# blyssprivacy/sdk

Measured on NVIDIA H100. Metric: PIR server queries/sec (Spiral process_query), higher is better.
Workload: dtype u64

## Files before the change

sdk_b200/build.py:

```python
import os
import subprocess
import sys

HERE = os.path.dirname(os.path.abspath(__file__))
CSRC = os.path.join(HERE, "csrc")
SO = os.path.join(HERE, "libb200pir.so")
SOURCES = ["api.cu", "poly_kernels.cu", "mul_kernels.cu", "imma_kernels.cu", "wire_kernels.cu", "tc5_kernels.cu", "dpir_gemm.cu",
           "export_kernels.cu"]
HEADERS = ["common.cuh", "kernels.h", "ntt_core.cuh", "tc5_layout.cuh", "tc5_ptx.cuh", "ntt_core4096.cuh", "ntt_tables.hpp",
           "item_place.cuh", "update_body.hpp", os.path.join("..", "..", "include", "b200pir.h")]
NVCC_FLAGS = ["-gencode", "arch=compute_90a,code=sm_90a", "-lineinfo", "-O3", "-std=c++17", "--extended-lambda",
              "-Xcompiler", "-fPIC", "-ccbin", "/usr/bin/g++" if os.path.exists("/usr/bin/g++") else "g++"]


def _stale():
    if not os.path.exists(SO):
        return True
    t = os.path.getmtime(SO)
    return any(os.path.getmtime(os.path.join(CSRC, f)) > t for f in SOURCES + HEADERS)


def build(force=False, verbose=False):
    if not force and not _stale():
        return SO
    nvcc = os.environ.get("NVCC", "/usr/local/cuda/bin/nvcc")
    objs = []
    procs = []
    for src in SOURCES:
        obj = os.path.join(CSRC, src.replace(".cu", ".o"))
        cmd = [nvcc] + NVCC_FLAGS + (["-Xptxas", "-v"] if verbose else []) + ["-c", os.path.join(CSRC, src), "-o", obj]
        procs.append((src, subprocess.Popen(cmd, stdout=subprocess.PIPE, stderr=subprocess.STDOUT, text=True)))
        objs.append(obj)
    for src, p in procs:
        out, _ = p.communicate()
        if verbose or p.returncode:
            sys.stderr.write(out)
        if p.returncode:
            raise RuntimeError("nvcc failed on " + src)
    subprocess.check_call([nvcc, "-shared", "-gencode", "arch=compute_90a,code=sm_90a", "-o", SO] + objs + ["-ccbin", NVCC_FLAGS[-1]])
    return SO


if __name__ == "__main__":
    print(build(force="--force" in sys.argv, verbose="-v" in sys.argv))
```

sdk_b200/csrc/api.cu:

```cuda
#include "../../include/b200pir.h"
#include "kernels.h"
#include "ntt_tables.hpp"
#include "update_body.hpp"
#include <cstdio>
#include <cerrno>
#include <fcntl.h>
#include <unistd.h>
#include <algorithm>
#include <cmath>
#include <memory>
#include <cstring>
#include <condition_variable>
#include <chrono>
#include <deque>
#include <mutex>
#include <set>
#include <string>
#include <utility>
#include <vector>

using namespace b200pir;

namespace b200pir {
thread_local unsigned long long g_kernel_launches = 0;

void opt_in_smem_impl(const void* kernel, int bytes) {
  static std::mutex mu;
  static std::set<std::pair<const void*, int>> done;
  int dev = 0;
  B200_CUDA(cudaGetDevice(&dev));
  std::lock_guard<std::mutex> lk(mu);
  if (done.count({kernel, dev})) return;
  B200_CUDA(cudaFuncSetAttribute(kernel, cudaFuncAttributeMaxDynamicSharedMemorySize, bytes));
  done.insert({kernel, dev});
}
}

namespace {

thread_local std::string g_last_error;

using b200pir::tables::build_tables;
using b200pir::tables::invmod;
uint64_t log2_ceil_u64(uint64_t a) { return (uint64_t)std::ceil(std::log2((double)a)); }
int bits_per(int t) {
  if (t == 56) return 1;
  return 56 / t + 1;
}
const uint64_t kQ2Values[37] = {0, 0, 0, 0, 0, 0, 0, 0, 0, 0, 0, 0, 0, 0, 12289ULL, 12289ULL, 61441ULL, 65537ULL,
                                65537ULL, 520193ULL, 786433ULL, 786433ULL, 3604481ULL, 7340033ULL, 16515073ULL,
                                33292289ULL, 67043329ULL, 132120577ULL, 268369921ULL, 469762049ULL, 1073479681ULL,
                                2013265921ULL, 4293918721ULL, 8588886017ULL, 17175674881ULL, 34359214081ULL,
                                68718428161ULL};

template <typename T>
struct DevBuf {
  T* p = nullptr;
  size_t n = 0;
  DevBuf() {}
  explicit DevBuf(size_t count) { alloc(count); }
  void alloc(size_t count) {
    release();
    n = count;
    if (count) B200_CUDA(cudaMalloc(&p, count * sizeof(T)));
  }
  void ensure(size_t count) { if (count > n) alloc(count); }
  void release() { if (p) cudaFree(p); p = nullptr; n = 0; }
  ~DevBuf() { release(); }
  DevBuf(const DevBuf&) = delete;
  DevBuf& operator=(const DevBuf&) = delete;
};

enum Stage { ST_EXPAND = 0, ST_MUL, ST_FROMNTT, ST_FOLD, ST_PACK, ST_ENCODE, ST_QIMG , ST_COUNT };

}

struct b200pir_ctx {
  int device = 0;
  cudaStream_t stream = nullptr;
  bool own_stream = true;
  std::recursive_mutex mu;
  b200pir_params hp;
  int dim0, num_per, slices, trials, g, stop_round, num_packing;
  int bits_gsw, bits_conv, bits_left, bits_right;
  bool has_right;
  uint64_t q2, q1, setup_bytes, query_bytes, response_bytes;
  int q1_bits;
  DevParams dp;
  DevBuf<Twiddle> d_tw;
  DevBuf<Twiddle> d_tw4k;
  DevBuf<uint32_t> d_neg1;
  int mul_variant = 0, max_group = 16, profile = 0;
  int intt_variant = 0;
  int expand_variant = 0;
  long pair_min_ctas = 1;
  int sparse_fold = 0;
  int imma_variant = 0;
  int db_format = -1;
  DevBuf<uint2> w_qf;
  DevBuf<uint8_t> w_qt;
  int sm_count = 0;
  size_t ws_queries = 0, ws_rows = 0;
  DevBuf<uint64_t> w_query;
  DevBuf<uint32_t> w_v;
  DevBuf<uint32_t> w_zflags;
  DevBuf<uint32_t> w_xr;
  DevBuf<uint4> w_qdev;
  DevBuf<uint32_t> w_vfold, w_vfold_neg;
  DevBuf<uint32_t> w_mult;
  DevBuf<uint32_t> w_cts;
  const uint32_t* folded = nullptr;
  size_t folded_stride = 0;
  DevBuf<uint64_t> w_packed;
  DevBuf<uint8_t> w_resp;
  static constexpr size_t kWriteStageBytes = (size_t)64 << 20;
  static constexpr size_t kWriteStageItems = 65536;
  DevBuf<uint8_t> w_wbytes;
  DevBuf<ItemWrite> w_witems;
  std::mutex export_mu;
  uint8_t* h_export[2] = {nullptr, nullptr};
  size_t h_export_bytes = 0;
  cudaEvent_t export_done[2] = {nullptr, nullptr};
  void ensure_export_staging(size_t bytes) {
    w_wbytes.ensure(std::max(kWriteStageBytes, bytes));
    if (!export_done[0])
      for (auto& e : export_done) B200_CUDA(cudaEventCreateWithFlags(&e, cudaEventDisableTiming | cudaEventBlockingSync));
    if (bytes <= h_export_bytes) return;
    release_export_pinned();
    const size_t n = std::max(kWriteStageBytes, bytes);
    for (auto& h : h_export) B200_CUDA(cudaHostAlloc(reinterpret_cast<void**>(&h), n, cudaHostAllocDefault));
    h_export_bytes = n;
  }
  void release_export_pinned() {
    for (auto& h : h_export) { if (h) cudaFreeHost(h); h = nullptr; }
    h_export_bytes = 0;
  }
  struct Pending {
    b200pir_db* db; b200pir_pp* pp; const uint64_t* query_ct; const uint8_t* query_bytes; uint8_t* out;
    int rc = 0; std::string err; bool done = false;
  };
  static constexpr size_t kCoalesceMax = 32;
  static constexpr size_t kPassQueries = 16;
  int coalesce = 1;
  int coalesce_window_us = 200;
  size_t last_batch = 0;
  std::chrono::steady_clock::time_point last_batch_end{};
  std::mutex qmu;
  std::condition_variable qcv;
  std::deque<Pending*> pending;
  bool leader_active = false;
  unsigned long long coalesced_batches = 0, coalesced_queries = 0;
  DevBuf<const uint32_t*> d_pptab;
  size_t pptab_cap = 0;
  std::vector<const uint32_t*> h_pptab;
  b200pir_pp* const* multi_pps = nullptr;
  PpTable pp_table(b200pir_pp* pp, size_t count);
  struct Span { int stage; cudaEvent_t a, b; };
  std::vector<Span> spans;
  std::vector<cudaEvent_t> event_pool;
  size_t event_next = 0;
  int mul_launches = 0;
  double last_ms[9] = {0, 0, 0, 0, 0, 0, 0, 0, 0};

  size_t v_words() const { return ((size_t)1 << g) * 4 * POLY; }
  size_t fold_words() const { return (size_t)hp.nu_2 * 2 * 2 * hp.t_gsw * 2 * POLY; }
  MulGeom geom(int rows) const { return MulGeom{dim0, rows, slices}; }

  cudaEvent_t get_event() {
    if (event_next == event_pool.size()) {
      cudaEvent_t e;
      B200_CUDA(cudaEventCreate(&e));
      event_pool.push_back(e);
    }
    return event_pool[event_next++];
  }
  struct Scope {
    b200pir_ctx* c; int stage; cudaEvent_t a = nullptr;
    Scope(b200pir_ctx* ctx, int st) : c(ctx), stage(st) {
      if (c->profile) { a = c->get_event(); cudaEventRecord(a, c->stream); }
    }
    ~Scope() {
      if (c->profile) { cudaEvent_t b = c->get_event(); cudaEventRecord(b, c->stream); c->spans.push_back({stage, a, b}); }
    }
  };
  void prof_reset() { if (profile == 2) return; spans.clear(); event_next = 0; mul_launches = 0; }
  void prof_collect() {
    if (!profile) return;
    B200_CUDA(cudaStreamSynchronize(stream));
    for (int i = 0; i < 9; i++) last_ms[i] = 0;
    for (auto& s : spans) {
      float ms = 0;
      cudaEventElapsedTime(&ms, s.a, s.b);
      last_ms[s.stage == ST_QIMG ? 8 : s.stage] += ms;
      last_ms[6] += ms;
    }
    last_ms[7] = mul_launches;
  }
  void ensure_workspace_lite(size_t queries, size_t rows) {
    w_mult.ensure(queries * slices * rows * 4 * POLY);
    w_cts.ensure(queries * slices * rows * 4 * POLY);
    w_packed.ensure(queries * hp.instances * (hp.n + 1) * hp.n * POLY);
  }
  void ensure_workspace(size_t queries, size_t rows) {
    if (queries <= ws_queries && rows <= ws_rows) return;
    queries = std::max(queries, ws_queries);
    rows = std::max(rows, ws_rows);
    w_query.ensure(queries * 2 * POLY);
    if (hp.expand_queries) w_v.ensure(queries * v_words());
    w_qdev.ensure(queries * (size_t)dim0 * POLY);
    w_vfold.ensure(queries * std::max<size_t>(fold_words(), 1));
    w_vfold_neg.ensure(queries * std::max<size_t>(fold_words(), 1));
    w_mult.ensure(queries * slices * rows * 4 * POLY);
    w_cts.ensure(queries * slices * rows * 4 * POLY);
    w_packed.ensure(queries * hp.instances * (hp.n + 1) * hp.n * POLY);
    w_resp.ensure(queries * response_bytes);
    ws_queries = queries;
    ws_rows = rows;
  }
};

struct b200pir_db {
  b200pir_ctx* ctx;
  Shard shard;
  int rows;
  int format = 0;
  DevBuf<uint4> d;
  DevBuf<uint4> f;
  DevBuf<uint8_t> t;
  Tc5Geom T;
  ImmaGeom F;
  size_t slice_cells() const { return (size_t)rows * (ctx->dim0 / 2) * POLY; }
  std::vector<uint64_t> present;
  uint64_t present_count = 0;
  std::vector<uint32_t> h_tile_mask;
  DevBuf<uint32_t> tile_mask;
  uint64_t capacity() const { return (uint64_t)ctx->slices * rows * ctx->dim0; }
  void presence_init() {
    present.assign((capacity() + 63) / 64, 0);
    present_count = 0;
    h_tile_mask.assign((size_t)ctx->slices * T.mt, 0u);
    tile_mask.alloc(h_tile_mask.size());
    B200_CUDA(cudaMemset(tile_mask.p, 0, h_tile_mask.size() * 4));
  }
  bool mark_host(int slice, int il, int j) {
    const uint64_t bit = ((uint64_t)slice * rows + il) * ctx->dim0 + j;
    if (!((present[bit >> 6] >> (bit & 63)) & 1)) { present[bit >> 6] |= 1ull << (bit & 63); present_count++; }
    const size_t w = (size_t)slice * T.mt + (il >> 5);
    const uint32_t nv = h_tile_mask[w] | (1u << (j >> 5));
    if (nv == h_tile_mask[w]) return false;
    h_tile_mask[w] = nv;
    return true;
  }
  void mark(int slice, int il, int j, cudaStream_t s) {
    if (mark_host(slice, il, j)) {
      const size_t w = (size_t)slice * T.mt + (il >> 5);
      B200_CUDA(cudaMemcpyAsync(tile_mask.p + w, &h_tile_mask[w], 4, cudaMemcpyHostToDevice, s));
    }
  }
  void mark_items(const ItemWrite* items, size_t count, cudaStream_t s) {
    bool changed = false;
    for (size_t k = 0; k < count; k++)
      for (int sl = 0; sl < ctx->slices; sl++) changed |= mark_host(sl, (int)items[k].il, (int)items[k].j);
    if (changed)
      B200_CUDA(cudaMemcpyAsync(tile_mask.p, h_tile_mask.data(), h_tile_mask.size() * 4, cudaMemcpyHostToDevice, s));
  }
  void mark_slice(int slice, cudaStream_t s) {
    const uint64_t lo = (uint64_t)slice * rows * ctx->dim0, hi = lo + (uint64_t)rows * ctx->dim0;
    for (uint64_t b = lo; b < hi; b++)
      if (!((present[b >> 6] >> (b & 63)) & 1)) { present[b >> 6] |= 1ull << (b & 63); present_count++; }
    const uint32_t full = T.ks >= 32 ? 0xffffffffu : ((1u << T.ks) - 1u);
    for (int m = 0; m < T.mt; m++) h_tile_mask[(size_t)slice * T.mt + m] = full;
    B200_CUDA(cudaMemcpyAsync(tile_mask.p + (size_t)slice * T.mt, &h_tile_mask[(size_t)slice * T.mt], (size_t)T.mt * 4,
                              cudaMemcpyHostToDevice, s));
  }
};

struct b200pir_pp {
  b200pir_ctx* ctx;
  DevBuf<uint32_t> pack, left, right, conv;
};

PpTable b200pir_ctx::pp_table(b200pir_pp* pp, size_t count) {
  if (count > pptab_cap) {
    pptab_cap = std::max<size_t>(count, 16);
    d_pptab.alloc(4 * pptab_cap);
    h_pptab.clear();
  }
  std::vector<const uint32_t*> h(4 * pptab_cap, nullptr);
  for (size_t i = 0; i < count; i++) {
    const b200pir_pp* p = multi_pps ? multi_pps[i] : pp;
    h[0 * pptab_cap + i] = p->pack.p;
    h[1 * pptab_cap + i] = p->left.p;
    h[2 * pptab_cap + i] = p->right.p ? p->right.p : p->left.p;
    h[3 * pptab_cap + i] = p->conv.p;
  }
  if (h != h_pptab) {
    B200_CUDA(cudaMemcpyAsync(d_pptab.p, h.data(), h.size() * sizeof(const uint32_t*), cudaMemcpyHostToDevice, stream));
    h_pptab = h;
  }
  return PpTable{d_pptab.p, d_pptab.p + pptab_cap, d_pptab.p + 2 * pptab_cap, d_pptab.p + 3 * pptab_cap};
}

struct b200pir_dpir {
  int device;
  std::mutex mu;
  cudaStream_t stream = nullptr;
  bool own_stream = true;
  uint64_t rows, cols;
  DevBuf<uint32_t> a;
  DevBuf<uint32_t> b, out;
};

namespace {

int fail(const std::exception& e) {
  cudaGetLastError();
  g_last_error = e.what();
  const Error* pe = dynamic_cast<const Error*>(&e);
  return pe ? pe->code : B200PIR_E_CUDA;
}
#define API_BEGIN try {
#define API_END                                     \
  }                                                 \
  catch (const std::exception& e) { return fail(e); } \
  return 0;

struct Guard {
  std::lock_guard<std::recursive_mutex> lk;
  explicit Guard(b200pir_ctx* c) : lk(c->mu) { cudaSetDevice(c->device); }
};

void upload_ntt32(b200pir_ctx* c, DevBuf<uint32_t>& dst, const uint64_t* host, size_t words) {
  dst.alloc(words);
  DevBuf<uint64_t> tmp(words);
  B200_CUDA(cudaMemcpyAsync(tmp.p, host, words * 8, cudaMemcpyHostToDevice, c->stream));
  launch_narrow(dst.p, tmp.p, words, c->stream);
  B200_CUDA(cudaStreamSynchronize(c->stream));
}


void run_coefficient_expansion(b200pir_ctx* c, b200pir_pp* pp, uint32_t* v, size_t v_stride, int nq, bool all_slots) {
  const auto& hp = c->hp;
  cudaStream_t s = c->stream;
  const int g = c->g;
  const int stop_round = hp.nu_2 > 0 ? c->stop_round : 0;
  const int max_right = hp.nu_2 > 0 ? (int)(hp.t_gsw * hp.nu_2) : 0;
  const PpTable T = c->pp_table(pp, (size_t)nq);
  for (int r = 0; r < g; r++) {
    const int num_in = 1 << r;
    const long active = (long)((stop_round > 0 && r > stop_round) ? num_in / 2 : num_in) * nq;
    const bool pair = c->expand_variant != 1 && active >= c->pair_min_ctas;
    if (!pair) launch_expand_scalar(c->dp, v, v_stride, nq, num_in, c->d_neg1.p + (size_t)r * 2 * POLY, s);
    ExpandRound R;
    R.r = r; R.num_in = num_in; R.stop_round = stop_round; R.max_bits_to_gen_right = max_right;
    R.fill_skipped = all_slots ? 1 : 0;
    R.t_auto = (POLY >> r) + 1;
    R.t_left = (int)hp.t_exp_left; R.bits_left = c->bits_left;
    R.tab_left = T.left; R.off_left = (size_t)r * 2 * hp.t_exp_left * 2 * POLY;
    if (hp.nu_2 > 0 && c->has_right) {
      int rr = r <= c->stop_round ? r : c->stop_round;
      R.t_right = (int)hp.t_exp_right; R.bits_right = c->bits_right;
      R.tab_right = T.right; R.off_right = (size_t)rr * 2 * hp.t_exp_right * 2 * POLY;
    } else {
      R.t_right = R.t_left; R.bits_right = R.bits_left; R.tab_right = T.left; R.off_right = R.off_left;
    }
    if (pair && c->expand_variant == 0) {
      const size_t xr_stride = (size_t)num_in * 2 * POLY;
      c->w_xr.ensure((size_t)nq * xr_stride);
      launch_expand_round_res(c->dp, v, v_stride, c->w_xr.p, xr_stride, nq, R, c->d_neg1.p + (size_t)r * 2 * POLY, s);
    } else if (pair) launch_expand_round_pair(c->dp, v, v_stride, nq, R, c->d_neg1.p + (size_t)r * 2 * POLY, s);
    else launch_expand_round(c->dp, v, v_stride, nq, R, s);
  }
}

void run_expand_query(b200pir_ctx* c, b200pir_pp* pp, const uint64_t* query_raw, uint32_t* v, uint4* q_dev,
                      uint32_t* v_fold, int nq, uint8_t* images = nullptr) {
  const auto& hp = c->hp;
  cudaStream_t s = c->stream;
  launch_to_ntt_strided(c->dp, v, c->v_words(), query_raw, (size_t)2 * POLY, 2, nq, s);
  run_coefficient_expansion(c, pp, v, c->v_words(), nq, false);
  const int factor = hp.nu_2 > 0 ? 2 : 1;
  if (images) {
    const Tc5Geom T = make_tc5_geom(c->dim0, 32);
    for (int q0 = 0; q0 < nq; q0 += 16)
      launch_reorient_to_tc5(T, v + (size_t)q0 * c->v_words(), c->v_words(), factor, std::min(16, nq - q0),
                             images + (size_t)(q0 / 16) * tc5_query_bytes(T), s);
  } else {
    launch_reorient(c->geom(c->num_per), q_dev, (size_t)c->dim0 * POLY, v, c->v_words(), nq, factor, s);
  }
  if (hp.nu_2 > 0)
    launch_regev_to_gsw(c->dp, v_fold, c->fold_words(), v, c->v_words(), nq, (int)hp.nu_2, 2, 1, c->pp_table(pp, (size_t)nq).conv,
                        (int)hp.t_gsw, (int)hp.t_conv, c->bits_conv, s);
}

void run_fold(b200pir_ctx* c, uint64_t* cts, size_t batch, size_t batch_stride, size_t num, int k0,
              const uint32_t* vfold, const uint32_t* vfold_neg, int slices_per_query) {
  const size_t mat = (size_t)2 * 2 * c->hp.t_gsw * 2 * POLY;
  int k = k0;
  for (size_t half = num / 2; half >= 1; half /= 2, k--) {
    launch_fold_round(c->dp, cts, batch, batch_stride, (int)half, vfold + (size_t)k * mat, vfold_neg + (size_t)k * mat,
                      c->fold_words(), slices_per_query, (int)c->hp.t_gsw, c->bits_gsw, c->stream);
  }
}

const uint32_t* run_fold_res(b200pir_ctx* c, uint32_t* a, uint32_t* b, size_t batch, size_t batch_stride, size_t num,
                             int k0, const uint32_t* vfold, int slices_per_query) {
  const size_t mat = (size_t)2 * 2 * c->hp.t_gsw * 2 * POLY;
  int k = k0;
  uint32_t* src = a;
  uint32_t* dst = b;
  uint32_t* zero_flags = nullptr;
  if (c->sparse_fold) {
    c->w_zflags.ensure(batch * num);
    zero_flags = c->w_zflags.p;
  }
  for (size_t half = num / 2; half >= 1; half /= 2, k--) {
    launch_fold_res(c->dp, src, dst, batch, batch_stride, (int)half, vfold + (size_t)k * mat, c->fold_words(),
                    slices_per_query, (int)c->hp.t_gsw, c->bits_gsw, zero_flags, c->stream);
    std::swap(src, dst);
  }
  return src;
}

void run_prepare(b200pir_ctx* c, b200pir_pp* pp, size_t count, bool images = false) {
  b200pir_ctx::Scope sc(c, ST_EXPAND);
  if (images) c->w_qt.ensure((count + 15) / 16 * tc5_query_bytes(make_tc5_geom(c->dim0, 32)));
  if (c->hp.expand_queries)
    run_expand_query(c, pp, c->w_query.p, c->w_v.p, c->w_qdev.p, c->w_vfold.p, (int)count, images ? c->w_qt.p : nullptr);
}

void run_first_dim_and_fold(b200pir_ctx* c, b200pir_db* db, size_t count, const uint4* qdev = nullptr,
                            const uint32_t* vfold = nullptr, const uint8_t* images = nullptr, size_t per_group = 16) {
  if (!qdev) qdev = c->w_qdev.p;
  if (!vfold) vfold = c->w_vfold.p;
  const int rows = db->rows;
  MulGeom G = c->geom(rows);
  const size_t q_stride = (size_t)c->dim0 * POLY;
  const size_t out_stride = (size_t)c->slices * rows * 4 * POLY;
  if (db->format == 0) {
    {
      b200pir_ctx::Scope sc(c, ST_MUL);
      size_t qi = 0;
      while (qi < count) {
        int nq = 1;
        if (count - qi >= 4 && c->max_group >= 4) nq = 4;
        else if (count - qi >= 2 && c->max_group >= 2) nq = 2;
        launch_multiply(c->dp, G, db->d.p, qdev + qi * q_stride, c->w_mult.p + qi * out_stride, 0, c->slices, nq,
                        q_stride, out_stride, c->mul_variant, c->stream);
        c->mul_launches++;
        qi += nq;
      }
    }
    {
      b200pir_ctx::Scope sc(c, ST_FROMNTT);
      launch_ntt32(c->dp, c->w_mult.p, count * c->slices * rows * 2, true, c->stream);
    }
  } else if (db->format == 2) {
    if (!images) c->w_qt.ensure(tc5_query_bytes(db->T));
    const size_t step = images ? per_group : 16;
    for (size_t qi = 0, g = 0; qi < count; qi += step, g++) {
      const int nq = (int)std::min<size_t>(step, count - qi);
      const uint8_t* qt = images ? images + g * tc5_query_bytes(db->T) : c->w_qt.p;
      if (!images) {
        b200pir_ctx::Scope sq(c, ST_QIMG);
        launch_query_to_tc5(db->T, qdev + qi * q_stride, q_stride, nq, c->w_qt.p, c->stream);
      }
      b200pir_ctx::Scope sc(c, ST_MUL);
      launch_multiply_tc5(c->dp, db->T, db->t.p, db->tile_mask.p, qt, c->w_cts.p + qi * out_stride, out_stride, nq, 0, c->slices,
                          c->sm_count, c->stream);
      c->mul_launches++;
    }
    {
      b200pir_ctx::Scope sc(c, ST_FROMNTT);
      launch_intt_from_zmajor(c->dp, db->F, c->w_cts.p, out_stride, c->w_mult.p, (int)count, c->slices, c->intt_variant, c->stream);
    }
  } else {
    c->w_qf.ensure(imma_query_cells(db->F));
    const size_t per_pass = (c->max_group >= 16 && imma_supports_16(db->F)) ? 16 : (c->max_group >= 8 ? 8 : 4);
    for (size_t qi = 0; qi < count; qi += per_pass) {
      const int nq = (int)std::min<size_t>(per_pass, count - qi);
      {
        b200pir_ctx::Scope sq(c, ST_QIMG);
        launch_query_to_frag(db->F, qdev + qi * q_stride, q_stride, nq, c->w_qf.p, c->stream);
      }
      {
        b200pir_ctx::Scope sc(c, ST_MUL);
        launch_multiply_imma(c->dp, db->F, db->f.p, c->w_qf.p, c->w_cts.p + qi * out_stride, out_stride, nq, 0, c->slices,
                             c->imma_variant, c->stream);
        c->mul_launches++;
      }
    }
    {
      b200pir_ctx::Scope sc(c, ST_FROMNTT);
      launch_intt_from_zmajor(c->dp, db->F, c->w_cts.p, out_stride, c->w_mult.p, (int)count, c->slices, c->intt_variant, c->stream);
    }
  }
  {
    b200pir_ctx::Scope sc(c, ST_FOLD);
    c->folded = c->w_mult.p;
    c->folded_stride = (size_t)rows * 4 * POLY;
    if (rows > 1)
      c->folded = run_fold_res(c, c->w_mult.p, c->w_cts.p, count * c->slices, (size_t)rows * 4 * POLY, rows,
                               (int)c->hp.nu_2 - 1, vfold, c->slices);
  }
}

void run_pack_encode(b200pir_ctx* c, b200pir_pp* pp, const uint32_t* folded, size_t ct_stride, size_t count,
                     uint8_t* out_dev) {
  const auto& hp = c->hp;
  const size_t packed_words = (size_t)hp.instances * (hp.n + 1) * hp.n * POLY;
  {
    b200pir_ctx::Scope sc(c, ST_PACK);
    launch_pack(c->dp, c->w_packed.p, packed_words, folded, ct_stride, (size_t)c->slices * ct_stride, (int)count, c->pp_table(pp, count).pack,
                (int)hp.n, (int)hp.instances, (int)hp.t_conv, c->bits_conv, (int)hp.version, c->stream);
  }
  {
    b200pir_ctx::Scope sc(c, ST_ENCODE);
    launch_encode(c->dp, out_dev, c->response_bytes, c->w_packed.p, packed_words, (int)count, (int)hp.n, (int)hp.instances,
                  c->q2, (int)hp.q2_bits, c->q1, c->q1_bits, c->stream);
  }
}

bool same_params(const b200pir_ctx* a, const b200pir_ctx* b) {
  return a == b || (a->device == b->device && std::memcmp(&a->hp, &b->hp, sizeof(b200pir_params)) == 0);
}
void check_db(b200pir_ctx* c, b200pir_db* db) {
  if (!db || !same_params(db->ctx, c)) throw Error(B200PIR_E_BADARG, "db handle was created for different parameters / device");
}
void check_pp(b200pir_ctx* c, b200pir_pp* pp) {
  if (!pp || !same_params(pp->ctx, c)) throw Error(B200PIR_E_BADARG, "pp handle was created for different parameters / device");
}

}

extern "C" {

const char* b200pir_last_error(void) { return g_last_error.c_str(); }
int b200pir_device_count(void) {
  int n = 0;
  if (cudaGetDeviceCount(&n) != cudaSuccess) return 0;
  return n;
}

int b200pir_ctx_create(const b200pir_params* params, int device, b200pir_ctx** out) {
  API_BEGIN
  if (!params || !out) throw Error(B200PIR_E_BADARG, "null argument");
  int ndev = 0;
  B200_CUDA(cudaGetDeviceCount(&ndev));
  if (device < 0 || device >= ndev) throw Error(B200PIR_E_BADARG, "no such CUDA device (this library has no CPU path)");
  B200_CUDA(cudaSetDevice(device));
  std::unique_ptr<b200pir_ctx> c(new b200pir_ctx());
  c->device = device;
  B200_CUDA(cudaDeviceGetAttribute(&c->sm_count, cudaDevAttrMultiProcessorCount, device));
  c->hp = *params;
  auto& hp = c->hp;
  if (hp.q2_bits < 14) hp.q2_bits = 14;
  if (hp.q2_bits > 36) throw Error(B200PIR_E_BADARG, "q2_bits out of range");
  if (hp.instances == 0) hp.instances = 1;
  if (hp.n < 1 || hp.n > 4) throw Error(B200PIR_E_UNSUPPORTED, "n must be 1..4");
  if (hp.nu_1 < 1 || hp.nu_1 > 16 || hp.nu_2 > 16) throw Error(B200PIR_E_BADARG, "nu_1/nu_2 out of range");
  if (hp.version > 1) throw Error(B200PIR_E_BADARG, "unknown version");
  if (hp.p < 2 || (hp.p & (hp.p - 1)) || hp.p > (1u << 20)) throw Error(B200PIR_E_BADARG, "p must be a power of two <= 2^20");
  for (uint64_t t : {hp.t_gsw, hp.t_conv, hp.t_exp_left, hp.t_exp_right})
    if (t < 3 || t > 56)
      throw Error(B200PIR_E_UNSUPPORTED, "gadget dimensions must be in 3..56");
  if (hp.db_item_size == 0) hp.db_item_size = hp.instances * hp.n * hp.n * 2048 * log2_ceil_u64(hp.p) / 8;
  c->dim0 = 1 << hp.nu_1;
  c->num_per = 1 << hp.nu_2;
  c->trials = (int)(hp.n * hp.n);
  c->slices = (int)(hp.instances * c->trials);
  c->g = (int)log2_ceil_u64(hp.t_gsw * hp.nu_2 + c->dim0);
  c->stop_round = hp.nu_2 ? (int)log2_ceil_u64(hp.t_gsw * hp.nu_2) : 0;
  if (c->g > 11) throw Error(B200PIR_E_UNSUPPORTED, "expansion needs more than 2048 slots");
  if (hp.expand_queries && hp.nu_2 > 0 && 2 * std::max<uint64_t>(c->dim0, hp.t_gsw * hp.nu_2) > (1ull << c->g))
    throw Error(B200PIR_E_UNSUPPORTED, "expansion: dim0 and t_gsw * nu_2 must each fit in half of the 2^g slots");
  c->num_packing = hp.version == 0 ? (int)hp.n : 2;
  c->has_right = hp.expand_queries && (hp.version == 0 || hp.t_exp_right != hp.t_exp_left);
  c->bits_gsw = bits_per((int)hp.t_gsw);
  c->bits_conv = bits_per((int)hp.t_conv);
  c->bits_left = bits_per((int)hp.t_exp_left);
  c->bits_right = bits_per((int)hp.t_exp_right);
  c->q2 = kQ2Values[hp.q2_bits];
  c->q1 = 4 * hp.p;
  c->q1_bits = (int)log2_ceil_u64(c->q1);
  {
    uint64_t bits = hp.instances * (hp.q2_bits * hp.n * 2048 + (uint64_t)c->q1_bits * hp.n * hp.n * 2048);
    c->response_bytes = ((bits + 63) / 64) * 8;
    uint64_t sz = (uint64_t)c->num_packing * hp.n * hp.t_conv;
    if (hp.expand_queries) {
      uint64_t right = (uint64_t)(c->stop_round + 1) * hp.t_exp_right;
      if (hp.version > 0 && hp.t_exp_left == hp.t_exp_right) right = 0;
      sz += (uint64_t)c->g * hp.t_exp_left + right + 2 * hp.t_conv;
    }
    c->setup_bytes = 32 + sz * 2048 * 8;
    uint64_t qp = hp.expand_queries ? 1 : (uint64_t)c->dim0 + hp.nu_2 * 2 * hp.t_gsw;
    c->query_bytes = 32 + qp * 2048 * 8;
  }
  B200_CUDA(cudaStreamCreateWithFlags(&c->stream, cudaStreamNonBlocking));
  const uint64_t q0 = 268369921ULL, q1m = 249561089ULL;
  std::vector<Twiddle> f0, i0, f1, i1;
  build_tables(q0, f0, i0);
  build_tables(q1m, f1, i1);
  std::vector<Twiddle> l0, l1;
  b200pir::tables::build_inverse_table_lz(q0, l0);
  b200pir::tables::build_inverse_table_lz(q1m, l1);
  c->d_tw.alloc(6 * POLY);
  B200_CUDA(cudaMemcpy(c->d_tw.p + 4 * POLY, l0.data(), POLY * sizeof(Twiddle), cudaMemcpyHostToDevice));
  B200_CUDA(cudaMemcpy(c->d_tw.p + 5 * POLY, l1.data(), POLY * sizeof(Twiddle), cudaMemcpyHostToDevice));
  B200_CUDA(cudaMemcpy(c->d_tw.p, f0.data(), POLY * sizeof(Twiddle), cudaMemcpyHostToDevice));
  B200_CUDA(cudaMemcpy(c->d_tw.p + POLY, i0.data(), POLY * sizeof(Twiddle), cudaMemcpyHostToDevice));
  B200_CUDA(cudaMemcpy(c->d_tw.p + 2 * POLY, f1.data(), POLY * sizeof(Twiddle), cudaMemcpyHostToDevice));
  B200_CUDA(cudaMemcpy(c->d_tw.p + 3 * POLY, i1.data(), POLY * sizeof(Twiddle), cudaMemcpyHostToDevice));
  {
    std::vector<Twiddle> lo(2 * 3 * 64);
    for (int i = 0; i < 64; i++) { lo[(0 * 3 + 0) * 64 + i] = f0[i]; lo[(0 * 3 + 1) * 64 + i] = i0[i]; lo[(0 * 3 + 2) * 64 + i] = l0[i];
                                   lo[(1 * 3 + 0) * 64 + i] = f1[i]; lo[(1 * 3 + 1) * 64 + i] = i1[i]; lo[(1 * 3 + 2) * 64 + i] = l1[i]; }
    upload_poly_constants(lo.data());
    upload_mul_constants(lo.data());
    upload_imma_constants(lo.data());
  }
  DevParams& dp = c->dp;
  dp.q[0] = (uint32_t)q0; dp.q[1] = (uint32_t)q1m;
  dp.cr1[0] = (uint64_t)(((u128)1 << 64) / q0);
  dp.cr1[1] = (uint64_t)(((u128)1 << 64) / q1m);
  dp.modulus = q0 * q1m;
  dp.cr1_mod = (uint64_t)(((u128)1 << 64) / dp.modulus);
  dp.q1_inv_mod_q0 = (uint32_t)invmod(q1m % q0, q0);
  dp.fwd[0] = c->d_tw.p; dp.inv[0] = c->d_tw.p + POLY; dp.fwd[1] = c->d_tw.p + 2 * POLY; dp.inv[1] = c->d_tw.p + 3 * POLY;
  dp.inv_lz[0] = c->d_tw.p + 4 * POLY; dp.inv_lz[1] = c->d_tw.p + 5 * POLY;
  dp.mu58[0] = (uint32_t)(((uint64_t)1 << 58) / q0); dp.mu58[1] = (uint32_t)(((uint64_t)1 << 58) / q1m);
  {
    std::vector<uint32_t> h((size_t)NTT_LOG_N * 2 * POLY, 0);
    for (int i = 0; i < NTT_LOG_N; i++) {
      int idx = POLY - (1 << i);
      h[((size_t)i * 2 + 0) * POLY + idx] = (uint32_t)(q0 - 1);
      h[((size_t)i * 2 + 1) * POLY + idx] = (uint32_t)(q1m - 1);
    }
    c->d_neg1.alloc(h.size());
    B200_CUDA(cudaMemcpy(c->d_neg1.p, h.data(), h.size() * 4, cudaMemcpyHostToDevice));
    launch_ntt32(dp, c->d_neg1.p, NTT_LOG_N, false, c->stream);
    B200_CUDA(cudaStreamSynchronize(c->stream));
  }
  B200_CUDA(cudaGetLastError());
  *out = c.release();
  API_END
}

void b200pir_ctx_destroy(b200pir_ctx* c) {
  if (!c) return;
  cudaSetDevice(c->device);
  cudaDeviceSynchronize();
  for (auto e : c->event_pool) cudaEventDestroy(e);
  c->release_export_pinned();
  for (auto e : c->export_done) if (e) cudaEventDestroy(e);
  if (c->own_stream && c->stream) cudaStreamDestroy(c->stream);
  delete c;
}
int b200pir_ctx_set_stream(b200pir_ctx* c, void* cuda_stream) {
  API_BEGIN
  if (!c) throw Error(B200PIR_E_BADARG, "null ctx");
  Guard gd(c);
  B200_CUDA(cudaStreamSynchronize(c->stream));
  if (c->own_stream && c->stream) cudaStreamDestroy(c->stream);
  c->stream = (cudaStream_t)cuda_stream;
  c->own_stream = false;
  API_END
}
int b200pir_ctx_synchronize(b200pir_ctx* c) {
  API_BEGIN
  if (!c) throw Error(B200PIR_E_BADARG, "null ctx");
  Guard gd(c);
  B200_CUDA(cudaStreamSynchronize(c->stream));
  B200_CUDA(cudaGetLastError());
  API_END
}
int b200pir_ctx_reserve(b200pir_ctx* c, size_t queries, size_t rows_local) {
  API_BEGIN
  if (!c) throw Error(B200PIR_E_BADARG, "null ctx");
  if (queries == 0 || queries > 4096 || rows_local == 0 || rows_local > ((size_t)1 << c->hp.nu_2))
    throw Error(B200PIR_E_BADARG, "reserve: 1..4096 queries, 1..num_per rows");
  Guard gd(c);
  B200_CUDA(cudaStreamSynchronize(c->stream));
  c->ensure_workspace(queries, rows_local);
  B200_CUDA(cudaGetLastError());
  API_END
}
int b200pir_ctx_set_option(b200pir_ctx* c, const char* key, int64_t value) {
  API_BEGIN
  if (!c || !key) throw Error(B200PIR_E_BADARG, "null argument");
  Guard gd(c);
  std::string k(key);
  if (k == "mul_variant") c->mul_variant = (int)value;
  else if (k == "batch") { if (value != 1 && value != 2 && value != 4 && value != 8 && value != 16) throw Error(B200PIR_E_BADARG, "batch must be 1, 2, 4, 8 or 16"); c->max_group = (int)value; }
  else if (k == "fold_variant") {}
  else if (k == "intt_variant") c->intt_variant = (int)value;
  else if (k == "imma_variant") c->imma_variant = (int)value;
  else if (k == "sparse_fold") c->sparse_fold = value != 0;
  else if (k == "coalesce") c->coalesce = value != 0;
  else if (k == "coalesce_window_us") { if (value < 0 || value > 100000) throw Error(B200PIR_E_BADARG, "coalesce_window_us must be 0..100000"); c->coalesce_window_us = (int)value; }
  else if (k == "expand_variant") c->expand_variant = (int)value;
  else if (k == "expand_pair_min_ctas") c->pair_min_ctas = (long)value;
  else if (k == "db_format") { if (value < -1 || value > 2) throw Error(B200PIR_E_BADARG, "db_format must be -1 (automatic), 0, 1 or 2"); c->db_format = (int)value; }
  else if (k == "profile") {
    if (value < 0 || value > 2) throw Error(B200PIR_E_BADARG, "profile must be 0, 1 or 2");
    c->profile = (int)value;
    c->spans.clear(); c->event_next = 0; c->mul_launches = 0;
  }
  else throw Error(B200PIR_E_BADARG, "unknown option " + k);
  API_END
}
int b200pir_ctx_sizes(b200pir_ctx* c, uint64_t* setup_bytes, uint64_t* query_bytes, uint64_t* response_bytes) {
  API_BEGIN
  if (!c) throw Error(B200PIR_E_BADARG, "null ctx");
  if (setup_bytes) *setup_bytes = c->setup_bytes;
  if (query_bytes) *query_bytes = c->query_bytes;
  if (response_bytes) *response_bytes = c->response_bytes;
  API_END
}

int b200pir_db_create(b200pir_ctx* c, uint64_t shard_index, uint64_t shard_count, b200pir_db** out) {
  API_BEGIN
  if (!c || !out) throw Error(B200PIR_E_BADARG, "null argument");
  Guard gd(c);
  if (shard_count == 0) { shard_count = 1; shard_index = 0; }
  if (shard_index >= shard_count || (shard_count & (shard_count - 1)) || (uint64_t)c->num_per % shard_count)
    throw Error(B200PIR_E_BADARG, "shard_count must be a power of two dividing num_per");
  std::unique_ptr<b200pir_db> db(new b200pir_db());
  db->ctx = c;
  db->shard = Shard{(int)shard_index, (int)shard_count};
  db->rows = c->num_per / (int)shard_count;
  db->F = make_imma_geom(c->dim0, db->rows);
  db->T = make_tc5_geom(c->dim0, db->rows);
  db->format = c->db_format >= 0 ? c->db_format : (tc5_supported(db->T) ? 2 : 1);
  db->presence_init();
  if (db->format == 0) {
    size_t cells = (size_t)c->slices * db->slice_cells();
    db->d.alloc(cells);
    B200_CUDA(cudaMemsetAsync(db->d.p, 0, cells * sizeof(uint4), c->stream));
  } else if (db->format == 2) {
    if (!tc5_supported(db->T)) throw Error(B200PIR_E_UNSUPPORTED, "db_format 2: dim0 too large for the wgmma kernel");
    size_t bytes = tc5_db_bytes(db->T, c->slices);
    db->t.alloc(bytes);
    B200_CUDA(cudaMemsetAsync(db->t.p, 0, bytes, c->stream));
  } else {
    size_t cells = imma_db_cells(db->F, c->slices);
    db->f.alloc(cells);
    B200_CUDA(cudaMemsetAsync(db->f.p, 0, cells * sizeof(uint4), c->stream));
  }
  B200_CUDA(cudaStreamSynchronize(c->stream));
  *out = db.release();
  API_END
}
void b200pir_db_destroy(b200pir_db* db) {
  if (!db) return;
  cudaSetDevice(db->ctx->device);
  delete db;
}
extern "C++" {
namespace {
template <typename Fetch>
void upload_slice_impl(b200pir_ctx* c, b200pir_db* db, uint64_t slice, Fetch fetch) {
  const size_t per_z = (size_t)c->dim0 * c->num_per;
  int zc = (int)std::max<size_t>(1, std::min<size_t>(POLY, ((size_t)64 << 20) / (per_z * 8)));
  DevBuf<uint64_t> stage(per_z * zc);
  MulGeom G = c->geom(db->rows);
  DevBuf<uint4> tmp;
  uint4* dst;
  if (db->format == 0) dst = db->d.p + (size_t)slice * db->slice_cells();
  else { tmp.alloc(db->slice_cells()); dst = tmp.p; }
  for (int z0 = 0; z0 < POLY; z0 += zc) {
    int cur = std::min(zc, POLY - z0);
    const uint64_t* src = fetch((size_t)z0 * per_z, per_z * cur);
    B200_CUDA(cudaMemcpyAsync(stage.p, src, per_z * cur * 8, cudaMemcpyHostToDevice, c->stream));
    launch_db_retile_chunk(G, db->shard, dst, stage.p, z0, cur, c->stream);
    B200_CUDA(cudaStreamSynchronize(c->stream));
  }
  if (db->format == 1) {
    launch_db_to_frag(db->F, tmp.p, db->f.p, (int)slice, c->stream);
    B200_CUDA(cudaStreamSynchronize(c->stream));
  } else if (db->format == 2) {
    launch_db_to_tc5(db->T, tmp.p, db->t.p, (int)slice, c->stream);
    B200_CUDA(cudaStreamSynchronize(c->stream));
  }
  db->mark_slice((int)slice, c->stream);
  B200_CUDA(cudaStreamSynchronize(c->stream));
  B200_CUDA(cudaGetLastError());
}

void write_items(b200pir_ctx* c, b200pir_db* db, const uint8_t* host, size_t span, const ItemWrite* items, size_t count) {
  if (count == 0) return;
  c->w_wbytes.ensure(std::max(b200pir_ctx::kWriteStageBytes, span));
  c->w_witems.ensure(std::max(b200pir_ctx::kWriteStageItems, count));
  if (span) B200_CUDA(cudaMemcpyAsync(c->w_wbytes.p, host, span, cudaMemcpyHostToDevice, c->stream));
  B200_CUDA(cudaMemcpyAsync(c->w_witems.p, items, count * sizeof(ItemWrite), cudaMemcpyHostToDevice, c->stream));
  const size_t chunks = (size_t)c->slices;
  const size_t bpc = (c->hp.db_item_size + chunks - 1) / chunks;
  const DbDst dst{db->format, c->geom(db->rows), db->F, db->T, db->d.p, db->f.p, db->t.p};
  launch_write_items(c->dp, dst, c->w_wbytes.p, c->w_witems.p, (int)count, (int)chunks, (int)bpc, c->hp.p, c->stream);
}

template <typename Sink>
void export_impl(b200pir_ctx* c, b200pir_db* db, int slice_begin, int slice_end, Sink sink) {
  std::lock_guard<std::mutex> ex(c->export_mu);
  const size_t per_z = (size_t)db->rows * c->dim0;
  const int zc = (int)std::max<size_t>(1, std::min<size_t>(POLY, b200pir_ctx::kWriteStageBytes / (per_z * 8)));
  struct Chunk { int slice, z0, zc; };
  std::vector<Chunk> chunks;
  for (int s = slice_begin; s < slice_end; s++)
    for (int z0 = 0; z0 < POLY; z0 += zc) chunks.push_back(Chunk{s, z0, std::min(zc, POLY - z0)});
  {
    Guard gd(c);
    c->ensure_export_staging(per_z * zc * 8);
  }
  auto consume = [&](size_t k) {
    const int b = (int)(k & 1);
    B200_CUDA(cudaEventSynchronize(c->export_done[b]));
    sink(chunks[k].slice, chunks[k].z0, chunks[k].zc, reinterpret_cast<const uint64_t*>(c->h_export[b]));
  };
  try {
    for (size_t k = 0; k < chunks.size(); k++) {
      {
        Guard gd(c);
        const DbDst dst{db->format, c->geom(db->rows), db->F, db->T, db->d.p, db->f.p, db->t.p};
        uint64_t* stage = reinterpret_cast<uint64_t*>(c->w_wbytes.p);
        launch_db_export(dst, chunks[k].slice, chunks[k].z0, chunks[k].zc, stage, c->stream);
        B200_CUDA(cudaMemcpyAsync(c->h_export[k & 1], stage, per_z * chunks[k].zc * 8, cudaMemcpyDeviceToHost, c->stream));
        B200_CUDA(cudaEventRecord(c->export_done[k & 1], c->stream));
      }
      if (k > 0) consume(k - 1);
    }
    if (!chunks.empty()) consume(chunks.size() - 1);
  } catch (...) {
    for (auto e : c->export_done) cudaEventSynchronize(e);
    throw;
  }
  B200_CUDA(cudaGetLastError());
}

void download_impl(b200pir_ctx* c, b200pir_db* db, int slice_begin, int slice_end, uint64_t* words) {
  const size_t d0 = (size_t)c->dim0, npg = (size_t)c->num_per, rows = (size_t)db->rows;
  const size_t G = (size_t)db->shard.count, gi = (size_t)db->shard.index;
  const size_t slice_words = d0 * npg * POLY;
  export_impl(c, db, slice_begin, slice_end, [&](int s, int z0, int zc, const uint64_t* src) {
    uint64_t* dst = words + (size_t)(s - slice_begin) * slice_words + (size_t)z0 * npg * d0;
    if (G == 1) { std::memcpy(dst, src, (size_t)zc * rows * d0 * 8); return; }
    for (size_t zl = 0; zl < (size_t)zc; zl++)
      for (size_t il = 0; il < rows; il++)
        std::memcpy(dst + (zl * npg + il * G + gi) * d0, src + (zl * rows + il) * d0, d0 * 8);
  });
}
}
}

int b200pir_db_upload_slice(b200pir_ctx* c, b200pir_db* db, uint64_t slice, const uint64_t* words, size_t n_words) {
  API_BEGIN
  if (!c || !words) throw Error(B200PIR_E_BADARG, "null argument");
  Guard gd(c);
  check_db(c, db);
  const size_t slice_words = (size_t)c->dim0 * c->num_per * POLY;
  if (slice >= (uint64_t)c->slices) throw Error(B200PIR_E_SHAPE, "slice out of range");
  if (n_words != slice_words) throw Error(B200PIR_E_SHAPE, "slice must hold dim0*num_per*2048 words");
  upload_slice_impl(c, db, slice, [&](size_t off, size_t) { return words + off; });
  API_END
}
int b200pir_db_load_file(b200pir_ctx* c, b200pir_db* db, const char* path) {
  API_BEGIN
  if (!c || !path) throw Error(B200PIR_E_BADARG, "null argument");
  Guard gd(c);
  check_db(c, db);
  const size_t slice_words = (size_t)c->dim0 * c->num_per * POLY;
  struct Closer { FILE* f; ~Closer() { if (f) fclose(f); } } file{fopen(path, "rb")};
  if (!file.f) throw Error(B200PIR_E_BADARG, std::string("cannot open ") + path);
  if (fseeko(file.f, 0, SEEK_END)) throw Error(B200PIR_E_BADARG, "cannot seek in the database file");
  const off_t bytes = ftello(file.f);
  if (bytes < 0 || (uint64_t)bytes != (uint64_t)slice_words * c->slices * 8)
    throw Error(B200PIR_E_SHAPE, "database file must hold slices*dim0*num_per*2048 u64 words");
  std::vector<uint64_t> buf;
  for (int s = 0; s < c->slices; s++) {
    upload_slice_impl(c, db, (uint64_t)s, [&](size_t off, size_t n) -> const uint64_t* {
      buf.resize(n);
      if (fseeko(file.f, (off_t)(((size_t)s * slice_words + off) * 8), SEEK_SET) || fread(buf.data(), 8, n, file.f) != n)
        throw Error(B200PIR_E_SHAPE, "short read from the database file");
      return buf.data();
    });
// ... 209 lines not shown
  check_db(c, db);
  MulGeom G = c->geom(db->rows);
  size_t per_slice = (size_t)db->rows * (c->dim0 / 2);
  int step = (int)std::max<size_t>(1, std::min<size_t>(c->slices, ((size_t)1 << 30) / per_slice));
  if (db->format == 0) {
    for (int s0 = 0; s0 < c->slices; s0 += step)
      launch_db_synth(c->dp, G, db->shard, db->d.p, seed, c->hp.p, s0, std::min(step, c->slices - s0), c->stream);
  } else {
    DevBuf<uint4> tmp(db->slice_cells());
    for (int s0 = 0; s0 < c->slices; s0++) {
      launch_db_synth(c->dp, G, db->shard, tmp.p - (size_t)s0 * db->slice_cells(), seed, c->hp.p, s0, 1, c->stream);
      if (db->format == 2) launch_db_to_tc5(db->T, tmp.p, db->t.p, s0, c->stream);
      else launch_db_to_frag(db->F, tmp.p, db->f.p, s0, c->stream);
    }
  }
  for (int s0 = 0; s0 < c->slices; s0++) db->mark_slice(s0, c->stream);
  B200_CUDA(cudaStreamSynchronize(c->stream));
  B200_CUDA(cudaGetLastError());
  API_END
}

int b200pir_pp_create(b200pir_ctx* c, const uint64_t* v_packing, const uint64_t* left, const uint64_t* right,
                      const uint64_t* conv, b200pir_pp** out) {
  API_BEGIN
  if (!c || !out || !v_packing) throw Error(B200PIR_E_BADARG, "null argument");
  Guard gd(c);
  const auto& hp = c->hp;
  std::unique_ptr<b200pir_pp> pp(new b200pir_pp());
  pp->ctx = c;
  const size_t W = 2 * POLY;
  upload_ntt32(c, pp->pack, v_packing, (size_t)c->num_packing * (hp.n + 1) * hp.t_conv * W);
  if (hp.expand_queries) {
    if (!left || !conv) throw Error(B200PIR_E_BADARG, "expansion parameters missing");
    upload_ntt32(c, pp->left, left, (size_t)c->g * 2 * hp.t_exp_left * W);
    if (c->has_right) {
      if (!right) throw Error(B200PIR_E_BADARG, "v_expansion_right missing");
      upload_ntt32(c, pp->right, right, (size_t)(c->stop_round + 1) * 2 * hp.t_exp_right * W);
    }
    upload_ntt32(c, pp->conv, conv, (size_t)2 * 2 * hp.t_conv * W);
  }
  *out = pp.release();
  API_END
}

namespace {
void deserialize_group(b200pir_ctx* c, DevBuf<uint32_t>& dst, const uint8_t* seed, const uint8_t*& data, uint64_t& word,
                       size_t count, size_t rows, size_t cols) {
  const size_t row_words = cols * POLY, mat_words = rows * row_words, rest = (rows - 1) * row_words;
  DevBuf<uint64_t> raw(count * mat_words);
  launch_chacha_first_rows(raw.p, seed, word, (uint32_t)count, (uint32_t)row_words, mat_words, c->dp.modulus, c->stream);
  word += count * row_words;
  for (size_t i = 0; i < count; i++) {
    B200_CUDA(cudaMemcpyAsync(raw.p + i * mat_words + row_words, data, rest * 8, cudaMemcpyHostToDevice, c->stream));
    data += rest * 8;
  }
  dst.alloc(count * mat_words * 2);
  launch_to_ntt(c->dp, dst.p, raw.p, count * rows * cols, c->stream);
  B200_CUDA(cudaStreamSynchronize(c->stream));
}
}

int b200pir_pp_create_from_bytes(b200pir_ctx* c, const uint8_t* data, size_t len, b200pir_pp** out) {
  API_BEGIN
  if (!c || !out || !data) throw Error(B200PIR_E_BADARG, "null argument");
  if (len != c->setup_bytes) throw Error(B200PIR_E_SHAPE, "setup data: expected " + std::to_string(c->setup_bytes) + " bytes");
  Guard gd(c);
  const auto& hp = c->hp;
  std::unique_ptr<b200pir_pp> pp(new b200pir_pp());
  pp->ctx = c;
  const uint8_t* seed = data;
  const uint8_t* cur = data + 32;
  uint64_t word = 0;
  deserialize_group(c, pp->pack, seed, cur, word, (size_t)c->num_packing, hp.n + 1, hp.t_conv);
  if (hp.expand_queries) {
    deserialize_group(c, pp->left, seed, cur, word, (size_t)c->g, 2, hp.t_exp_left);
    if (c->has_right) deserialize_group(c, pp->right, seed, cur, word, (size_t)c->stop_round + 1, 2, hp.t_exp_right);
    deserialize_group(c, pp->conv, seed, cur, word, 1, 2, 2 * hp.t_conv);
  }
  if ((size_t)(cur - data) != len) throw Error(B200PIR_E_SHAPE, "setup data: trailing bytes");
  *out = pp.release();
  API_END
}

namespace {
void deserialize_queries(b200pir_ctx* c, const uint8_t* data, size_t count, uint64_t* dst_dev) {
  for (size_t i = 0; i < count; i++) {
    const uint8_t* q = data + i * c->query_bytes;
    launch_chacha_first_rows(dst_dev + i * 2 * POLY, q, 0, 1, POLY, 2 * POLY, c->dp.modulus, c->stream);
    B200_CUDA(cudaMemcpyAsync(dst_dev + i * 2 * POLY + POLY, q + 32, POLY * 8, cudaMemcpyHostToDevice, c->stream));
  }
}
void deserialize_query_direct(b200pir_ctx* c, const uint8_t* q, size_t slot) {
  const size_t dim0 = (size_t)c->dim0, t2 = 2 * c->hp.t_gsw, nu2 = c->hp.nu_2;
  cudaStream_t s = c->stream;
  DevBuf<uint64_t> sig_raw(dim0 * POLY);
  DevBuf<uint32_t> sig_ntt(dim0 * 2 * POLY);
  launch_chacha_first_rows(sig_raw.p, q, 0, (uint32_t)dim0, POLY, POLY, c->dp.modulus, s);
  launch_to_ntt(c->dp, sig_ntt.p, sig_raw.p, dim0, s);
  DevBuf<uint64_t> wire(dim0 * POLY);
  B200_CUDA(cudaMemcpyAsync(wire.p, q + 32, dim0 * POLY * 8, cudaMemcpyHostToDevice, s));
  launch_direct_query_to_dev(c->w_qdev.p + slot * dim0 * POLY, sig_ntt.p, wire.p, (int)dim0, s);
  if (nu2) {
    DevBuf<uint64_t> raw(nu2 * 2 * t2 * POLY);
    launch_chacha_first_rows(raw.p, q, dim0 * POLY, (uint32_t)nu2, (uint32_t)(t2 * POLY), 2 * t2 * POLY, c->dp.modulus, s);
    const uint8_t* rest = q + 32 + dim0 * POLY * 8;
    for (size_t i = 0; i < nu2; i++)
      B200_CUDA(cudaMemcpyAsync(raw.p + (i * 2 + 1) * t2 * POLY, rest + i * t2 * POLY * 8, t2 * POLY * 8, cudaMemcpyHostToDevice, s));
    launch_to_ntt(c->dp, c->w_vfold.p + slot * c->fold_words(), raw.p, nu2 * 2 * t2, s);
  }
  B200_CUDA(cudaStreamSynchronize(s));
}
}

int b200pir_query_from_bytes(b200pir_ctx* c, const uint8_t* data, size_t len, uint64_t* query_ct) {
  API_BEGIN
  if (!c || !data || !query_ct) throw Error(B200PIR_E_BADARG, "null argument");
  if (!c->hp.expand_queries) throw Error(B200PIR_E_UNSUPPORTED, "serialized direct-upload queries are not supported");
  if (len != c->query_bytes) throw Error(B200PIR_E_SHAPE, "query: expected " + std::to_string(c->query_bytes) + " bytes");
  Guard gd(c);
  DevBuf<uint64_t> ct(2 * POLY);
  deserialize_queries(c, data, 1, ct.p);
  B200_CUDA(cudaMemcpyAsync(query_ct, ct.p, 2 * POLY * 8, cudaMemcpyDeviceToHost, c->stream));
  B200_CUDA(cudaStreamSynchronize(c->stream));
  API_END
}

void b200pir_pp_destroy(b200pir_pp* pp) {
  if (!pp) return;
  cudaSetDevice(pp->ctx->device);
  delete pp;
}

static int ntt_host(b200pir_ctx* c, uint64_t* polys, size_t count, bool inverse) {
  API_BEGIN
  if (!c || (!polys && count)) throw Error(B200PIR_E_BADARG, "null argument");
  Guard gd(c);
  if (count == 0) return 0;
  DevBuf<uint64_t> d(count * 2 * POLY);
  B200_CUDA(cudaMemcpyAsync(d.p, polys, d.n * 8, cudaMemcpyHostToDevice, c->stream));
  launch_ntt_u64(c->dp, d.p, count, inverse, c->stream);
  B200_CUDA(cudaMemcpyAsync(polys, d.p, d.n * 8, cudaMemcpyDeviceToHost, c->stream));
  B200_CUDA(cudaStreamSynchronize(c->stream));
  B200_CUDA(cudaGetLastError());
  API_END
}
int b200pir_ntt_forward(b200pir_ctx* c, uint64_t* polys, size_t count) { return ntt_host(c, polys, count, false); }
int b200pir_ntt_inverse(b200pir_ctx* c, uint64_t* polys, size_t count) { return ntt_host(c, polys, count, true); }

int b200pir_ntt32_dev(b200pir_ctx* c, uint32_t* polys_dev, size_t count, int inverse) {
  API_BEGIN
  if (!c || !polys_dev) throw Error(B200PIR_E_BADARG, "null argument");
  Guard gd(c);
  launch_ntt32(c->dp, polys_dev, count, inverse != 0, c->stream);
  B200_CUDA(cudaGetLastError());
  API_END
}

namespace {
const Twiddle* tables_4k(b200pir_ctx* c) {
  if (!c->d_tw4k.p) {
    const int N = 4096, LG = 12;
    std::vector<Twiddle> all;
    for (int n = 0; n < 2; n++) {
      std::vector<Twiddle> f, i;
      build_tables(c->dp.q[n], f, i, N, LG);
      all.insert(all.end(), f.begin(), f.end());
      all.insert(all.end(), i.begin(), i.end());
    }
    c->d_tw4k.alloc(all.size());
    B200_CUDA(cudaMemcpy(c->d_tw4k.p, all.data(), all.size() * sizeof(Twiddle), cudaMemcpyHostToDevice));
  }
  return c->d_tw4k.p;
}
}
int b200pir_ntt4096_dev(b200pir_ctx* c, uint32_t* polys_dev, size_t count, int inverse) {
  API_BEGIN
  if (!c || !polys_dev) throw Error(B200PIR_E_BADARG, "null argument");
  Guard gd(c);
  launch_ntt32_4k(c->dp.q[0], c->dp.q[1], tables_4k(c), polys_dev, count, inverse != 0, c->stream);
  B200_CUDA(cudaGetLastError());
  API_END
}
int b200pir_ntt4096(b200pir_ctx* c, uint64_t* polys, size_t count, int inverse) {
  API_BEGIN
  if (!c || (!polys && count)) throw Error(B200PIR_E_BADARG, "null argument");
  Guard gd(c);
  if (count == 0) return 0;
  const size_t words = count * 2 * 4096;
  DevBuf<uint64_t> wide(words);
  DevBuf<uint32_t> nar(words);
  B200_CUDA(cudaMemcpyAsync(wide.p, polys, words * 8, cudaMemcpyHostToDevice, c->stream));
  launch_narrow(nar.p, wide.p, words, c->stream);
  launch_ntt32_4k(c->dp.q[0], c->dp.q[1], tables_4k(c), nar.p, count, inverse != 0, c->stream);
  launch_widen(wide.p, nar.p, words, c->stream);
  B200_CUDA(cudaMemcpyAsync(polys, wide.p, words * 8, cudaMemcpyDeviceToHost, c->stream));
  B200_CUDA(cudaStreamSynchronize(c->stream));
  B200_CUDA(cudaGetLastError());
  API_END
}

int b200pir_to_ntt(b200pir_ctx* c, uint64_t* out_ntt, const uint64_t* raw, size_t count) {
  API_BEGIN
  if (!c || !out_ntt || !raw) throw Error(B200PIR_E_BADARG, "null argument");
  Guard gd(c);
  DevBuf<uint64_t> in(count * POLY), wide(count * 2 * POLY);
  DevBuf<uint32_t> o(count * 2 * POLY);
  B200_CUDA(cudaMemcpyAsync(in.p, raw, in.n * 8, cudaMemcpyHostToDevice, c->stream));
  launch_to_ntt(c->dp, o.p, in.p, count, c->stream);
  launch_widen(wide.p, o.p, o.n, c->stream);
  B200_CUDA(cudaMemcpyAsync(out_ntt, wide.p, wide.n * 8, cudaMemcpyDeviceToHost, c->stream));
  B200_CUDA(cudaStreamSynchronize(c->stream));
  B200_CUDA(cudaGetLastError());
  API_END
}
int b200pir_from_ntt(b200pir_ctx* c, uint64_t* out_raw, const uint64_t* ntt, size_t count) {
  API_BEGIN
  if (!c || !out_raw || !ntt) throw Error(B200PIR_E_BADARG, "null argument");
  Guard gd(c);
  DevBuf<uint64_t> wide(count * 2 * POLY), o(count * POLY);
  DevBuf<uint32_t> in(count * 2 * POLY);
  B200_CUDA(cudaMemcpyAsync(wide.p, ntt, wide.n * 8, cudaMemcpyHostToDevice, c->stream));
  launch_narrow(in.p, wide.p, in.n, c->stream);
  launch_from_ntt(c->dp, o.p, in.p, count, c->stream);
  B200_CUDA(cudaMemcpyAsync(out_raw, o.p, o.n * 8, cudaMemcpyDeviceToHost, c->stream));
  B200_CUDA(cudaStreamSynchronize(c->stream));
  B200_CUDA(cudaGetLastError());
  API_END
}

int b200pir_multiply_reg_by_database(b200pir_ctx* c, b200pir_db* db, uint64_t slice, const uint64_t* v_firstdim,
                                     uint64_t* out) {
  API_BEGIN
  if (!c || !v_firstdim || !out) throw Error(B200PIR_E_BADARG, "null argument");
  Guard gd(c);
  check_db(c, db);
  if (slice >= (uint64_t)c->slices) throw Error(B200PIR_E_SHAPE, "slice out of range");
  const int rows = db->rows;
  MulGeom G = c->geom(rows);
  DevBuf<uint64_t> vq((size_t)c->dim0 * 2 * POLY);
  DevBuf<uint4> qd((size_t)c->dim0 * POLY);
  DevBuf<uint32_t> o((size_t)c->slices * rows * 4 * POLY);
  DevBuf<uint64_t> wide((size_t)rows * 4 * POLY);
  B200_CUDA(cudaMemcpyAsync(vq.p, v_firstdim, vq.n * 8, cudaMemcpyHostToDevice, c->stream));
  launch_query_to_dev(G, qd.p, vq.p, c->stream);
  if (db->format == 0) {
    launch_multiply(c->dp, G, db->d.p, qd.p, o.p, (int)slice, 1, 1, 0, 0, c->mul_variant, c->stream);
  } else if (db->format == 2) {
    DevBuf<uint8_t> qt(tc5_query_bytes(db->T));
    DevBuf<uint32_t> zm((size_t)c->slices * rows * 4 * POLY);
    launch_query_to_tc5(db->T, qd.p, 0, 1, qt.p, c->stream);
    launch_multiply_tc5(c->dp, db->T, db->t.p, db->tile_mask.p, qt.p, zm.p, 0, 1, (int)slice, 1, c->sm_count, c->stream);
    launch_zmajor_to_ntt32(db->F, zm.p, o.p + (size_t)slice * rows * 4 * POLY, (int)slice, c->stream);
    B200_CUDA(cudaStreamSynchronize(c->stream));
  } else {
    DevBuf<uint2> qf(imma_query_cells(db->F));
    DevBuf<uint32_t> zm((size_t)c->slices * rows * 4 * POLY);
    launch_query_to_frag(db->F, qd.p, 0, 1, qf.p, c->stream);
    launch_multiply_imma(c->dp, db->F, db->f.p, qf.p, zm.p, 0, 1, (int)slice, 1, c->imma_variant, c->stream);
    launch_zmajor_to_ntt32(db->F, zm.p, o.p + (size_t)slice * rows * 4 * POLY, (int)slice, c->stream);
    B200_CUDA(cudaStreamSynchronize(c->stream));
  }
  launch_widen(wide.p, o.p + (size_t)slice * rows * 4 * POLY, wide.n, c->stream);
  B200_CUDA(cudaMemcpyAsync(out, wide.p, wide.n * 8, cudaMemcpyDeviceToHost, c->stream));
  B200_CUDA(cudaStreamSynchronize(c->stream));
  B200_CUDA(cudaGetLastError());
  API_END
}

int b200pir_fold_ciphertexts(b200pir_ctx* c, uint64_t* v_cts, size_t num, const uint64_t* v_folding,
                             const uint64_t* v_folding_neg) {
  API_BEGIN
  if (!c || !v_cts) throw Error(B200PIR_E_BADARG, "null argument");
  Guard gd(c);
  if (num == 0 || (num & (num - 1))) throw Error(B200PIR_E_SHAPE, "number of ciphertexts must be a power of two");
  if (num == 1) return 0;
  if (!v_folding) throw Error(B200PIR_E_BADARG, "null argument");
  int dims = 0;
  while (((size_t)1 << dims) < num) dims++;
  if (dims > (int)c->hp.nu_2) throw Error(B200PIR_E_SHAPE, "more ciphertexts than 2^nu_2");
  const size_t mat = (size_t)2 * 2 * c->hp.t_gsw * 2 * POLY;
  DevBuf<uint64_t> cts(num * 2 * POLY), wide(dims * mat);
  DevBuf<uint32_t> vf(c->fold_words());
  B200_CUDA(cudaMemcpyAsync(cts.p, v_cts, cts.n * 8, cudaMemcpyHostToDevice, c->stream));
  B200_CUDA(cudaMemcpyAsync(wide.p, v_folding, wide.n * 8, cudaMemcpyHostToDevice, c->stream));
  launch_narrow(vf.p, wide.p, wide.n, c->stream);
  const bool has_q = std::find(v_cts, v_cts + cts.n, c->dp.modulus) != v_cts + cts.n;
  if ((v_folding_neg || has_q) && !c->sparse_fold) {
    DevBuf<uint32_t> vfn(c->fold_words());
    if (v_folding_neg) {
      B200_CUDA(cudaMemcpyAsync(wide.p, v_folding_neg, wide.n * 8, cudaMemcpyHostToDevice, c->stream));
      launch_narrow(vfn.p, wide.p, wide.n, c->stream);
    } else {
      launch_folding_neg(c->dp, vfn.p, vf.p, dims, (int)c->hp.t_gsw, c->bits_gsw, c->stream);
    }
    run_fold(c, cts.p, 1, num * 2 * POLY, num, dims - 1, vf.p, vfn.p, 1);
  } else {
    DevBuf<uint32_t> a(num * 4 * POLY), b(num * 4 * POLY);
    DevBuf<uint32_t> zflags;
    if (c->sparse_fold) zflags.alloc(num);
    launch_raw_to_res(c->dp, a.p, cts.p, num * 2, c->stream);
    int k = dims - 1;
    for (size_t half = num / 2; half >= 1; half /= 2, k--) {
      launch_fold_res(c->dp, a.p, b.p, 1, num * 4 * POLY, (int)half, vf.p + (size_t)k * mat, c->fold_words(), 1,
                      (int)c->hp.t_gsw, c->bits_gsw, zflags.p, c->stream);
      B200_CUDA(cudaMemcpyAsync(a.p, b.p, half * 4 * POLY * 4, cudaMemcpyDeviceToDevice, c->stream));
    }
    launch_res_to_raw(c->dp, cts.p, a.p, num * 2, c->stream);
  }
  B200_CUDA(cudaMemcpyAsync(v_cts, cts.p, cts.n * 8, cudaMemcpyDeviceToHost, c->stream));
  B200_CUDA(cudaStreamSynchronize(c->stream));
  B200_CUDA(cudaGetLastError());
  API_END
}

int b200pir_get_v_folding_neg(b200pir_ctx* c, uint64_t* out, const uint64_t* v_folding) {
  API_BEGIN
  if (!c || !out || !v_folding) throw Error(B200PIR_E_BADARG, "null argument");
  Guard gd(c);
  const size_t words = c->fold_words();
  if (!words) return 0;
  DevBuf<uint64_t> wide(words);
  DevBuf<uint32_t> in(words), o(words);
  B200_CUDA(cudaMemcpyAsync(wide.p, v_folding, words * 8, cudaMemcpyHostToDevice, c->stream));
  launch_narrow(in.p, wide.p, words, c->stream);
  launch_folding_neg(c->dp, o.p, in.p, (int)c->hp.nu_2, (int)c->hp.t_gsw, c->bits_gsw, c->stream);
  launch_widen(wide.p, o.p, words, c->stream);
  B200_CUDA(cudaMemcpyAsync(out, wide.p, words * 8, cudaMemcpyDeviceToHost, c->stream));
  B200_CUDA(cudaStreamSynchronize(c->stream));
  B200_CUDA(cudaGetLastError());
  API_END
}

int b200pir_coefficient_expansion(b200pir_ctx* c, b200pir_pp* pp, uint64_t* v) {
  API_BEGIN
  if (!c || !v) throw Error(B200PIR_E_BADARG, "null argument");
  Guard gd(c);
  check_pp(c, pp);
  if (!c->hp.expand_queries) throw Error(B200PIR_E_BADARG, "context was created with expand_queries = 0");
  const size_t words = c->v_words();
  DevBuf<uint64_t> wide(words);
  DevBuf<uint32_t> dv(words);
  B200_CUDA(cudaMemcpyAsync(wide.p, v, words * 8, cudaMemcpyHostToDevice, c->stream));
  launch_narrow(dv.p, wide.p, words, c->stream);
  run_coefficient_expansion(c, pp, dv.p, words, 1, true);
  launch_widen(wide.p, dv.p, words, c->stream);
  B200_CUDA(cudaMemcpyAsync(v, wide.p, words * 8, cudaMemcpyDeviceToHost, c->stream));
  B200_CUDA(cudaStreamSynchronize(c->stream));
  B200_CUDA(cudaGetLastError());
  API_END
}

int b200pir_expand_query(b200pir_ctx* c, b200pir_pp* pp, const uint64_t* query_ct, uint64_t* out_v_firstdim,
                         uint64_t* out_v_folding) {
  API_BEGIN
  if (!c || !query_ct || !out_v_firstdim) throw Error(B200PIR_E_BADARG, "null argument");
  Guard gd(c);
  check_pp(c, pp);
  if (!c->hp.expand_queries) throw Error(B200PIR_E_BADARG, "context was created with expand_queries = 0");
  c->ensure_workspace(1, 1);
  B200_CUDA(cudaMemcpyAsync(c->w_query.p, query_ct, 2 * POLY * 8, cudaMemcpyHostToDevice, c->stream));
  run_expand_query(c, pp, c->w_query.p, c->w_v.p, c->w_qdev.p, c->w_vfold.p, 1);
  const size_t qwords = (size_t)c->dim0 * 2 * POLY;
  std::vector<uint32_t> hq(qwords * 2);
  B200_CUDA(cudaMemcpyAsync(hq.data(), c->w_qdev.p, hq.size() * 4, cudaMemcpyDeviceToHost, c->stream));
  B200_CUDA(cudaStreamSynchronize(c->stream));
  for (int j = 0; j < c->dim0; j++)
    for (int z = 0; z < POLY; z++) {
      const uint32_t* cell = hq.data() + (((size_t)(j >> 1) * 2 + (j & 1)) * POLY + z) * 4;
      out_v_firstdim[((size_t)z * c->dim0 + j) * 2 + 0] = (uint64_t)cell[0] | ((uint64_t)cell[1] << 32);
      out_v_firstdim[((size_t)z * c->dim0 + j) * 2 + 1] = (uint64_t)cell[2] | ((uint64_t)cell[3] << 32);
    }
  if (out_v_folding && c->fold_words()) {
    DevBuf<uint64_t> wide(c->fold_words());
    launch_widen(wide.p, c->w_vfold.p, c->fold_words(), c->stream);
    B200_CUDA(cudaMemcpyAsync(out_v_folding, wide.p, wide.n * 8, cudaMemcpyDeviceToHost, c->stream));
    B200_CUDA(cudaStreamSynchronize(c->stream));
  }
  B200_CUDA(cudaGetLastError());
  API_END
}

int b200pir_pack(b200pir_ctx* c, b200pir_pp* pp, const uint64_t* v_ct, uint64_t* out_ntt) {
  API_BEGIN
  if (!c || !v_ct || !out_ntt) throw Error(B200PIR_E_BADARG, "null argument");
  Guard gd(c);
  check_pp(c, pp);
  const auto& hp = c->hp;
  const size_t nn = hp.n * hp.n, outp = (hp.n + 1) * hp.n;
  DevBuf<uint64_t> cts(nn * 2 * POLY), raw(outp * POLY), wide(outp * 2 * POLY);
  DevBuf<uint32_t> o(outp * 2 * POLY), res(nn * 4 * POLY);
  B200_CUDA(cudaMemcpyAsync(cts.p, v_ct, cts.n * 8, cudaMemcpyHostToDevice, c->stream));
  launch_raw_to_res(c->dp, res.p, cts.p, nn * 2, c->stream);
  launch_pack(c->dp, raw.p, 0, res.p, 4 * POLY, 0, 1, c->pp_table(pp, 1).pack, (int)hp.n, 1, (int)hp.t_conv, c->bits_conv, (int)hp.version, c->stream,
              cts.p);
  launch_to_ntt(c->dp, o.p, raw.p, outp, c->stream);
  launch_widen(wide.p, o.p, o.n, c->stream);
  B200_CUDA(cudaMemcpyAsync(out_ntt, wide.p, wide.n * 8, cudaMemcpyDeviceToHost, c->stream));
  B200_CUDA(cudaStreamSynchronize(c->stream));
  B200_CUDA(cudaGetLastError());
  API_END
}

int b200pir_encode(b200pir_ctx* c, const uint64_t* v_packed_raw, uint8_t* out, size_t* out_len) {
  API_BEGIN
  if (!c || !v_packed_raw || !out) throw Error(B200PIR_E_BADARG, "null argument");
  Guard gd(c);
  const auto& hp = c->hp;
  const size_t words = (size_t)hp.instances * (hp.n + 1) * hp.n * POLY;
  DevBuf<uint64_t> in(words);
  DevBuf<uint8_t> o(c->response_bytes);
  B200_CUDA(cudaMemcpyAsync(in.p, v_packed_raw, words * 8, cudaMemcpyHostToDevice, c->stream));
  launch_encode(c->dp, o.p, c->response_bytes, in.p, 0, 1, (int)hp.n, (int)hp.instances, c->q2, (int)hp.q2_bits, c->q1, c->q1_bits, c->stream);
  B200_CUDA(cudaMemcpyAsync(out, o.p, c->response_bytes, cudaMemcpyDeviceToHost, c->stream));
  B200_CUDA(cudaStreamSynchronize(c->stream));
  if (out_len) *out_len = c->response_bytes;
  B200_CUDA(cudaGetLastError());
  API_END
}

static void run_query_batch_resident(b200pir_ctx* c, b200pir_db* db, b200pir_pp* pp, size_t count, uint8_t* out_dev) {
  const bool images = db->format == 2 && c->hp.expand_queries;
  run_prepare(c, pp, count, images);
  run_first_dim_and_fold(c, db, count, nullptr, nullptr, images ? c->w_qt.p : nullptr, 16);
  run_pack_encode(c, pp, c->folded, c->folded_stride, count, out_dev);
}

int b200pir_process_query_batch_dev(b200pir_ctx* c, b200pir_db* db, b200pir_pp* pp, const uint64_t* query_cts_dev,
                                    size_t count, uint8_t* out_dev) {
  API_BEGIN
  if (!c || !out_dev || !query_cts_dev) throw Error(B200PIR_E_BADARG, "null argument");
  Guard gd(c);
  check_db(c, db);
  check_pp(c, pp);
  if (db->shard.count != 1) throw Error(B200PIR_E_BADARG, "sharded database: use the stage_a / stage_b entry points");
  if (!c->hp.expand_queries) throw Error(B200PIR_E_BADARG, "batch entry point needs expand_queries");
  if (count == 0) return 0;
  c->ensure_workspace(count, db->rows);
  c->prof_reset();
  B200_CUDA(cudaMemcpyAsync(c->w_query.p, query_cts_dev, count * 2 * POLY * 8, cudaMemcpyDeviceToDevice, c->stream));
  run_query_batch_resident(c, db, pp, count, out_dev);
  B200_CUDA(cudaGetLastError());
  API_END
}

int b200pir_process_query_batch(b200pir_ctx* c, b200pir_db* db, b200pir_pp* pp, const uint64_t* query_cts, size_t count,
                                uint8_t* out, size_t* out_len_each) {
  API_BEGIN
  if (!c || !out || !query_cts) throw Error(B200PIR_E_BADARG, "null argument");
  Guard gd(c);
  check_db(c, db);
  check_pp(c, pp);
  if (db->shard.count != 1) throw Error(B200PIR_E_BADARG, "sharded database: use the stage_a / stage_b entry points");
  if (!c->hp.expand_queries) throw Error(B200PIR_E_BADARG, "batch entry point needs expand_queries");
  if (count == 0) return 0;
  c->ensure_workspace(count, db->rows);
  c->prof_reset();
  B200_CUDA(cudaMemcpyAsync(c->w_query.p, query_cts, count * 2 * POLY * 8, cudaMemcpyHostToDevice, c->stream));
  run_query_batch_resident(c, db, pp, count, c->w_resp.p);
  B200_CUDA(cudaMemcpyAsync(out, c->w_resp.p, count * c->response_bytes, cudaMemcpyDeviceToHost, c->stream));
  B200_CUDA(cudaStreamSynchronize(c->stream));
  if (c->profile == 1) c->prof_collect();
  if (out_len_each) *out_len_each = c->response_bytes;
  B200_CUDA(cudaGetLastError());
  API_END
}

namespace {
void process_multi(b200pir_ctx* c, b200pir_db* db, b200pir_pp* const* pps, const uint64_t* const* cts,
                   const uint8_t* const* bytes, size_t count, uint8_t* const* outs) {
  Guard gd(c);
  check_db(c, db);
  for (size_t i = 0; i < count; i++) check_pp(c, pps[i]);
  if (db->shard.count != 1) throw Error(B200PIR_E_BADARG, "sharded database: use the stage_a / stage_b entry points");
  if (!c->hp.expand_queries) throw Error(B200PIR_E_BADARG, "multi-client batches need expand_queries");
  c->ensure_workspace(std::max(count, c->coalesce ? b200pir_ctx::kCoalesceMax : count), db->rows);
  c->prof_reset();
  for (size_t i = 0; i < count; i++) {
    if (bytes && bytes[i]) deserialize_queries(c, bytes[i], 1, c->w_query.p + i * 2 * POLY);
    else B200_CUDA(cudaMemcpyAsync(c->w_query.p + i * 2 * POLY, cts[i], 2 * POLY * 8, cudaMemcpyHostToDevice, c->stream));
  }
  c->multi_pps = pps;
  try {
    run_query_batch_resident(c, db, pps[0], count, c->w_resp.p);
  } catch (...) { c->multi_pps = nullptr; throw; }
  c->multi_pps = nullptr;
  for (size_t i = 0; i < count; i++)
    B200_CUDA(cudaMemcpyAsync(outs[i], c->w_resp.p + i * c->response_bytes, c->response_bytes, cudaMemcpyDeviceToHost, c->stream));
  B200_CUDA(cudaStreamSynchronize(c->stream));
  if (c->profile == 1) c->prof_collect();
  B200_CUDA(cudaGetLastError());
}

int coalesced_query(b200pir_ctx* c, b200pir_db* db, b200pir_pp* pp, const uint64_t* query_ct, const uint8_t* query_bytes,
                    uint8_t* out) {
  b200pir_ctx::Pending me;
  me.db = db; me.pp = pp; me.query_ct = query_ct; me.query_bytes = query_bytes; me.out = out;
  std::unique_lock<std::mutex> lk(c->qmu);
  c->pending.push_back(&me);
  c->qcv.notify_all();
  while (!me.done) {
    if (c->leader_active) { c->qcv.wait(lk); continue; }
    c->leader_active = true;
    if (c->coalesce_window_us > 0 && c->last_batch > 1 && c->pending.size() < std::min(c->last_batch, b200pir_ctx::kPassQueries)) {
      const auto now = std::chrono::steady_clock::now();
      if (now - c->last_batch_end < std::chrono::milliseconds(1)) {
        const size_t want = std::min(c->last_batch, b200pir_ctx::kPassQueries);
        c->qcv.wait_until(lk, now + std::chrono::microseconds(c->coalesce_window_us), [&] { return c->pending.size() >= want; });
      }
    }
    std::vector<b200pir_ctx::Pending*> batch;
    b200pir_db* bdb = c->pending.front()->db;
    size_t avail = 0;
    for (auto* p : c->pending) avail += p->db == bdb;
    size_t take = std::min(avail, b200pir_ctx::kCoalesceMax);
    if (take > b200pir_ctx::kPassQueries) take -= take % b200pir_ctx::kPassQueries;
    for (auto it = c->pending.begin(); it != c->pending.end() && batch.size() < take;) {
      if ((*it)->db == bdb) { batch.push_back(*it); it = c->pending.erase(it); } else ++it;
    }
    lk.unlock();
    int rc = 0;
    std::string err;
    try {
      std::vector<b200pir_pp*> pps; std::vector<const uint64_t*> cts; std::vector<const uint8_t*> bys; std::vector<uint8_t*> outs;
      for (auto* p : batch) { pps.push_back(p->pp); cts.push_back(p->query_ct); bys.push_back(p->query_bytes); outs.push_back(p->out); }
      process_multi(c, bdb, pps.data(), cts.data(), bys.data(), batch.size(), outs.data());
    } catch (const std::exception& e) { rc = fail(e); err = e.what(); }
    lk.lock();
    c->coalesced_batches++; c->coalesced_queries += batch.size();
    c->last_batch = batch.size();
    c->last_batch_end = std::chrono::steady_clock::now();
    for (auto* p : batch) { p->rc = rc; p->err = err; p->done = true; }
    c->leader_active = false;
    c->qcv.notify_all();
  }
  if (me.rc) g_last_error = me.err;
  return me.rc;
}
}

int b200pir_process_queries(b200pir_ctx* c, b200pir_db* db, b200pir_pp* const* pps, const uint64_t* const* query_cts, size_t count,
                            uint8_t* const* outs) {
  API_BEGIN
  if (!c || !pps || !query_cts || !outs) throw Error(B200PIR_E_BADARG, "null argument");
  for (size_t i = 0; i < count; i++)
    if (!pps[i] || !query_cts[i] || !outs[i]) throw Error(B200PIR_E_BADARG, "null entry");
  if (count == 0) return 0;
  process_multi(c, db, pps, query_cts, nullptr, count, outs);
  API_END
}
int b200pir_coalesce_stats(b200pir_ctx* c, uint64_t* batches, uint64_t* queries) {
  API_BEGIN
  if (!c) throw Error(B200PIR_E_BADARG, "null ctx");
  std::lock_guard<std::mutex> lk(c->qmu);
  if (batches) *batches = c->coalesced_batches;
  if (queries) *queries = c->coalesced_queries;
  API_END
}

int b200pir_process_query_bytes(b200pir_ctx* c, b200pir_db* db, b200pir_pp* pp, const uint8_t* queries, size_t len,
                                size_t count, uint8_t* out, size_t* out_len_each) {
  API_BEGIN
  if (!c || !out || !queries) throw Error(B200PIR_E_BADARG, "null argument");
  if (len != count * c->query_bytes) throw Error(B200PIR_E_SHAPE, "queries: expected " + std::to_string(count * c->query_bytes) + " bytes");
  if (count == 1 && c->coalesce && c->hp.expand_queries && db && pp) {
    const int rc = coalesced_query(c, db, pp, nullptr, queries, out);
    if (rc == 0 && out_len_each) *out_len_each = c->response_bytes;
    return rc;
  }
  Guard gd(c);
  check_db(c, db);
  check_pp(c, pp);
  if (db->shard.count != 1) throw Error(B200PIR_E_BADARG, "sharded database: use the stage_a / stage_b entry points");
  if (count == 0) return 0;
  c->ensure_workspace(count, db->rows);
  c->prof_reset();
  if (c->hp.expand_queries) {
    deserialize_queries(c, queries, count, c->w_query.p);
    run_query_batch_resident(c, db, pp, count, c->w_resp.p);
  } else {
    for (size_t i = 0; i < count; i++) deserialize_query_direct(c, queries + i * c->query_bytes, i);
    run_first_dim_and_fold(c, db, count);
    run_pack_encode(c, pp, c->folded, c->folded_stride, count, c->w_resp.p);
  }
  B200_CUDA(cudaMemcpyAsync(out, c->w_resp.p, count * c->response_bytes, cudaMemcpyDeviceToHost, c->stream));
  B200_CUDA(cudaStreamSynchronize(c->stream));
  if (c->profile == 1) c->prof_collect();
  if (out_len_each) *out_len_each = c->response_bytes;
  B200_CUDA(cudaGetLastError());
  API_END
}

int b200pir_process_query(b200pir_ctx* c, b200pir_db* db, b200pir_pp* pp, const uint64_t* query_ct, const uint64_t* v_buf,
                          const uint64_t* v_ct, uint8_t* out, size_t* out_len) {
  if (!c) { g_last_error = "null ctx"; return B200PIR_E_BADARG; }
  if (c->hp.expand_queries) {
    if (!query_ct || !out || !db || !pp) { g_last_error = "null argument"; return B200PIR_E_BADARG; }
    if (!c->coalesce) return b200pir_process_query_batch(c, db, pp, query_ct, 1, out, out_len);
    const int rc = coalesced_query(c, db, pp, query_ct, nullptr, out);
    if (rc == 0 && out_len) *out_len = c->response_bytes;
    return rc;
  }
  API_BEGIN
  if (!v_buf || (!v_ct && c->hp.nu_2) || !out) throw Error(B200PIR_E_BADARG, "null argument");
  Guard gd(c);
  check_db(c, db);
  check_pp(c, pp);
  if (db->shard.count != 1) throw Error(B200PIR_E_BADARG, "sharded database: use the stage_a / stage_b entry points");
  c->ensure_workspace(1, db->rows);
  c->prof_reset();
  DevBuf<uint64_t> vq((size_t)c->dim0 * 2 * POLY);
  B200_CUDA(cudaMemcpyAsync(vq.p, v_buf, vq.n * 8, cudaMemcpyHostToDevice, c->stream));
  launch_query_to_dev(c->geom(db->rows), c->w_qdev.p, vq.p, c->stream);
  const size_t npolys = (size_t)c->hp.nu_2 * 2 * 2 * c->hp.t_gsw;
  DevBuf<uint64_t> raw(std::max<size_t>(npolys, 1) * POLY);
  if (npolys) {
    B200_CUDA(cudaMemcpyAsync(raw.p, v_ct, npolys * POLY * 8, cudaMemcpyHostToDevice, c->stream));
    launch_to_ntt(c->dp, c->w_vfold.p, raw.p, npolys, c->stream);
  }
  run_prepare(c, pp, 1);
  run_first_dim_and_fold(c, db, 1);
  run_pack_encode(c, pp, c->folded, c->folded_stride, 1, c->w_resp.p);
  B200_CUDA(cudaMemcpyAsync(out, c->w_resp.p, c->response_bytes, cudaMemcpyDeviceToHost, c->stream));
  B200_CUDA(cudaStreamSynchronize(c->stream));
  if (c->profile == 1) c->prof_collect();
  if (out_len) *out_len = c->response_bytes;
  B200_CUDA(cudaGetLastError());
  API_END
}

int b200pir_expand_queries_dev(b200pir_ctx* c, b200pir_pp* pp, const uint64_t* query_cts_dev, size_t count,
                               void* q_expanded_dev, uint32_t* v_folding_dev) {
  API_BEGIN
  if (!c || !query_cts_dev || !q_expanded_dev || (!v_folding_dev && c->hp.nu_2)) throw Error(B200PIR_E_BADARG, "null argument");
  Guard gd(c);
  check_pp(c, pp);
  if (!c->hp.expand_queries) throw Error(B200PIR_E_BADARG, "needs expand_queries");
  if (count == 0) return 0;
  c->w_v.ensure(count * c->v_words());
  c->prof_reset();
  {
    b200pir_ctx::Scope sc(c, ST_EXPAND);
    run_expand_query(c, pp, query_cts_dev, c->w_v.p, (uint4*)q_expanded_dev, v_folding_dev, (int)count);
  }
  B200_CUDA(cudaGetLastError());
  API_END
}
int b200pir_first_dim_fold_dev(b200pir_ctx* c, b200pir_db* db, const void* q_expanded_dev, const uint32_t* v_folding_dev,
                               size_t count, uint32_t* partial_dev) {
  API_BEGIN
  if (!c || !q_expanded_dev || !partial_dev || (!v_folding_dev && c->hp.nu_2)) throw Error(B200PIR_E_BADARG, "null argument");
  Guard gd(c);
  check_db(c, db);
  if (count == 0) return 0;
  c->ensure_workspace_lite(count, db->rows);
  run_first_dim_and_fold(c, db, count, (const uint4*)q_expanded_dev, v_folding_dev);
  B200_CUDA(cudaMemcpy2DAsync(partial_dev, 4 * POLY * 4, c->folded, c->folded_stride * 4, 4 * POLY * 4, count * c->slices,
                              cudaMemcpyDeviceToDevice, c->stream));
  B200_CUDA(cudaGetLastError());
  API_END
}
size_t b200pir_query_image_bytes(b200pir_ctx* c) { return c ? tc5_query_bytes(make_tc5_geom(c->dim0, 32)) : 0; }
int b200pir_expand_queries_images_dev(b200pir_ctx* c, b200pir_pp* pp, const uint64_t* query_cts_dev, size_t count, void* image_dev,
                                      uint32_t* v_folding_dev) {
  API_BEGIN
  if (!c || !query_cts_dev || !image_dev || (!v_folding_dev && c->hp.nu_2)) throw Error(B200PIR_E_BADARG, "null argument");
  Guard gd(c);
  check_pp(c, pp);
  if (!c->hp.expand_queries) throw Error(B200PIR_E_BADARG, "needs expand_queries");
  if (count == 0 || count > 16) throw Error(B200PIR_E_SHAPE, "one image holds 1..16 queries");
  if (!tc5_supported(make_tc5_geom(c->dim0, 32))) throw Error(B200PIR_E_UNSUPPORTED, "dim0 too large for the wgmma kernel");
  c->w_v.ensure(count * c->v_words());
  c->prof_reset();
  {
    b200pir_ctx::Scope sc(c, ST_EXPAND);
    run_expand_query(c, pp, query_cts_dev, c->w_v.p, nullptr, v_folding_dev, (int)count, (uint8_t*)image_dev);
  }
  B200_CUDA(cudaGetLastError());
  API_END
}
int b200pir_first_dim_fold_images_dev(b200pir_ctx* c, b200pir_db* db, const void* images_dev, size_t groups, size_t per_group,
                                      const uint32_t* v_folding_dev, uint32_t* partial_dev) {
  API_BEGIN
  if (!c || !images_dev || !partial_dev || (!v_folding_dev && c->hp.nu_2)) throw Error(B200PIR_E_BADARG, "null argument");
  Guard gd(c);
  check_db(c, db);
  if (db->format != 2) throw Error(B200PIR_E_BADARG, "tile images need a wgmma-layout database (db_format 2)");
  if (per_group == 0 || per_group > 16) throw Error(B200PIR_E_SHAPE, "one image holds 1..16 queries");
  const size_t count = groups * per_group;
  if (count == 0) return 0;
  c->ensure_workspace_lite(count, db->rows);
  run_first_dim_and_fold(c, db, count, nullptr, v_folding_dev, (const uint8_t*)images_dev, per_group);
  B200_CUDA(cudaMemcpy2DAsync(partial_dev, 4 * POLY * 4, c->folded, c->folded_stride * 4, 4 * POLY * 4, count * c->slices,
                              cudaMemcpyDeviceToDevice, c->stream));
  B200_CUDA(cudaGetLastError());
  API_END
}
// ... 320 lines not shown
```

sdk_b200/csrc/kernels.h:

```cpp
#pragma once
#include "common.cuh"
#include "item_place.cuh"

namespace b200pir {

extern thread_local unsigned long long g_kernel_launches;

void opt_in_smem_impl(const void* kernel, int bytes);
template <typename K>
inline void opt_in_smem(K* kernel, int bytes) { opt_in_smem_impl(reinterpret_cast<const void*>(kernel), bytes); }

void launch_ntt_u64(const DevParams& P, uint64_t* polys, size_t count, bool inverse, cudaStream_t s);
void launch_ntt32(const DevParams& P, uint32_t* polys, size_t count, bool inverse, cudaStream_t s);
void launch_ntt32_4k(uint32_t q0, uint32_t q1, const Twiddle* tw, uint32_t* polys, size_t count, bool inverse, cudaStream_t s);
void launch_to_ntt(const DevParams& P, uint32_t* out, const uint64_t* raw, size_t count, cudaStream_t s);
void launch_to_ntt_strided(const DevParams& P, uint32_t* out, size_t out_stride, const uint64_t* raw, size_t raw_stride,
                           size_t count, int batches, cudaStream_t s);
void launch_chacha_first_rows(uint64_t* raw, const uint8_t seed[32], uint64_t word0, uint32_t n_mats, uint32_t row_words,
                              uint64_t mat_words, uint64_t modulus, cudaStream_t s);
void launch_direct_query_to_dev(uint4* q_dev, const uint32_t* sig_ntt, const uint64_t* wire_words, int dim0, cudaStream_t s);
void launch_from_ntt(const DevParams& P, uint64_t* out_raw, const uint32_t* in, size_t count, cudaStream_t s);
void launch_raw_to_res(const DevParams& P, uint32_t* out, const uint64_t* raw, size_t polys, cudaStream_t s);
void launch_res_to_raw(const DevParams& P, uint64_t* out, const uint32_t* res, size_t polys, cudaStream_t s);
void upload_poly_constants(const Twiddle* lo );
void upload_mul_constants(const Twiddle* lo );
void launch_widen(uint64_t* out, const uint32_t* in, size_t words, cudaStream_t s);
void launch_narrow(uint32_t* out, const uint64_t* in, size_t words, cudaStream_t s);

void launch_multiply(const DevParams& P, const MulGeom& G, const uint4* db_dev, const uint4* q_dev, uint32_t* out,
                     int slice_begin, int slice_count, int nq, size_t q_stride, size_t out_stride, int variant,
                     cudaStream_t s);
void launch_query_to_dev(const MulGeom& G, uint4* q_dev, const uint64_t* v_firstdim, cudaStream_t s);
struct Shard { int index, count; };
void launch_db_retile_chunk(const MulGeom& G, Shard sh, uint4* db_dev_slice, const uint64_t* ref_chunk, int z0, int zc,
                            cudaStream_t s);
void launch_db_upsert(const MulGeom& G, uint4* db_dev, int slice, int il, int j, const uint64_t* poly, cudaStream_t s);
void launch_db_synth(const DevParams& P, const MulGeom& G, Shard sh, uint4* db_dev, uint64_t seed, uint64_t pt_modulus,
                     int slice_begin, int slice_count, cudaStream_t s);

size_t imma_db_cells(const ImmaGeom& F, int slices);
size_t imma_query_cells(const ImmaGeom& F);
bool imma_supports_16(const ImmaGeom& F);
inline int imma_query_tiles(int nq) { return nq > 8 ? 4 : (nq > 4 ? 2 : 1); }
void upload_imma_constants(const Twiddle* lo);
void launch_db_to_frag(const ImmaGeom& F, const uint4* db0_slice, uint4* dbf, int slice, cudaStream_t s);
void launch_db_upsert_frag(const ImmaGeom& F, uint4* dbf, int slice, int il, int j, const uint64_t* poly, cudaStream_t s);
void launch_query_to_frag(const ImmaGeom& F, const uint4* q_dev, size_t q_stride, int nq, uint2* qf, cudaStream_t s);
void launch_multiply_imma(const DevParams& P, const ImmaGeom& F, const uint4* dbf, const uint2* qf, uint32_t* out_zm,
                          size_t out_stride, int nq, int slice_begin, int slice_count, int variant, cudaStream_t s);
void launch_intt_from_zmajor(const DevParams& P, const ImmaGeom& F, const uint32_t* in_zm, size_t in_stride, uint32_t* out,
                             int nq, int slices, int variant, cudaStream_t s);
void launch_zmajor_to_ntt32(const ImmaGeom& F, const uint32_t* in_zm, uint32_t* out, int slice, cudaStream_t s);

size_t tc5_db_bytes(const Tc5Geom& T, int slices);
size_t tc5_query_bytes(const Tc5Geom& T);
bool tc5_supported(const Tc5Geom& T);
void launch_db_to_tc5(const Tc5Geom& T, const uint4* db0_slice, uint8_t* dbt, int slice, cudaStream_t s);
void launch_db_upsert_tc5(const Tc5Geom& T, uint8_t* dbt, int slice, int il, int j, const uint64_t* poly, cudaStream_t s);
void launch_query_to_tc5(const Tc5Geom& T, const uint4* q_dev, size_t q_stride, int nq, uint8_t* qt, cudaStream_t s);
void launch_reorient_to_tc5(const Tc5Geom& T, const uint32_t* v, size_t v_stride, int idx_factor, int nq, uint8_t* qt, cudaStream_t s);
void launch_multiply_tc5(const DevParams& P, const Tc5Geom& T, const uint8_t* dbt, const uint32_t* tile_mask, const uint8_t* qt,
                         uint32_t* out_zm, size_t out_stride, int nq, int slice_begin, int slice_count, int sm_count, cudaStream_t s);

struct DbDst {
  int format;
  MulGeom G; ImmaGeom F; Tc5Geom T;
  uint4* d; uint4* f; uint8_t* t;
};
struct ItemWrite { uint32_t off, len, il, j; };
void launch_write_items(const DevParams& P, const DbDst& D, const uint8_t* bytes, const ItemWrite* items, int count, int chunks,
                        int bpc, uint64_t pt_modulus, cudaStream_t s);
void launch_db_export(const DbDst& D, int slice, int z0, int zc, uint64_t* out, cudaStream_t s);

void launch_fold_round(const DevParams& P, uint64_t* cts, size_t batch, size_t batch_stride , int half,
                       const uint32_t* c_pos, const uint32_t* c_neg, size_t c_batch_stride ,
                       int slices_per_query, int t_gsw, int bits, cudaStream_t s);
void launch_fold_res(const DevParams& P, const uint32_t* in, uint32_t* out, size_t batch, size_t batch_stride ,
                     int half, const uint32_t* c_pos, size_t c_batch_stride, int slices_per_query, int t_gsw, int bits,
                     uint32_t* zero_flags , cudaStream_t s);
void launch_folding_neg(const DevParams& P, uint32_t* out, const uint32_t* v_folding, int count, int t_gsw, int bits,
                        cudaStream_t s);

void launch_expand_scalar(const DevParams& P, uint32_t* v, size_t v_stride, int nq, int num_in, const uint32_t* neg1_r,
                          cudaStream_t s);
struct PpTable { const uint32_t* const* pack; const uint32_t* const* left; const uint32_t* const* right; const uint32_t* const* conv; };
struct ExpandRound {
  int r, num_in, stop_round, max_bits_to_gen_right, t_auto;
  const uint32_t* const* tab_left;
  const uint32_t* const* tab_right;
  size_t off_left, off_right;
  int t_left, t_right, bits_left, bits_right;
  int fill_skipped;
};
void launch_expand_round(const DevParams& P, uint32_t* v, size_t v_stride, int nq, const ExpandRound& R, cudaStream_t s);
void launch_expand_round_pair(const DevParams& P, uint32_t* v, size_t v_stride, int nq, const ExpandRound& R,
                              const uint32_t* neg1_r, cudaStream_t s);
void launch_expand_round_res(const DevParams& P, uint32_t* v, size_t v_stride, uint32_t* xr, size_t xr_stride, int nq,
                             const ExpandRound& R, const uint32_t* neg1_r, cudaStream_t s);
void launch_reorient(const MulGeom& G, uint4* q_dev, size_t q_stride, const uint32_t* v, size_t v_stride, int nq,
                     int idx_factor, cudaStream_t s);
void launch_regev_to_gsw(const DevParams& P, uint32_t* v_gsw, size_t gsw_stride, const uint32_t* v, size_t v_stride,
                         int nq, int count, int idx_factor, int idx_offset, const uint32_t* const* tab_conv, int t_gsw,
                         int t_conv, int bits_conv, cudaStream_t s);

void launch_pack(const DevParams& P, uint64_t* out_raw, size_t out_q_stride, const uint32_t* folded, size_t ct_stride,
                 size_t in_q_stride, int nq, const uint32_t* const* tab_pack, int n, int instances, int t_conv, int bits_conv,
                 int version, cudaStream_t s, const uint64_t* raw_cts = nullptr);
void launch_encode(const DevParams& P, uint8_t* out, size_t out_bytes, const uint64_t* packed_raw, size_t packed_q_stride,
                   int nq, int n, int instances, uint64_t q2, int q2_bits, uint64_t q1, int q1_bits, cudaStream_t s);

void launch_dpir_matvec(uint32_t* out, const uint32_t* a, const uint32_t* b, size_t rows, size_t cols, int variant,
                        cudaStream_t s);

void launch_dpir_mul_transposed(uint32_t* out, const uint32_t* a, const uint32_t* b, size_t a_rows, size_t a_cols,
                                size_t b_rows, size_t b_cols, cudaStream_t s);
void launch_dpir_transpose_expand(uint32_t* out, const uint32_t* a, size_t rows, size_t cols, uint64_t modulus, size_t delta,
                                  size_t concat, size_t out_rows, size_t out_cols, cudaStream_t s);

void launch_dpir_gemm(uint32_t* c, const uint32_t* a, const uint32_t* b, size_t rows, size_t k_dim, size_t n_cols, cudaStream_t s);
void launch_dpir_transpose_expand_concat(uint32_t* out, const uint32_t* h, size_t l, size_t n, uint32_t p, int delta, size_t x,
                                         cudaStream_t s);
void launch_dpir_add_squish(uint32_t* out, const uint32_t* m, size_t rows, size_t cols, uint32_t add, cudaStream_t s);
void launch_dpir_pad_transpose(uint32_t* out, const uint32_t* a, size_t rows, size_t cols, size_t rows3, cudaStream_t s);

}
```

sdk_b200/csrc/poly_kernels.cu:

```cuda
#include "kernels.h"
#include "ntt_core4096.cuh"

namespace b200pir {

namespace {

constexpr int CTA = 512;
constexpr int HI_TW = NTT_N - 64;

__constant__ Twiddle c_tw_lo[2][3][64];

struct TwConst {
  int n, dir;
  __device__ __forceinline__ Twiddle operator()(int i) const { return c_tw_lo[n][dir][i]; }
  __device__ __forceinline__ void load2(int i, Twiddle (&t)[2]) const { t[0] = (*this)(i); t[1] = (*this)(i + 1); }
  __device__ __forceinline__ void load4(int i, Twiddle (&t)[4]) const {
    t[0] = (*this)(i); t[1] = (*this)(i + 1); t[2] = (*this)(i + 2); t[3] = (*this)(i + 3);
  }
};
struct TwShared {
  const Twiddle* p;
  __device__ __forceinline__ Twiddle operator()(int i) const { return p[i - 64]; }
  __device__ __forceinline__ void load2(int i, Twiddle (&t)[2]) const {
    uint4 v = *reinterpret_cast<const uint4*>(p + (i - 64));
    t[0] = Twiddle{v.x, v.y}; t[1] = Twiddle{v.z, v.w};
  }
  __device__ __forceinline__ void load4(int i, Twiddle (&t)[4]) const {
    uint4 v = *reinterpret_cast<const uint4*>(p + (i - 64)), w = *(reinterpret_cast<const uint4*>(p + (i - 64)) + 1);
    t[0] = Twiddle{v.x, v.y}; t[1] = Twiddle{v.z, v.w}; t[2] = Twiddle{w.x, w.y}; t[3] = Twiddle{w.z, w.w};
  }
};
struct TwGlobal {
  const Twiddle* p;
  __device__ __forceinline__ Twiddle operator()(int i) const {
    uint2 v = __ldg(reinterpret_cast<const uint2*>(p + i));
    return Twiddle{v.x, v.y};
  }
  __device__ __forceinline__ void load2(int i, Twiddle (&t)[2]) const {
    uint4 v = __ldg(reinterpret_cast<const uint4*>(p + i));
    t[0] = Twiddle{v.x, v.y}; t[1] = Twiddle{v.z, v.w};
  }
  __device__ __forceinline__ void load4(int i, Twiddle (&t)[4]) const {
    uint4 v = __ldg(reinterpret_cast<const uint4*>(p + i)), w = __ldg(reinterpret_cast<const uint4*>(p + i) + 1);
    t[0] = Twiddle{v.x, v.y}; t[1] = Twiddle{v.z, v.w}; t[2] = Twiddle{w.x, w.y}; t[3] = Twiddle{w.z, w.w};
  }
};

struct Grp {
  int tid;
  int n;
  uint32_t q;
  uint64_t cr1;
  const Twiddle* fwd;
  const Twiddle* inv;
  const Twiddle* inv_lz;
  uint32_t* smem;
  uint32_t* smem2;
  const Twiddle* fwd_hi_sm;
};
struct CtaSync {
  __device__ __forceinline__ void operator()() const { __syncthreads(); }
};

__device__ __forceinline__ Grp make_grp(const DevParams& P, uint32_t* ntt_smem) {
  Grp g;
  g.n = threadIdx.x >> 8;
  g.tid = threadIdx.x & 255;
  g.q = g.n ? P.q[1] : P.q[0];
  g.cr1 = g.n ? P.cr1[1] : P.cr1[0];
  g.fwd = g.n ? P.fwd[1] : P.fwd[0];
  g.inv = g.n ? P.inv[1] : P.inv[0];
  g.inv_lz = g.n ? P.inv_lz[1] : P.inv_lz[0];
  g.smem = ntt_smem + g.n * NTT_SMEM_WORDS;
  g.smem2 = nullptr;
  g.fwd_hi_sm = nullptr;
  return g;
}
__device__ __forceinline__ Grp make_grp_single(const DevParams& P, uint32_t* ntt_smem, int n) {
  Grp g;
  g.n = n;
  g.tid = threadIdx.x;
  g.q = n ? P.q[1] : P.q[0];
  g.cr1 = n ? P.cr1[1] : P.cr1[0];
  g.fwd = n ? P.fwd[1] : P.fwd[0];
  g.inv = n ? P.inv[1] : P.inv[0];
  g.inv_lz = n ? P.inv_lz[1] : P.inv_lz[0];
  g.smem = ntt_smem;
  g.smem2 = nullptr;
  g.fwd_hi_sm = nullptr;
  return g;
}
__device__ __forceinline__ void stage_fwd_twiddles(Grp& g, Twiddle* dst) {
  for (int i = g.tid; i < HI_TW; i += 256) {
    uint2 v = __ldg(reinterpret_cast<const uint2*>(g.fwd + 64 + i));
    dst[i] = Twiddle{v.x, v.y};
  }
  g.fwd_hi_sm = dst;
}
template <bool SM>
__device__ __forceinline__ void grp_ntt_fwd(const Grp& g, uint32_t (&x)[8]) {
  if (SM) ntt_forward_group_lz<NTT_OUT_CANON, true>(g.tid, x, g.smem, TwConst{g.n, 0}, TwShared{g.fwd_hi_sm}, g.q, CtaSync());
  else ntt_forward_group_lz<NTT_OUT_CANON, true>(g.tid, x, g.smem, TwConst{g.n, 0}, TwGlobal{g.fwd}, g.q, CtaSync());
}
__device__ __forceinline__ void grp_ntt_inv(const Grp& g, uint32_t (&x)[8]) {
  ntt_inverse_group_nh(g.tid, x, g.smem, TwConst{g.n, 2}, TwGlobal{g.inv_lz}, g.q, CtaSync());
}

__device__ __forceinline__ void ld8(uint32_t (&x)[8], const uint32_t* p) {
  uint4 a = *reinterpret_cast<const uint4*>(p), b = *reinterpret_cast<const uint4*>(p + 4);
  x[0] = a.x; x[1] = a.y; x[2] = a.z; x[3] = a.w; x[4] = b.x; x[5] = b.y; x[6] = b.z; x[7] = b.w;
}
__device__ __forceinline__ void ld8_ro(uint32_t (&x)[8], const uint32_t* p) {
  uint4 a = __ldg(reinterpret_cast<const uint4*>(p)), b = __ldg(reinterpret_cast<const uint4*>(p + 4));
  x[0] = a.x; x[1] = a.y; x[2] = a.z; x[3] = a.w; x[4] = b.x; x[5] = b.y; x[6] = b.z; x[7] = b.w;
}
__device__ __forceinline__ void st8(uint32_t* p, const uint32_t (&x)[8]) {
  *reinterpret_cast<uint4*>(p) = make_uint4(x[0], x[1], x[2], x[3]);
  *reinterpret_cast<uint4*>(p + 4) = make_uint4(x[4], x[5], x[6], x[7]);
}

template <int ROWS>
__device__ __forceinline__ void acc_reduce(uint64_t (&acc)[ROWS][8], const Grp& g) {
#pragma unroll
  for (int r = 0; r < ROWS; r++)
#pragma unroll
    for (int k = 0; k < 8; k++) acc[r][k] = barrett64(acc[r][k], g.cr1, g.q);
}

template <bool BYTE>
__device__ __forceinline__ uint32_t gadget_digit_fast(uint64_t v, int k, int bits, uint64_t mask) {
  if (BYTE) return __byte_perm((uint32_t)v, (uint32_t)(v >> 32), 0x7770u | (uint32_t)k);
  return gadget_digit(v, k, bits, mask);
}

struct RegCoef {
  const uint64_t (&v)[8];
  __device__ __forceinline__ uint64_t operator()(int a) const { return v[a]; }
};
struct SmemCoef {
  const uint64_t* p;
  __device__ __forceinline__ uint64_t operator()(int a) const { return p[a * 256]; }
};

template <int ROWS, bool SM, bool BYTE, typename Coef>
__device__ __forceinline__ void digits_mac_impl(uint64_t (&acc)[ROWS][8], int& cnt, Coef v, int ndig,
                                                int bits, const uint32_t* c0, size_t col_step, size_t row_step,
                                                const Grp& g) {
  const uint64_t mask = (1ull << bits) - 1;
  int k = 0;
  if (SM) {
#pragma unroll 1
    for (; k + 1 < ndig; k += 2) {
      uint32_t x0[8], x1[8];
#pragma unroll
      for (int a = 0; a < 8; a++) {
        const uint64_t va = v(a);
        x0[a] = gadget_digit_fast<BYTE>(va, k, bits, mask);
        x1[a] = gadget_digit_fast<BYTE>(va, k + 1, bits, mask);
      }
      ntt_forward_group2_lz<NTT_OUT_LAZY16>(g.tid, x0, x1, g.smem, g.smem2, TwConst{g.n, 0}, TwShared{g.fwd_hi_sm}, g.q, CtaSync());
      if (cnt + 2 > 16) { acc_reduce<ROWS>(acc, g); cnt = 1; }
      cnt += 2;
      const uint32_t* c = c0 + (size_t)k * col_step;
#pragma unroll
      for (int r = 0; r < ROWS; r++) {
        uint32_t cv[8];
        ld8_ro(cv, c + (size_t)r * row_step);
#pragma unroll
        for (int e = 0; e < 8; e++) acc[r][e] += (uint64_t)x0[e] * cv[e];
      }
#pragma unroll
      for (int r = 0; r < ROWS; r++) {
        uint32_t cv[8];
        ld8_ro(cv, c + col_step + (size_t)r * row_step);
#pragma unroll
        for (int e = 0; e < 8; e++) acc[r][e] += (uint64_t)x1[e] * cv[e];
      }
    }
  }
#pragma unroll 1
  for (; k < ndig; k++) {
    uint32_t x[8];
#pragma unroll
    for (int a = 0; a < 8; a++) x[a] = gadget_digit_fast<BYTE>(v(a), k, bits, mask);
    if (SM) ntt_forward_group_lz<NTT_OUT_LAZY16>(g.tid, x, g.smem, TwConst{g.n, 0}, TwShared{g.fwd_hi_sm}, g.q, CtaSync());
    else ntt_forward_group_lz<NTT_OUT_LAZY16>(g.tid, x, g.smem, TwConst{g.n, 0}, TwGlobal{g.fwd}, g.q, CtaSync());
    if (cnt + 1 > 16) { acc_reduce<ROWS>(acc, g); cnt = 1; }
    cnt += 1;
    const uint32_t* c = c0 + (size_t)k * col_step;
#pragma unroll
    for (int r = 0; r < ROWS; r++) {
      uint32_t cv[8];
      ld8_ro(cv, c + (size_t)r * row_step);
#pragma unroll
      for (int e = 0; e < 8; e++) acc[r][e] += (uint64_t)x[e] * cv[e];
    }
  }
}

template <int ROWS, bool SM, typename Coef>
__device__ __forceinline__ void digits_mac(uint64_t (&acc)[ROWS][8], int& cnt, Coef v, int ndig,
                                           int bits, const uint32_t* c0, size_t col_step, size_t row_step,
                                           const Grp& g) {
  if (bits == 8) digits_mac_impl<ROWS, SM, true>(acc, cnt, v, ndig, bits, c0, col_step, row_step, g);
  else digits_mac_impl<ROWS, SM, false>(acc, cnt, v, ndig, bits, c0, col_step, row_step, g);
}

template <typename Sink>
__device__ __forceinline__ void crt_lift(const uint32_t (&x)[8], uint32_t* res, const Grp& g, const DevParams& P,
                                         Sink sink) {
  __syncthreads();
#pragma unroll
  for (int a = 0; a < 8; a++) res[g.n * POLY + a * 256 + g.tid] = x[a];
  __syncthreads();
#pragma unroll
  for (int a4 = 0; a4 < 4; a4++) {
    int z = (g.n * 4 + a4) * 256 + g.tid;
    sink(z, crt_compose(res[z], res[POLY + z], P));
  }
}

__global__ void __launch_bounds__(256) k_ntt32(DevParams P, uint32_t* polys, int inverse) {
  __shared__ __align__(16) uint32_t ntt_smem[NTT_SMEM_WORDS];
  Grp g = make_grp_single(P, ntt_smem, blockIdx.y);
  uint32_t* p = polys + ((size_t)blockIdx.x * 2 + g.n) * POLY;
  uint32_t x[8];
  if (!inverse) {
#pragma unroll
    for (int a = 0; a < 8; a++) x[a] = p[a * 256 + g.tid];
    grp_ntt_fwd<false>(g, x);
    st8(p + g.tid * 8, x);
  } else {
    ld8(x, p + g.tid * 8);
    grp_ntt_inv(g, x);
#pragma unroll
    for (int a = 0; a < 8; a++) p[a * 256 + g.tid] = x[a];
  }
}
__global__ void __launch_bounds__(NTT4K_THREADS)
k_ntt32_4k(uint32_t q0, uint32_t q1, const Twiddle* __restrict__ tw , uint32_t* polys, int inverse) {
  __shared__ __align__(16) uint32_t sm[NTT4K_SMEM_WORDS];
  const int n = blockIdx.y, tid = threadIdx.x;
  const uint32_t q = n ? q1 : q0;
  uint32_t* p = polys + ((size_t)blockIdx.x * 2 + n) * NTT4K_N;
  const TwGlobal tab{tw + (size_t)(2 * n + (inverse ? 1 : 0)) * NTT4K_N};
  uint32_t x[8];
  if (!inverse) {
#pragma unroll
    for (int a = 0; a < 8; a++) x[a] = p[a * NTT4K_THREADS + tid];
    ntt4k_forward_group(tid, x, sm, tab, q, CtaSync());
    st8(p + tid * 8, x);
  } else {
    ld8(x, p + tid * 8);
    ntt4k_inverse_group(tid, x, sm, tab, q, CtaSync());
#pragma unroll
    for (int a = 0; a < 8; a++) p[a * NTT4K_THREADS + tid] = x[a];
  }
}
__global__ void __launch_bounds__(256) k_ntt_u64(DevParams P, uint64_t* polys, int inverse) {
  __shared__ __align__(16) uint32_t ntt_smem[NTT_SMEM_WORDS];
  Grp g = make_grp_single(P, ntt_smem, blockIdx.y);
  uint64_t* p = polys + ((size_t)blockIdx.x * 2 + g.n) * POLY;
  uint32_t x[8];
  if (!inverse) {
#pragma unroll
    for (int a = 0; a < 8; a++) x[a] = (uint32_t)p[a * 256 + g.tid];
    grp_ntt_fwd<false>(g, x);
#pragma unroll
    for (int k = 0; k < 8; k++) p[g.tid * 8 + k] = x[k];
  } else {
#pragma unroll
    for (int k = 0; k < 8; k++) x[k] = (uint32_t)p[g.tid * 8 + k];
    grp_ntt_inv(g, x);
#pragma unroll
    for (int a = 0; a < 8; a++) p[a * 256 + g.tid] = x[a];
  }
}
__global__ void __launch_bounds__(256) k_to_ntt(DevParams P, uint32_t* out, const uint64_t* raw, size_t out_stride,
                                                size_t raw_stride) {
  __shared__ __align__(16) uint32_t ntt_smem[NTT_SMEM_WORDS];
  Grp g = make_grp_single(P, ntt_smem, blockIdx.y);
  out += (size_t)blockIdx.z * out_stride;
  raw += (size_t)blockIdx.z * raw_stride;
  const uint64_t* src = raw + (size_t)blockIdx.x * POLY;
  uint32_t x[8];
#pragma unroll
  for (int a = 0; a < 8; a++) x[a] = barrett64(src[a * 256 + g.tid], g.cr1, g.q);
  grp_ntt_fwd<false>(g, x);
  st8(out + ((size_t)blockIdx.x * 2 + g.n) * POLY + g.tid * 8, x);
}
__global__ void k_raw_to_res(DevParams P, uint32_t* out, const uint64_t* raw, size_t polys) {
  size_t idx = (size_t)blockIdx.x * blockDim.x + threadIdx.x;
  if (idx >= polys * POLY) return;
  size_t poly = idx / POLY;
  int z = (int)(idx % POLY);
  uint64_t v = raw[idx];
  out[(poly * 2 + 0) * POLY + z] = barrett64(v, P.cr1[0], P.q[0]);
  out[(poly * 2 + 1) * POLY + z] = barrett64(v, P.cr1[1], P.q[1]);
}
__global__ void k_res_to_raw(DevParams P, uint64_t* out, const uint32_t* res, size_t polys) {
  size_t idx = (size_t)blockIdx.x * blockDim.x + threadIdx.x;
  if (idx >= polys * POLY) return;
  size_t poly = idx / POLY;
  int z = (int)(idx % POLY);
  out[idx] = crt_compose(res[(poly * 2 + 0) * POLY + z], res[(poly * 2 + 1) * POLY + z], P);
}
__global__ void __launch_bounds__(CTA) k_from_ntt(DevParams P, uint64_t* out, const uint32_t* in) {
  __shared__ __align__(16) uint32_t ntt_smem[2 * NTT_SMEM_WORDS];
  __shared__ uint32_t res[2 * POLY];
  Grp g = make_grp(P, ntt_smem);
  uint32_t x[8];
  ld8(x, in + ((size_t)blockIdx.x * 2 + g.n) * POLY + g.tid * 8);
  grp_ntt_inv(g, x);
  uint64_t* dst = out + (size_t)blockIdx.x * POLY;
  crt_lift(x, res, g, P, [&](int z, uint64_t v) { dst[z] = v; });
}
__global__ void k_widen(uint64_t* out, const uint32_t* in, size_t words) {
  size_t i = (size_t)blockIdx.x * blockDim.x + threadIdx.x;
  if (i < words) out[i] = in[i];
}
__global__ void k_narrow(uint32_t* out, const uint64_t* in, size_t words) {
  size_t i = (size_t)blockIdx.x * blockDim.x + threadIdx.x;
  if (i < words) out[i] = (uint32_t)in[i];
}

__global__ void __launch_bounds__(CTA, 1)
k_fold_round(DevParams P, uint64_t* cts, size_t batch_stride, int half, const uint32_t* c_pos, const uint32_t* c_neg,
             size_t c_batch_stride, int slices_per_query, int t_gsw, int bits) {
  __shared__ __align__(16) uint32_t ntt_smem[2 * NTT_SMEM_WORDS];
  __shared__ uint32_t res[2 * POLY];
  Grp g = make_grp(P, ntt_smem);
  const int b = blockIdx.x / half, i = blockIdx.x % half;
  uint64_t* base = cts + (size_t)b * batch_stride;
  const size_t qoff = (size_t)(b / slices_per_query) * c_batch_stride;
  const int cols = 2 * t_gsw;
  const size_t col_step = (size_t)2 * 2 * POLY;
  const size_t row_step = (size_t)cols * 2 * POLY;

  uint64_t acc[2][8];
#pragma unroll
  for (int r = 0; r < 2; r++)
#pragma unroll
    for (int e = 0; e < 8; e++) acc[r][e] = 0;
  int cnt = 0;
#pragma unroll 1
  for (int src = 0; src < 2; src++) {
    const uint64_t* ct = base + (size_t)(src == 0 ? i : half + i) * 2 * POLY;
    const uint32_t* C = (src == 0 ? c_neg : c_pos) + qoff;
#pragma unroll 1
    for (int rho = 0; rho < 2; rho++) {
      uint64_t v[8];
#pragma unroll
      for (int a = 0; a < 8; a++) v[a] = ct[rho * POLY + a * 256 + g.tid];
      const uint32_t* c0 = C + ((size_t)rho * 2 + g.n) * POLY + g.tid * 8;
      digits_mac<2, false>(acc, cnt, RegCoef{v}, t_gsw, bits, c0, col_step, row_step, g);
    }
  }
  uint64_t* dst = base + (size_t)i * 2 * POLY;
#pragma unroll 1
  for (int r = 0; r < 2; r++) {
    uint32_t x[8];
#pragma unroll
    for (int e = 0; e < 8; e++) x[e] = barrett64(acc[r][e], g.cr1, g.q);
    grp_ntt_inv(g, x);
    uint64_t* d = dst + r * POLY;
    crt_lift(x, res, g, P, [&](int z, uint64_t val) { d[z] = val; });
  }
}

__device__ __forceinline__ uint32_t digit_diff(uint64_t vh, uint64_t vi, int k, int bits, uint64_t mask, uint32_t q) {
  return gadget_digit(vh, k, bits, mask) - gadget_digit(vi, k, bits, mask) + q;
}
__device__ __forceinline__ uint32_t byte_pair_diff(uint64_t vh, uint64_t vi, int k) {
  const uint32_t sel = 0x7070u | ((uint32_t)(k + 1) << 8) | (uint32_t)k;
  return __byte_perm((uint32_t)vh, (uint32_t)(vh >> 32), sel) + 0x01000100u -
         __byte_perm((uint32_t)vi, (uint32_t)(vi >> 32), sel);
}
constexpr int kFoldPlanes = 4;

template <bool BYTE>
__global__ void __launch_bounds__(256, 2)
k_fold_res_lz(DevParams P, const uint32_t* __restrict__ in, uint32_t* __restrict__ out, size_t batch_stride, int half,
              const uint32_t* __restrict__ c_pos, size_t c_batch_stride, int slices_per_query, int t_gsw, int bits,
              const uint32_t* __restrict__ zero_flags ) {
  if (zero_flags) {
    const int bz = blockIdx.x / half, iz = blockIdx.x % half;
    const uint32_t fa = zero_flags[(size_t)bz * 2 * half + iz], fb = zero_flags[(size_t)bz * 2 * half + half + iz];
    if (fa | fb) {
      const uint32_t* src = in + (size_t)bz * batch_stride + (size_t)((fa ? half : 0) + iz) * 4 * POLY;
      uint32_t* dst = out + (size_t)bz * batch_stride + (size_t)iz * 4 * POLY;
#pragma unroll
      for (int rho = 0; rho < 2; rho++) {
        uint32_t x[8];
        ld8_ro(x, src + ((size_t)rho * 2 + blockIdx.y) * POLY + threadIdx.x * 8);
        st8(dst + ((size_t)rho * 2 + blockIdx.y) * POLY + threadIdx.x * 8, x);
      }
      return;
    }
  }
  extern __shared__ __align__(16) uint8_t dyn_smem[];
  uint32_t* sm0 = reinterpret_cast<uint32_t*>(dyn_smem);
  uint32_t* sm1 = sm0 + NTT_SMEM_WORDS;
  Twiddle* tw = reinterpret_cast<Twiddle*>(sm1 + NTT_SMEM_WORDS);
  Grp g = make_grp_single(P, sm0, blockIdx.y);
  stage_fwd_twiddles(g, tw);
  const TwConst lo{g.n, 0};
  const TwShared hi{tw};
  const int b = blockIdx.x / half, i = blockIdx.x % half;
  const uint32_t* ci = in + (size_t)b * batch_stride + (size_t)i * 4 * POLY;
  const uint32_t* ch = in + (size_t)b * batch_stride + (size_t)(half + i) * 4 * POLY;
  const uint32_t* C = c_pos + (size_t)(b / slices_per_query) * c_batch_stride;
  const int cols = 2 * t_gsw;
  const size_t row_step = (size_t)cols * 2 * POLY;
  const uint64_t mask = (1ull << bits) - 1;
  const uint32_t q = g.q;
  uint32_t* planes = reinterpret_cast<uint32_t*>(tw + HI_TW) + g.tid;

  uint64_t acc[2][8];
#pragma unroll
  for (int r = 0; r < 2; r++)
#pragma unroll
    for (int e = 0; e < 8; e++) acc[r][e] = 0;
  int cnt = 0;
#pragma unroll 1
  for (int rho = 0; rho < 2; rho++) {
    uint64_t vi[8], vh[8];
#pragma unroll
    for (int a = 0; a < 8; a++) {
      const int z = a * 256 + g.tid;
      vi[a] = crt_compose(__ldg(ci + (rho * 2 + 0) * POLY + z), __ldg(ci + (rho * 2 + 1) * POLY + z), P);
      vh[a] = crt_compose(__ldg(ch + (rho * 2 + 0) * POLY + z), __ldg(ch + (rho * 2 + 1) * POLY + z), P);
      if (BYTE) {
#pragma unroll
        for (int p = 0; p < kFoldPlanes; p++)
          if (2 * p < t_gsw) planes[p * POLY + a * 256] = byte_pair_diff(vh[a], vi[a], 2 * p);
      }
    }
    const uint32_t* c0 = C + ((size_t)rho * 2 + g.n) * POLY + g.tid * 8;
    int k = 0;
#pragma unroll 1
    for (; k + 1 < t_gsw; k += 2) {
      uint32_t x0[8], x1[8];
#pragma unroll
      for (int a = 0; a < 8; a++) {
        if (BYTE) {
          const uint32_t w = planes[(k >> 1) * POLY + a * 256];
          x0[a] = (w & 0xffffu) + (q - 256u);
          x1[a] = (w >> 16) + (q - 256u);
        } else {
          x0[a] = digit_diff(vh[a], vi[a], k, bits, mask, q);
          x1[a] = digit_diff(vh[a], vi[a], k + 1, bits, mask, q);
        }
      }
      ntt_forward_group2_lz<NTT_OUT_LAZY16>(g.tid, x0, x1, sm0, sm1, lo, hi, q, CtaSync());
      if (cnt + 2 > 16) { acc_reduce<2>(acc, g); cnt = 1; }
      cnt += 2;
#pragma unroll
      for (int r = 0; r < 2; r++) {
        uint32_t cv[8];
        ld8_ro(cv, c0 + (size_t)r * row_step + (size_t)k * 4 * POLY);
#pragma unroll
        for (int e = 0; e < 8; e++) acc[r][e] += (uint64_t)x0[e] * cv[e];
      }
#pragma unroll
      for (int r = 0; r < 2; r++) {
        uint32_t cv[8];
        ld8_ro(cv, c0 + (size_t)r * row_step + (size_t)(k + 1) * 4 * POLY);
#pragma unroll
        for (int e = 0; e < 8; e++) acc[r][e] += (uint64_t)x1[e] * cv[e];
      }
    }
    if (k < t_gsw) {
      uint32_t x0[8];
#pragma unroll
      for (int a = 0; a < 8; a++)
        x0[a] = BYTE ? (planes[(k >> 1) * POLY + a * 256] & 0xffffu) + (q - 256u) : digit_diff(vh[a], vi[a], k, bits, mask, q);
      ntt_forward_group_lz<NTT_OUT_LAZY16>(g.tid, x0, sm0, lo, hi, q, CtaSync());
      if (cnt + 1 > 16) { acc_reduce<2>(acc, g); cnt = 1; }
      cnt += 1;
#pragma unroll
      for (int r = 0; r < 2; r++) {
        uint32_t cv[8];
        ld8_ro(cv, c0 + (size_t)r * row_step + (size_t)k * 4 * POLY);
#pragma unroll
        for (int e = 0; e < 8; e++) acc[r][e] += (uint64_t)x0[e] * cv[e];
      }
    }
  }
  uint32_t y0[8], y1[8];
#pragma unroll
  for (int e = 0; e < 8; e++) {
    y0[e] = barrett64(acc[0][e], g.cr1, q);
    y1[e] = barrett64(acc[1][e], g.cr1, q);
  }
  ntt_inverse_group2_nh(g.tid, y0, y1, sm0, sm1, TwConst{g.n, 2}, TwGlobal{g.inv_lz}, q, CtaSync());
  uint32_t* co = out + (size_t)b * batch_stride + (size_t)i * 4 * POLY;
#pragma unroll
  for (int a = 0; a < 8; a++) {
    const int z = a * 256 + g.tid;
    co[(0 * 2 + g.n) * POLY + z] = addmod(y0[a], __ldg(ci + (0 * 2 + g.n) * POLY + z), q);
    co[(1 * 2 + g.n) * POLY + z] = addmod(y1[a], __ldg(ci + (1 * 2 + g.n) * POLY + z), q);
  }
}

__global__ void __launch_bounds__(256)
k_ct_zero_flags(const uint32_t* __restrict__ cts, size_t batch_stride, int per_batch, uint32_t* __restrict__ flags) {
  const int b = blockIdx.x / per_batch, idx = blockIdx.x % per_batch;
  const uint4* p = reinterpret_cast<const uint4*>(cts + (size_t)b * batch_stride + (size_t)idx * 4 * POLY);
  uint32_t acc = 0;
#pragma unroll
  for (int k = 0; k < 8; k++) {
    const uint4 v = __ldg(p + k * 256 + threadIdx.x);
    acc |= v.x | v.y | v.z | v.w;
  }
  const int any = __syncthreads_or(acc != 0);
  if (threadIdx.x == 0) flags[blockIdx.x] = any ? 0u : 1u;
}

__global__ void k_folding_neg(DevParams P, uint32_t* out, const uint32_t* vf, size_t total, int t_gsw, int bits) {
  size_t idx = (size_t)blockIdx.x * blockDim.x + threadIdx.x;
  if (idx >= total) return;
  int n = (int)((idx / POLY) & 1);
  size_t poly = idx / (2 * POLY);
  int cols = 2 * t_gsw;
  int c = (int)(poly % cols);
  int r = (int)((poly / cols) & 1);
  uint32_t q = P.q[n];
  uint32_t v = vf[idx];
  uint32_t neg = v == 0 ? 0u : q - v;
  uint32_t gval = 0;
  if ((c & 1) == r) {
    int j = c >> 1;
    if (bits * j < 64) gval = barrett64(1ull << (bits * j), P.cr1[n], q);
  }
  out[idx] = addmod(neg, gval, q);
}

__global__ void k_expand_scalar(DevParams P, uint32_t* v, size_t v_stride, int num_in, const uint32_t* neg1) {
  v += (size_t)blockIdx.y * v_stride;
  size_t idx = (size_t)blockIdx.x * blockDim.x + threadIdx.x;
  size_t total = (size_t)num_in * 4 * POLY;
  if (idx >= total) return;
  int z = (int)(idx % POLY);
  int n = (int)((idx / POLY) & 1);
  uint32_t a = v[idx], b = neg1[n * POLY + z];
  v[total + idx] = barrett64((uint64_t)a * b, P.cr1[n], P.q[n]);
}

__global__ void __launch_bounds__(CTA, 1) k_expand_round(DevParams P, uint32_t* v, size_t v_stride, ExpandRound R) {
  v += (size_t)blockIdx.y * v_stride;
  extern __shared__ __align__(16) uint8_t dyn_smem[];
  uint32_t* ntt_smem = reinterpret_cast<uint32_t*>(dyn_smem);
  uint32_t* res = ntt_smem + 4 * NTT_SMEM_WORDS;
  uint64_t* autom = reinterpret_cast<uint64_t*>(res + 2 * POLY);
  Twiddle* tw = reinterpret_cast<Twiddle*>(autom + 2 * POLY);
  Grp g = make_grp(P, ntt_smem);
  g.smem2 = ntt_smem + (2 + g.n) * NTT_SMEM_WORDS;

  const int i = blockIdx.x;
  const int ih = i < R.num_in ? i : i - R.num_in;
  if ((R.stop_round > 0 && R.r > R.stop_round && (ih & 1)) ||
      (R.stop_round > 0 && R.r == R.stop_round && (ih & 1) && (ih / 2) >= R.max_bits_to_gen_right))
    return;
  const bool left = (R.r != 0) && ((ih & 1) == 0);
  const uint32_t* W = left ? R.tab_left[blockIdx.y] + R.off_left : R.tab_right[blockIdx.y] + R.off_right;
  const int t_exp = left ? R.t_left : R.t_right;
  const int bits = left ? R.bits_left : R.bits_right;

  stage_fwd_twiddles(g, tw + g.n * HI_TW);
  uint32_t* vi = v + (size_t)i * 4 * POLY;
  {
    uint32_t x[8];
    ld8(x, vi + (size_t)g.n * POLY + g.tid * 8);
    grp_ntt_inv(g, x);
    const int t_auto = R.t_auto;
    const uint64_t Q = P.modulus;
    crt_lift(x, res, g, P, [&](int z, uint64_t val) {
      unsigned prod = (unsigned)z * (unsigned)t_auto;
      unsigned num = prod >> NTT_LOG_N, rem = prod & (POLY - 1);
      autom[rem] = (num & 1u) ? Q - val : val;
    });
  }
  __syncthreads();
  uint64_t acc[2][8];
#pragma unroll
  for (int r = 0; r < 2; r++)
#pragma unroll
    for (int e = 0; e < 8; e++) acc[r][e] = 0;
  int cnt = 0;
  digits_mac<2, true>(acc, cnt, SmemCoef{autom + g.tid}, t_exp, bits, W + (size_t)g.n * POLY + g.tid * 8, (size_t)2 * POLY,
                      (size_t)t_exp * 2 * POLY, g);
  uint32_t y[8];
  {
    const uint32_t* row1 = vi + ((size_t)2 + g.n) * POLY;
#pragma unroll
    for (int k = 0; k < 8; k++) {
      const unsigned sidx = (unsigned)(g.tid * 8 + k);
      const unsigned e = 2u * (__brev(sidx) >> (32 - NTT_LOG_N)) + 1u;
      const unsigned e2 = (e * (unsigned)R.t_auto) & (2u * POLY - 1u);
      const unsigned src = __brev((e2 - 1u) >> 1) >> (32 - NTT_LOG_N);
      y[k] = row1[src];
    }
  }
  __syncthreads();
#pragma unroll
  for (int rho = 0; rho < 2; rho++) {
    uint32_t o[8];
    ld8(o, vi + ((size_t)rho * 2 + g.n) * POLY + g.tid * 8);
#pragma unroll
    for (int e = 0; e < 8; e++) {
      uint32_t s = addmod(o[e], barrett64(acc[rho][e], g.cr1, g.q), g.q);
      o[e] = rho ? addmod(s, y[e], g.q) : s;
    }
    st8(vi + ((size_t)rho * 2 + g.n) * POLY + g.tid * 8, o);
  }
}

__global__ void __launch_bounds__(CTA, 1)
k_expand_round_pair(DevParams P, uint32_t* v, size_t v_stride, ExpandRound R, const uint32_t* __restrict__ neg1) {
  v += (size_t)blockIdx.y * v_stride;
  extern __shared__ __align__(16) uint8_t dyn_smem[];
  uint32_t* ntt_smem = reinterpret_cast<uint32_t*>(dyn_smem);
  uint32_t* res = ntt_smem + 4 * NTT_SMEM_WORDS;
  uint64_t* autom = reinterpret_cast<uint64_t*>(res + 2 * POLY);
  Twiddle* tw = reinterpret_cast<Twiddle*>(autom + 2 * POLY);
  Grp g = make_grp(P, ntt_smem);
  g.smem2 = ntt_smem + (2 + g.n) * NTT_SMEM_WORDS;

  const int i = blockIdx.x;
  if ((R.stop_round > 0 && R.r > R.stop_round && (i & 1)) ||
      (R.stop_round > 0 && R.r == R.stop_round && (i & 1) && (i / 2) >= R.max_bits_to_gen_right)) {
    if (R.fill_skipped) {
      const int n = threadIdx.x >> 8, tid = threadIdx.x & 255;
      const uint32_t qn = n ? P.q[1] : P.q[0];
      const uint64_t cr1 = n ? P.cr1[1] : P.cr1[0];
      uint32_t nn[8];
      ld8_ro(nn, neg1 + (size_t)n * POLY + tid * 8);
#pragma unroll
      for (int rho = 0; rho < 2; rho++) {
        uint32_t x[8];
        ld8(x, v + ((size_t)i * 4 + rho * 2 + n) * POLY + tid * 8);
#pragma unroll
        for (int e = 0; e < 8; e++) x[e] = barrett64((uint64_t)x[e] * nn[e], cr1, qn);
        st8(v + ((size_t)(i + R.num_in) * 4 + rho * 2 + n) * POLY + tid * 8, x);
      }
    }
    return;
  }
  const bool left = (R.r != 0) && ((i & 1) == 0);
  const uint32_t* W = left ? R.tab_left[blockIdx.y] + R.off_left : R.tab_right[blockIdx.y] + R.off_right;
  const int t_exp = left ? R.t_left : R.t_right;
  const int bits = left ? R.bits_left : R.bits_right;

  stage_fwd_twiddles(g, tw + g.n * HI_TW);
  uint32_t* vi = v + (size_t)i * 4 * POLY;
  uint32_t* vo = v + (size_t)(i + R.num_in) * 4 * POLY;
  const uint32_t* ng = neg1 + (size_t)g.n * POLY;
  uint32_t keep[2][8], y[8];
  {
    uint32_t x[8];
    ld8(x, vi + (size_t)g.n * POLY + g.tid * 8);
#pragma unroll
    for (int e = 0; e < 8; e++) keep[0][e] = x[e];
    grp_ntt_inv(g, x);
    __syncthreads();
#pragma unroll
    for (int a = 0; a < 8; a++) res[g.n * POLY + a * 256 + g.tid] = x[a];
  }
  const uint32_t* row1 = vi + ((size_t)2 + g.n) * POLY;
  ld8(keep[1], row1 + g.tid * 8);
#pragma unroll
  for (int k = 0; k < 8; k++) {
    const unsigned sidx = (unsigned)(g.tid * 8 + k);
    const unsigned e = 2u * (__brev(sidx) >> (32 - NTT_LOG_N)) + 1u;
    const unsigned e2 = (e * (unsigned)R.t_auto) & (2u * POLY - 1u);
    const unsigned src = __brev((e2 - 1u) >> 1) >> (32 - NTT_LOG_N);
    y[k] = row1[src];
  }
  __syncthreads();
  const uint64_t Q = P.modulus;
  const uint32_t q0 = P.q[0], q1 = P.q[1];
#pragma unroll 1
  for (int half = 1; half >= 0; half--) {
    const int shift = half ? R.num_in : 0;
#pragma unroll
    for (int a4 = 0; a4 < 4; a4++) {
      const int k = (g.n * 4 + a4) * 256 + g.tid;
      const int zs = (k + shift) & (POLY - 1);
      uint32_t a0 = res[zs], a1 = res[POLY + zs];
      if (k + shift >= POLY) {
        a0 = a0 ? q0 - a0 : 0u;
        a1 = a1 ? q1 - a1 : 0u;
      }
      const uint64_t val = crt_compose(a0, a1, P);
      const unsigned prod = (unsigned)k * (unsigned)R.t_auto;
      const unsigned num = prod >> NTT_LOG_N, rem = prod & (POLY - 1);
      autom[rem] = (num & 1u) ? Q - val : val;
    }
    __syncthreads();
    uint64_t acc[2][8];
#pragma unroll
    for (int r = 0; r < 2; r++)
#pragma unroll
      for (int e = 0; e < 8; e++) acc[r][e] = 0;
    int cnt = 0;
    digits_mac<2, true>(acc, cnt, SmemCoef{autom + g.tid}, t_exp, bits, W + (size_t)g.n * POLY + g.tid * 8, (size_t)2 * POLY,
                        (size_t)t_exp * 2 * POLY, g);
    uint32_t* dst = half ? vo : vi;
#pragma unroll
    for (int rho = 0; rho < 2; rho++) {
      uint32_t o[8], nn[8];
      if (half) ld8_ro(nn, ng + g.tid * 8);
#pragma unroll
      for (int e = 0; e < 8; e++) {
        uint32_t base = keep[rho][e];
        if (half) base = barrett64((uint64_t)base * nn[e], g.cr1, g.q);
        uint32_t s = addmod(base, barrett64(acc[rho][e], g.cr1, g.q), g.q);
        if (rho) {
          uint32_t yy = y[e];
          if (half) {
            const unsigned sidx = (unsigned)(g.tid * 8 + e);
            const unsigned ee = 2u * (__brev(sidx) >> (32 - NTT_LOG_N)) + 1u;
            const unsigned e2 = (ee * (unsigned)R.t_auto) & (2u * POLY - 1u);
            const unsigned src = __brev((e2 - 1u) >> 1) >> (32 - NTT_LOG_N);
            yy = barrett64((uint64_t)yy * __ldg(ng + src), g.cr1, g.q);
          }
          s = addmod(s, yy, g.q);
        }
        o[e] = s;
      }
      st8(dst + ((size_t)rho * 2 + g.n) * POLY + g.tid * 8, o);
    }
    __syncthreads();
  }
}

__global__ void __launch_bounds__(256)
k_expand_intt(DevParams P, const uint32_t* __restrict__ v, size_t v_stride, uint32_t* __restrict__ xr, size_t xr_stride,
              ExpandRound R) {
  __shared__ __align__(16) uint32_t ntt_smem[NTT_SMEM_WORDS];
  const int i = blockIdx.x;
  if ((R.stop_round > 0 && R.r > R.stop_round && (i & 1)) ||
      (R.stop_round > 0 && R.r == R.stop_round && (i & 1) && (i / 2) >= R.max_bits_to_gen_right))
    return;
  Grp g = make_grp_single(P, ntt_smem, blockIdx.y);
  const uint32_t* src = v + (size_t)blockIdx.z * v_stride + ((size_t)i * 4 + g.n) * POLY;
  uint32_t x[8];
  ld8_ro(x, src + g.tid * 8);
  grp_ntt_inv(g, x);
  uint32_t* dst = xr + (size_t)blockIdx.z * xr_stride + ((size_t)i * 2 + g.n) * POLY;
#pragma unroll
  for (int a = 0; a < 8; a++) dst[a * 256 + g.tid] = x[a];
}

__global__ void __launch_bounds__(256, 2)
k_expand_round_res(DevParams P, uint32_t* v, size_t v_stride, const uint32_t* __restrict__ xr, size_t xr_stride,
                   ExpandRound R, const uint32_t* __restrict__ neg1) {
  v += (size_t)blockIdx.z * v_stride;
  xr += (size_t)blockIdx.z * xr_stride;
  extern __shared__ __align__(16) uint8_t dyn_smem[];
  uint32_t* sm0 = reinterpret_cast<uint32_t*>(dyn_smem);
  uint32_t* sm1 = sm0 + NTT_SMEM_WORDS;
  uint64_t* autom = reinterpret_cast<uint64_t*>(sm1 + NTT_SMEM_WORDS);
  Twiddle* tw = reinterpret_cast<Twiddle*>(autom + POLY);
  Grp g = make_grp_single(P, sm0, blockIdx.y);
  g.smem2 = sm1;
  const int i = blockIdx.x;
  const uint32_t* ng = neg1 + (size_t)g.n * POLY;
  uint32_t* vi = v + (size_t)i * 4 * POLY;
  uint32_t* vo = v + (size_t)(i + R.num_in) * 4 * POLY;
  if ((R.stop_round > 0 && R.r > R.stop_round && (i & 1)) ||
      (R.stop_round > 0 && R.r == R.stop_round && (i & 1) && (i / 2) >= R.max_bits_to_gen_right)) {
    if (R.fill_skipped) {
      uint32_t nn[8];
      ld8_ro(nn, ng + g.tid * 8);
#pragma unroll
      for (int rho = 0; rho < 2; rho++) {
        uint32_t x[8];
        ld8(x, vi + ((size_t)rho * 2 + g.n) * POLY + g.tid * 8);
#pragma unroll
        for (int e = 0; e < 8; e++) x[e] = barrett64((uint64_t)x[e] * nn[e], g.cr1, g.q);
        st8(vo + ((size_t)rho * 2 + g.n) * POLY + g.tid * 8, x);
      }
    }
    return;
  }
  const bool left = (R.r != 0) && ((i & 1) == 0);
  const uint32_t* W = left ? R.tab_left[blockIdx.z] + R.off_left : R.tab_right[blockIdx.z] + R.off_right;
  const int t_exp = left ? R.t_left : R.t_right;
  const int bits = left ? R.bits_left : R.bits_right;
  stage_fwd_twiddles(g, tw);
  const uint32_t* x0r = xr + (size_t)i * 2 * POLY;
  const uint32_t* x1r = x0r + POLY;
  const uint32_t* row1 = vi + ((size_t)2 + g.n) * POLY;
  const uint64_t Q = P.modulus;
  const uint32_t q0 = P.q[0], q1 = P.q[1];
#pragma unroll 1
  for (int half = 1; half >= 0; half--) {
    const int shift = half ? R.num_in : 0;
#pragma unroll
    for (int a = 0; a < 8; a++) {
      const int k = a * 256 + g.tid;
      const int zs = (k + shift) & (POLY - 1);
      uint32_t a0 = __ldg(x0r + zs), a1 = __ldg(x1r + zs);
      if (k + shift >= POLY) {
        a0 = a0 ? q0 - a0 : 0u;
        a1 = a1 ? q1 - a1 : 0u;
      }
      const uint64_t val = crt_compose(a0, a1, P);
      const unsigned prod = (unsigned)k * (unsigned)R.t_auto;
      const unsigned num = prod >> NTT_LOG_N, rem = prod & (POLY - 1);
      autom[rem] = (num & 1u) ? Q - val : val;
    }
    __syncthreads();
    uint64_t acc[2][8];
#pragma unroll
    for (int r = 0; r < 2; r++)
#pragma unroll
      for (int e = 0; e < 8; e++) acc[r][e] = 0;
    int cnt = 0;
    digits_mac<2, true>(acc, cnt, SmemCoef{autom + g.tid}, t_exp, bits, W + (size_t)g.n * POLY + g.tid * 8, (size_t)2 * POLY,
                        (size_t)t_exp * 2 * POLY, g);
    uint32_t yy[8];
#pragma unroll
    for (int e = 0; e < 8; e++) {
      const unsigned sidx = (unsigned)(g.tid * 8 + e);
      const unsigned ee = 2u * (__brev(sidx) >> (32 - NTT_LOG_N)) + 1u;
      const unsigned e2 = (ee * (unsigned)R.t_auto) & (2u * POLY - 1u);
      const unsigned src = __brev((e2 - 1u) >> 1) >> (32 - NTT_LOG_N);
      uint32_t t = row1[src];
      if (half) t = barrett64((uint64_t)t * __ldg(ng + src), g.cr1, g.q);
      yy[e] = t;
    }
    __syncthreads();
    uint32_t* dst = half ? vo : vi;
    uint32_t nn[8];
    if (half) ld8_ro(nn, ng + g.tid * 8);
#pragma unroll
    for (int rho = 0; rho < 2; rho++) {
      uint32_t o[8];
      ld8(o, vi + ((size_t)rho * 2 + g.n) * POLY + g.tid * 8);
#pragma unroll
      for (int e = 0; e < 8; e++) {
        uint32_t base = o[e];
        if (half) base = barrett64((uint64_t)base * nn[e], g.cr1, g.q);
        uint32_t s = addmod(base, barrett64(acc[rho][e], g.cr1, g.q), g.q);
        o[e] = rho ? addmod(s, yy[e], g.q) : s;
      }
      st8(dst + ((size_t)rho * 2 + g.n) * POLY + g.tid * 8, o);
    }
  }
}

__global__ void k_reorient(MulGeom G, uint4* q_dev, size_t q_stride, const uint32_t* v, size_t v_stride, int idx_factor) {
  q_dev += (size_t)blockIdx.y * q_stride;
  v += (size_t)blockIdx.y * v_stride;
  size_t idx = (size_t)blockIdx.x * blockDim.x + threadIdx.x;
  if (idx >= (size_t)G.dim0 * POLY) return;
  int z = (int)(idx % POLY), j = (int)(idx / POLY);
  const uint32_t* ct = v + (size_t)idx_factor * j * 4 * POLY;
  uint4 o = make_uint4(ct[z], ct[POLY + z], ct[2 * POLY + z], ct[3 * POLY + z]);
  q_dev[((size_t)(j >> 1) * 2 + (j & 1)) * POLY + z] = o;
}

__global__ void __launch_bounds__(CTA, 1)
k_regev_to_gsw(DevParams P, uint32_t* v_gsw, size_t gsw_stride, const uint32_t* v, size_t v_stride, int idx_factor,
               int idx_offset, const uint32_t* const* tab_conv, int t_gsw, int t_conv, int bits_conv) {
  const uint32_t* v_conv = tab_conv[blockIdx.y];
  v_gsw += (size_t)blockIdx.y * gsw_stride;
  v += (size_t)blockIdx.y * v_stride;
  extern __shared__ __align__(16) uint8_t dyn_smem[];
  uint32_t* ntt_smem = reinterpret_cast<uint32_t*>(dyn_smem);
  uint32_t* res = ntt_smem + 4 * NTT_SMEM_WORDS;
  uint64_t* raw = reinterpret_cast<uint64_t*>(res + 2 * POLY);
  Twiddle* tw = reinterpret_cast<Twiddle*>(raw + 2 * POLY);
  Grp g = make_grp(P, ntt_smem);
  g.smem2 = ntt_smem + (2 + g.n) * NTT_SMEM_WORDS;
  stage_fwd_twiddles(g, tw + g.n * HI_TW);
  const int i = blockIdx.x / t_gsw, j = blockIdx.x % t_gsw;
  const int idx_inp = idx_factor * (i * t_gsw + j) + idx_offset;
  const uint32_t* inp = v + (size_t)idx_inp * 4 * POLY;
  const int cols = 2 * t_gsw;
  uint32_t* out = v_gsw + (size_t)i * 2 * cols * 2 * POLY;
#pragma unroll 1
  for (int rho = 0; rho < 2; rho++) {
    uint32_t x[8];
    ld8(x, inp + ((size_t)rho * 2 + g.n) * POLY + g.tid * 8);
    st8(out + (((size_t)rho * cols + 2 * j + 1) * 2 + g.n) * POLY + g.tid * 8, x);
    grp_ntt_inv(g, x);
    uint64_t* d = raw + rho * POLY;
    crt_lift(x, res, g, P, [&](int z, uint64_t val) { d[z] = val; });
  }
  __syncthreads();
  uint64_t acc[2][8];
#pragma unroll
  for (int r = 0; r < 2; r++)
#pragma unroll
    for (int e = 0; e < 8; e++) acc[r][e] = 0;
  int cnt = 0;
  const int ccols = 2 * t_conv;
#pragma unroll 1
  for (int rho = 0; rho < 2; rho++) {
    const uint32_t* c0 = v_conv + ((size_t)rho * 2 + g.n) * POLY + g.tid * 8;
    digits_mac<2, true>(acc, cnt, SmemCoef{raw + rho * POLY + g.tid}, t_conv, bits_conv, c0, (size_t)2 * 2 * POLY, (size_t)ccols * 2 * POLY, g);
  }
#pragma unroll
  for (int r = 0; r < 2; r++) {
    uint32_t o[8];
#pragma unroll
    for (int e = 0; e < 8; e++) o[e] = barrett64(acc[r][e], g.cr1, g.q);
    st8(out + (((size_t)r * cols + 2 * j) * 2 + g.n) * POLY + g.tid * 8, o);
  }
}

template <int ROWS>
__global__ void __launch_bounds__(CTA, 1)
k_pack(DevParams P, uint64_t* out_raw, size_t out_q_stride, const uint32_t* folded, size_t ct_stride, size_t in_q_stride,
       const uint32_t* const* tab_pack, int t_conv, int bits, int version, const uint64_t* __restrict__ raw_cts) {
  const uint32_t* v_packing = tab_pack[blockIdx.y];
  out_raw += (size_t)blockIdx.y * out_q_stride;
  folded += (size_t)blockIdx.y * in_q_stride;
  extern __shared__ __align__(16) uint8_t dyn_smem[];
  uint32_t* ntt_smem = reinterpret_cast<uint32_t*>(dyn_smem);
  uint32_t* res = ntt_smem + 4 * NTT_SMEM_WORDS;
  uint64_t* rawbuf = reinterpret_cast<uint64_t*>(res + 2 * POLY);
  Twiddle* tw = reinterpret_cast<Twiddle*>(rawbuf + 2 * POLY);
  Grp g = make_grp(P, ntt_smem);
  g.smem2 = ntt_smem + (2 + g.n) * NTT_SMEM_WORDS;
  stage_fwd_twiddles(g, tw + g.n * HI_TW);
  constexpr int n = ROWS - 1;
  const int inst = blockIdx.x / n, c = blockIdx.x % n;
  const size_t mat_words = (size_t)ROWS * t_conv * 2 * POLY;
  const size_t row_step = (size_t)t_conv * 2 * POLY, col_step = (size_t)2 * POLY;

  uint32_t vint[ROWS][8];
#pragma unroll
  for (int m = 0; m < ROWS; m++)
#pragma unroll
    for (int e = 0; e < 8; e++) vint[m][e] = 0;

#pragma unroll 1
  for (int r = 0; r < n; r++) {
    const uint32_t* ct = folded + ((size_t)inst * n * n + (size_t)r * n + c) * ct_stride;
    const uint32_t* W = v_packing + (version == 0 ? (size_t)r * mat_words : 0);
    uint64_t acc[ROWS][8];
#pragma unroll
    for (int m = 0; m < ROWS; m++)
#pragma unroll
      for (int e = 0; e < 8; e++) acc[m][e] = 0;
    int cnt = 0;
    {
      uint64_t vv[8];
      if (raw_cts) {
        const uint64_t* ct0 = raw_cts + ((size_t)inst * n * n + (size_t)r * n + c) * 2 * POLY;
#pragma unroll
        for (int a = 0; a < 8; a++) vv[a] = __ldg(ct0 + a * 256 + g.tid);
      } else {
#pragma unroll
        for (int a = 0; a < 8; a++) vv[a] = crt_compose(__ldg(ct + a * 256 + g.tid), __ldg(ct + POLY + a * 256 + g.tid), P);
      }
      digits_mac<ROWS, true>(acc, cnt, RegCoef{vv}, t_conv, bits, W + (size_t)g.n * POLY + g.tid * 8, col_step, row_step, g);
    }
    uint32_t y[8];
#pragma unroll
    for (int a = 0; a < 8; a++) y[a] = __ldg(ct + (2 + g.n) * POLY + a * 256 + g.tid);
    grp_ntt_fwd<true>(g, y);
    uint32_t prod[ROWS][8];
#pragma unroll
    for (int m = 0; m < ROWS; m++)
#pragma unroll
      for (int e = 0; e < 8; e++) prod[m][e] = barrett64(acc[m][e], g.cr1, g.q);
    if (version == 0) {
#pragma unroll
      for (int m = 0; m < ROWS; m++)
#pragma unroll
        for (int e = 0; e < 8; e++) {
          uint32_t s = addmod(vint[m][e], prod[m][e], g.q);
          vint[m][e] = (m == 1 + r) ? addmod(s, y[e], g.q) : s;
        }
    } else {
#pragma unroll
      for (int e = 0; e < 8; e++) prod[1][e] = addmod(prod[1][e], y[e], g.q);
      const uint32_t* Wshift = v_packing + mat_words;
#pragma unroll 1
      for (int sft = 0; sft < r; sft++) {
        uint32_t x[8];
#pragma unroll
        for (int e = 0; e < 8; e++) x[e] = prod[0][e];
        grp_ntt_inv(g, x);
        crt_lift(x, res, g, P, [&](int z, uint64_t val) { rawbuf[z] = val; });
        __syncthreads();
#pragma unroll
        for (int m = 0; m < ROWS; m++)
#pragma unroll
          for (int e = 0; e < 8; e++) acc[m][e] = 0;
        cnt = 0;
        digits_mac<ROWS, true>(acc, cnt, SmemCoef{rawbuf + g.tid}, t_conv, bits, Wshift + (size_t)g.n * POLY + g.tid * 8, col_step, row_step, g);
        uint32_t np[ROWS][8];
#pragma unroll
        for (int m = 0; m < ROWS; m++)
#pragma unroll
          for (int e = 0; e < 8; e++) {
            uint32_t p1 = barrett64(acc[m][e], g.cr1, g.q);
            uint32_t p2 = (m == 0) ? 0u : (m == 1 ? prod[n][e] : prod[m - 1][e]);
            np[m][e] = addmod(p1, p2, g.q);
          }
#pragma unroll
        for (int m = 0; m < ROWS; m++)
#pragma unroll
          for (int e = 0; e < 8; e++) prod[m][e] = np[m][e];
      }
#pragma unroll
      for (int m = 0; m < ROWS; m++)
#pragma unroll
        for (int e = 0; e < 8; e++) vint[m][e] = addmod(vint[m][e], prod[m][e], g.q);
    }
  }
#pragma unroll 1
  for (int m = 0; m < ROWS; m++) {
    uint32_t x[8];
#pragma unroll
    for (int e = 0; e < 8; e++) x[e] = vint[m][e];
    grp_ntt_inv(g, x);
    uint64_t* d = out_raw + (((size_t)inst * ROWS + m) * n + c) * POLY;
    crt_lift(x, res, g, P, [&](int z, uint64_t val) { d[z] = val; });
  }
}

__device__ __forceinline__ uint64_t rescale_dev(uint64_t a, uint64_t inp_mod, uint64_t out_mod) {
  typedef __int128 i128;
  long long inp_mod_i = (long long)inp_mod;
  long long inp_val = (long long)(a % inp_mod);
  if (inp_val >= inp_mod_i / 2) inp_val -= inp_mod_i;
  long long sign = inp_val >= 0 ? 1 : -1;
  i128 val = (i128)inp_val * (i128)out_mod;
  i128 result = (val + (i128)(sign * (inp_mod_i / 2))) / (i128)inp_mod;
  i128 om = (i128)out_mod;
  result = (result + (i128)((inp_mod / out_mod) * out_mod) + 2 * om) % om;
  return (uint64_t)((result + om) % om);
}
__global__ void k_encode(DevParams P, uint64_t* out, size_t out_words, const uint64_t* packed, size_t packed_q_stride, int n,
                         int instances, uint64_t q2, int q2_bits, uint64_t q1, int q1_bits) {
  size_t w = (size_t)blockIdx.x * blockDim.x + threadIdx.x;
  if (w >= out_words) return;
  out += (size_t)blockIdx.y * out_words;
  packed += (size_t)blockIdx.y * packed_q_stride;
  const uint64_t first_cnt = (uint64_t)n * POLY, rest_cnt = (uint64_t)n * n * POLY;
  const uint64_t inst_bits = first_cnt * q2_bits + rest_cnt * q1_bits;
  uint64_t lo_bit = (uint64_t)w * 64, hi_bit = lo_bit + 64;
  uint64_t word = 0;
  uint64_t bit = lo_bit;
  while (bit < hi_bit) {
    uint64_t inst = bit / inst_bits;
    if (inst >= (uint64_t)instances) break;
    uint64_t off = bit - inst * inst_bits;
    const uint64_t* pk = packed + inst * (uint64_t)(n + 1) * n * POLY;
    uint64_t vstart, val;
    int vb;
    if (off < first_cnt * q2_bits) {
      uint64_t vi = off / q2_bits;
      vstart = inst * inst_bits + vi * q2_bits;
      vb = q2_bits;
      val = rescale_dev(pk[vi], P.modulus, q2);
    } else {
      uint64_t o2 = off - first_cnt * q2_bits;
      uint64_t vi = o2 / q1_bits;
      vstart = inst * inst_bits + first_cnt * q2_bits + vi * q1_bits;
      vb = q1_bits;
      val = rescale_dev(pk[first_cnt + vi], P.modulus, q1);
    }
    val &= (vb >= 64) ? ~0ull : ((1ull << vb) - 1);
    if (vstart >= lo_bit) word |= val << (vstart - lo_bit);
    else word |= val >> (lo_bit - vstart);
    bit = vstart + vb;
  }
  out[w] = word;
}

inline unsigned grid1d(size_t total, int block) { return (unsigned)((total + block - 1) / block); }
const size_t kDynSmemBig = (size_t)(4 * NTT_SMEM_WORDS + 2 * POLY) * 4 + (size_t)2 * POLY * 8 + (size_t)2 * HI_TW * 8;
const size_t kDynSmemFold = (size_t)(2 * NTT_SMEM_WORDS) * 4 + (size_t)HI_TW * 8;

}

void upload_poly_constants(const Twiddle* lo ) {
  B200_CUDA(cudaMemcpyToSymbol(c_tw_lo, lo, sizeof(Twiddle) * 2 * 3 * 64));
}
void launch_ntt_u64(const DevParams& P, uint64_t* polys, size_t count, bool inverse, cudaStream_t s) {
  if (count) ++g_kernel_launches, k_ntt_u64<<<dim3((unsigned)count, 2), 256, 0, s>>>(P, polys, inverse ? 1 : 0);
}
void launch_ntt32(const DevParams& P, uint32_t* polys, size_t count, bool inverse, cudaStream_t s) {
  if (count) ++g_kernel_launches, k_ntt32<<<dim3((unsigned)count, 2), 256, 0, s>>>(P, polys, inverse ? 1 : 0);
}
void launch_ntt32_4k(uint32_t q0, uint32_t q1, const Twiddle* tw, uint32_t* polys, size_t count, bool inverse, cudaStream_t s) {
  if (count) ++g_kernel_launches, k_ntt32_4k<<<dim3((unsigned)count, 2), NTT4K_THREADS, 0, s>>>(q0, q1, tw, polys, inverse ? 1 : 0);
}
void launch_to_ntt(const DevParams& P, uint32_t* out, const uint64_t* raw, size_t count, cudaStream_t s) {
  if (count) ++g_kernel_launches, k_to_ntt<<<dim3((unsigned)count, 2), 256, 0, s>>>(P, out, raw, 0, 0);
}
void launch_to_ntt_strided(const DevParams& P, uint32_t* out, size_t out_stride, const uint64_t* raw, size_t raw_stride,
                           size_t count, int batches, cudaStream_t s) {
  if (count && batches)
    ++g_kernel_launches, k_to_ntt<<<dim3((unsigned)count, 2, (unsigned)batches), 256, 0, s>>>(P, out, raw, out_stride, raw_stride);
}
void launch_raw_to_res(const DevParams& P, uint32_t* out, const uint64_t* raw, size_t polys, cudaStream_t s) {
  if (polys) ++g_kernel_launches, k_raw_to_res<<<grid1d(polys * POLY, 256), 256, 0, s>>>(P, out, raw, polys);
}
void launch_res_to_raw(const DevParams& P, uint64_t* out, const uint32_t* res, size_t polys, cudaStream_t s) {
  if (polys) ++g_kernel_launches, k_res_to_raw<<<grid1d(polys * POLY, 256), 256, 0, s>>>(P, out, res, polys);
}
void launch_fold_res(const DevParams& P, const uint32_t* in, uint32_t* out, size_t batch, size_t batch_stride, int half,
                     const uint32_t* c_pos, size_t c_batch_stride, int slices_per_query, int t_gsw, int bits,
                     uint32_t* zero_flags, cudaStream_t s) {
  if (batch == 0 || half == 0) return;
  if (zero_flags) {
    ++g_kernel_launches;
    k_ct_zero_flags<<<(unsigned)(batch * 2 * half), 256, 0, s>>>(in, batch_stride, 2 * half, zero_flags);
  }
  ++g_kernel_launches;
  const dim3 grid((unsigned)(batch * half), 2);
  const bool byte = bits == 8 && t_gsw <= 2 * kFoldPlanes;
  const size_t smem = kDynSmemFold + (byte ? (size_t)kFoldPlanes * POLY * 4 : 0);
  auto kern = byte ? k_fold_res_lz<true> : k_fold_res_lz<false>;
  opt_in_smem(kern, (int)smem);
  kern<<<grid, 256, smem, s>>>(P, in, out, batch_stride, half, c_pos, c_batch_stride, slices_per_query, t_gsw, bits, zero_flags);
}
void launch_from_ntt(const DevParams& P, uint64_t* out_raw, const uint32_t* in, size_t count, cudaStream_t s) {
  if (count) ++g_kernel_launches, k_from_ntt<<<(unsigned)count, CTA, 0, s>>>(P, out_raw, in);
}
void launch_widen(uint64_t* out, const uint32_t* in, size_t words, cudaStream_t s) {
  if (words) ++g_kernel_launches, k_widen<<<grid1d(words, 256), 256, 0, s>>>(out, in, words);
}
void launch_narrow(uint32_t* out, const uint64_t* in, size_t words, cudaStream_t s) {
  if (words) ++g_kernel_launches, k_narrow<<<grid1d(words, 256), 256, 0, s>>>(out, in, words);
}
void launch_fold_round(const DevParams& P, uint64_t* cts, size_t batch, size_t batch_stride, int half,
                       const uint32_t* c_pos, const uint32_t* c_neg, size_t c_batch_stride, int slices_per_query,
                       int t_gsw, int bits, cudaStream_t s) {
  if (batch == 0 || half == 0) return;
  ++g_kernel_launches;
  k_fold_round<<<(unsigned)(batch * half), CTA, 0, s>>>(P, cts, batch_stride, half, c_pos, c_neg, c_batch_stride,
                                                        slices_per_query, t_gsw, bits);
}
void launch_folding_neg(const DevParams& P, uint32_t* out, const uint32_t* v_folding, int count, int t_gsw, int bits,
                        cudaStream_t s) {
  size_t total = (size_t)count * 2 * 2 * t_gsw * 2 * POLY;
  if (total) ++g_kernel_launches, k_folding_neg<<<grid1d(total, 256), 256, 0, s>>>(P, out, v_folding, total, t_gsw, bits);
}
void launch_expand_scalar(const DevParams& P, uint32_t* v, size_t v_stride, int nq, int num_in, const uint32_t* neg1_r,
                          cudaStream_t s) {
  size_t total = (size_t)num_in * 4 * POLY;
  ++g_kernel_launches;
  k_expand_scalar<<<dim3(grid1d(total, 256), nq), 256, 0, s>>>(P, v, v_stride, num_in, neg1_r);
}
void launch_expand_round(const DevParams& P, uint32_t* v, size_t v_stride, int nq, const ExpandRound& R, cudaStream_t s) {
  opt_in_smem(k_expand_round, (int)kDynSmemBig);
  ++g_kernel_launches;
  k_expand_round<<<dim3((unsigned)(2 * R.num_in), nq), CTA, kDynSmemBig, s>>>(P, v, v_stride, R);
}
void launch_expand_round_pair(const DevParams& P, uint32_t* v, size_t v_stride, int nq, const ExpandRound& R,
                              const uint32_t* neg1_r, cudaStream_t s) {
  opt_in_smem(k_expand_round_pair, (int)kDynSmemBig);
  ++g_kernel_launches;
  k_expand_round_pair<<<dim3((unsigned)R.num_in, nq), CTA, kDynSmemBig, s>>>(P, v, v_stride, R, neg1_r);
}
void launch_expand_round_res(const DevParams& P, uint32_t* v, size_t v_stride, uint32_t* xr, size_t xr_stride, int nq,
                             const ExpandRound& R, const uint32_t* neg1_r, cudaStream_t s) {
  const size_t smem = (size_t)2 * NTT_SMEM_WORDS * 4 + (size_t)POLY * 8 + (size_t)HI_TW * 8;
  opt_in_smem(k_expand_round_res, (int)smem);
  g_kernel_launches += 2;
  k_expand_intt<<<dim3((unsigned)R.num_in, 2, nq), 256, 0, s>>>(P, v, v_stride, xr, xr_stride, R);
  k_expand_round_res<<<dim3((unsigned)R.num_in, 2, nq), 256, smem, s>>>(P, v, v_stride, xr, xr_stride, R, neg1_r);
}
void launch_reorient(const MulGeom& G, uint4* q_dev, size_t q_stride, const uint32_t* v, size_t v_stride, int nq,
                     int idx_factor, cudaStream_t s) {
  size_t total = (size_t)G.dim0 * POLY;
  ++g_kernel_launches;
  k_reorient<<<dim3(grid1d(total, 256), nq), 256, 0, s>>>(G, q_dev, q_stride, v, v_stride, idx_factor);
}
void launch_regev_to_gsw(const DevParams& P, uint32_t* v_gsw, size_t gsw_stride, const uint32_t* v, size_t v_stride,
                         int nq, int count, int idx_factor, int idx_offset, const uint32_t* const* tab_conv, int t_gsw,
                         int t_conv, int bits_conv, cudaStream_t s) {
  if (count == 0) return;
  opt_in_smem(k_regev_to_gsw, (int)kDynSmemBig);
  ++g_kernel_launches;
  k_regev_to_gsw<<<dim3((unsigned)(count * t_gsw), nq), CTA, kDynSmemBig, s>>>(P, v_gsw, gsw_stride, v, v_stride,
                                                                               idx_factor, idx_offset, tab_conv, t_gsw,
                                                                               t_conv, bits_conv);
}
template <int ROWS>
static void launch_pack_t(const DevParams& P, uint64_t* out_raw, size_t out_q_stride, const uint32_t* folded,
                          size_t ct_stride, size_t in_q_stride, int nq, const uint32_t* const* tab_pack, int instances,
                          int t_conv, int bits_conv, int version, const uint64_t* raw_cts, cudaStream_t s) {
  opt_in_smem(k_pack<ROWS>, (int)kDynSmemBig);
  ++g_kernel_launches;
  k_pack<ROWS><<<dim3((unsigned)(instances * (ROWS - 1)), nq), CTA, kDynSmemBig, s>>>(
      P, out_raw, out_q_stride, folded, ct_stride, in_q_stride, tab_pack, t_conv, bits_conv, version, raw_cts);
}
void launch_pack(const DevParams& P, uint64_t* out_raw, size_t out_q_stride, const uint32_t* folded, size_t ct_stride,
                 size_t in_q_stride, int nq, const uint32_t* const* tab_pack, int n, int instances, int t_conv, int bits_conv,
                 int version, cudaStream_t s, const uint64_t* raw_cts) {
  if (raw_cts && nq != 1) throw Error(-2, "pack: raw ciphertexts are taken for one query");
  switch (n) {
    case 1: launch_pack_t<2>(P, out_raw, out_q_stride, folded, ct_stride, in_q_stride, nq, tab_pack, instances, t_conv, bits_conv, version, raw_cts, s); break;
    case 2: launch_pack_t<3>(P, out_raw, out_q_stride, folded, ct_stride, in_q_stride, nq, tab_pack, instances, t_conv, bits_conv, version, raw_cts, s); break;
    case 3: launch_pack_t<4>(P, out_raw, out_q_stride, folded, ct_stride, in_q_stride, nq, tab_pack, instances, t_conv, bits_conv, version, raw_cts, s); break;
    case 4: launch_pack_t<5>(P, out_raw, out_q_stride, folded, ct_stride, in_q_stride, nq, tab_pack, instances, t_conv, bits_conv, version, raw_cts, s); break;
    default: throw Error(-2, "pack: n must be 1..4");
  }
}
void launch_encode(const DevParams& P, uint8_t* out, size_t out_bytes, const uint64_t* packed_raw, size_t packed_q_stride,
                   int nq, int n, int instances, uint64_t q2, int q2_bits, uint64_t q1, int q1_bits, cudaStream_t s) {
  size_t words = out_bytes / 8;
  ++g_kernel_launches;
  k_encode<<<dim3(grid1d(words, 128), nq), 128, 0, s>>>(P, reinterpret_cast<uint64_t*>(out), words, packed_raw,
                                                        packed_q_stride, n, instances, q2, q2_bits, q1, q1_bits);
}

}
```

Measured before the change: 1214.

## Skip gadget digits above the modulus width in fold, expand, conversion and pack

Adds a live_digits helper that counts how many gadget-decomposition digits can be nonzero for a 56-bit modulus, and passes it to the fold, expansion, regev-to-GSW and pack kernels so their digit loops stop there instead of running to t. Each skipped digit saves one NTT and one multiply-accumulate. The fold kernel also moves to a 3D grid (n, half, batch), cuts the byte planes from 4 to 3, and puts an odd trailing digit into a spare shared-memory buffer that is paired across rho. The risk is correctness if the higher digits are not actually zero, and the new grid limits batch to 65535 per launch.

```diff
diff --git a/sdk_b200/build.py b/sdk_b200/build.py
--- a/sdk_b200/build.py
+++ b/sdk_b200/build.py
@@ -8,7 +8,7 @@
 SOURCES = ["api.cu", "poly_kernels.cu", "mul_kernels.cu", "imma_kernels.cu", "wire_kernels.cu", "tc5_kernels.cu", "dpir_gemm.cu",
            "export_kernels.cu"]
 HEADERS = ["common.cuh", "kernels.h", "ntt_core.cuh", "tc5_layout.cuh", "tc5_ptx.cuh", "ntt_core4096.cuh", "ntt_tables.hpp",
-           "item_place.cuh", "update_body.hpp", os.path.join("..", "..", "include", "b200pir.h")]
+           "item_place.cuh", "update_body.hpp", "gadget.hpp", os.path.join("..", "..", "include", "b200pir.h")]
 NVCC_FLAGS = ["-gencode", "arch=compute_90a,code=sm_90a", "-lineinfo", "-O3", "-std=c++17", "--extended-lambda",
               "-Xcompiler", "-fPIC", "-ccbin", "/usr/bin/g++" if os.path.exists("/usr/bin/g++") else "g++"]
 
diff --git a/sdk_b200/csrc/api.cu b/sdk_b200/csrc/api.cu
--- a/sdk_b200/csrc/api.cu
+++ b/sdk_b200/csrc/api.cu
@@ -2,6 +2,7 @@
 #include "kernels.h"
 #include "ntt_tables.hpp"
 #include "update_body.hpp"
+#include "gadget.hpp"
 #include <cstdio>
 #include <cerrno>
 #include <fcntl.h>
@@ -43,10 +44,8 @@
 using b200pir::tables::build_tables;
 using b200pir::tables::invmod;
 uint64_t log2_ceil_u64(uint64_t a) { return (uint64_t)std::ceil(std::log2((double)a)); }
-int bits_per(int t) {
-  if (t == 56) return 1;
-  return 56 / t + 1;
-}
+using b200pir::bits_per;
+using b200pir::live_digits;
 const uint64_t kQ2Values[37] = {0, 0, 0, 0, 0, 0, 0, 0, 0, 0, 0, 0, 0, 0, 12289ULL, 12289ULL, 61441ULL, 65537ULL,
                                 65537ULL, 520193ULL, 786433ULL, 786433ULL, 3604481ULL, 7340033ULL, 16515073ULL,
                                 33292289ULL, 67043329ULL, 132120577ULL, 268369921ULL, 469762049ULL, 1073479681ULL,
@@ -83,6 +82,7 @@
   b200pir_params hp;
   int dim0, num_per, slices, trials, g, stop_round, num_packing;
   int bits_gsw, bits_conv, bits_left, bits_right;
+  int live_gsw, live_conv, live_left, live_right;
   bool has_right;
   uint64_t q2, q1, setup_bytes, query_bytes, response_bytes;
   int q1_bits;
@@ -355,14 +355,14 @@
     R.r = r; R.num_in = num_in; R.stop_round = stop_round; R.max_bits_to_gen_right = max_right;
     R.fill_skipped = all_slots ? 1 : 0;
     R.t_auto = (POLY >> r) + 1;
-    R.t_left = (int)hp.t_exp_left; R.bits_left = c->bits_left;
+    R.t_left = (int)hp.t_exp_left; R.bits_left = c->bits_left; R.live_left = c->live_left;
     R.tab_left = T.left; R.off_left = (size_t)r * 2 * hp.t_exp_left * 2 * POLY;
     if (hp.nu_2 > 0 && c->has_right) {
       int rr = r <= c->stop_round ? r : c->stop_round;
-      R.t_right = (int)hp.t_exp_right; R.bits_right = c->bits_right;
+      R.t_right = (int)hp.t_exp_right; R.bits_right = c->bits_right; R.live_right = c->live_right;
       R.tab_right = T.right; R.off_right = (size_t)rr * 2 * hp.t_exp_right * 2 * POLY;
     } else {
-      R.t_right = R.t_left; R.bits_right = R.bits_left; R.tab_right = T.left; R.off_right = R.off_left;
+      R.t_right = R.t_left; R.bits_right = R.bits_left; R.live_right = R.live_left; R.tab_right = T.left; R.off_right = R.off_left;
     }
     if (pair && c->expand_variant == 0) {
       const size_t xr_stride = (size_t)num_in * 2 * POLY;
@@ -390,7 +390,7 @@
   }
   if (hp.nu_2 > 0)
     launch_regev_to_gsw(c->dp, v_fold, c->fold_words(), v, c->v_words(), nq, (int)hp.nu_2, 2, 1, c->pp_table(pp, (size_t)nq).conv,
-                        (int)hp.t_gsw, (int)hp.t_conv, c->bits_conv, s);
+                        (int)hp.t_gsw, (int)hp.t_conv, c->bits_conv, c->live_conv, s);
 }
 
 void run_fold(b200pir_ctx* c, uint64_t* cts, size_t batch, size_t batch_stride, size_t num, int k0,
@@ -416,7 +416,7 @@
   }
   for (size_t half = num / 2; half >= 1; half /= 2, k--) {
     launch_fold_res(c->dp, src, dst, batch, batch_stride, (int)half, vfold + (size_t)k * mat, c->fold_words(),
-                    slices_per_query, (int)c->hp.t_gsw, c->bits_gsw, zero_flags, c->stream);
+                    slices_per_query, (int)c->hp.t_gsw, c->bits_gsw, c->live_gsw, zero_flags, c->stream);
     std::swap(src, dst);
   }
   return src;
@@ -512,7 +512,7 @@
   {
     b200pir_ctx::Scope sc(c, ST_PACK);
     launch_pack(c->dp, c->w_packed.p, packed_words, folded, ct_stride, (size_t)c->slices * ct_stride, (int)count, c->pp_table(pp, count).pack,
-                (int)hp.n, (int)hp.instances, (int)hp.t_conv, c->bits_conv, (int)hp.version, c->stream);
+                (int)hp.n, (int)hp.instances, (int)hp.t_conv, c->bits_conv, c->live_conv, (int)hp.version, c->stream);
   }
   {
     b200pir_ctx::Scope sc(c, ST_ENCODE);
@@ -580,6 +580,10 @@
   c->bits_conv = bits_per((int)hp.t_conv);
   c->bits_left = bits_per((int)hp.t_exp_left);
   c->bits_right = bits_per((int)hp.t_exp_right);
+  c->live_gsw = live_digits((int)hp.t_gsw);
+  c->live_conv = live_digits((int)hp.t_conv);
+  c->live_left = live_digits((int)hp.t_exp_left);
+  c->live_right = live_digits((int)hp.t_exp_right);
   c->q2 = kQ2Values[hp.q2_bits];
   c->q1 = 4 * hp.p;
   c->q1_bits = (int)log2_ceil_u64(c->q1);
@@ -1395,7 +1399,7 @@
     int k = dims - 1;
     for (size_t half = num / 2; half >= 1; half /= 2, k--) {
       launch_fold_res(c->dp, a.p, b.p, 1, num * 4 * POLY, (int)half, vf.p + (size_t)k * mat, c->fold_words(), 1,
-                      (int)c->hp.t_gsw, c->bits_gsw, zflags.p, c->stream);
+                      (int)c->hp.t_gsw, c->bits_gsw, c->live_gsw, zflags.p, c->stream);
       B200_CUDA(cudaMemcpyAsync(a.p, b.p, half * 4 * POLY * 4, cudaMemcpyDeviceToDevice, c->stream));
     }
     launch_res_to_raw(c->dp, cts.p, a.p, num * 2, c->stream);
@@ -1484,7 +1488,7 @@
   DevBuf<uint32_t> o(outp * 2 * POLY), res(nn * 4 * POLY);
   B200_CUDA(cudaMemcpyAsync(cts.p, v_ct, cts.n * 8, cudaMemcpyHostToDevice, c->stream));
   launch_raw_to_res(c->dp, res.p, cts.p, nn * 2, c->stream);
-  launch_pack(c->dp, raw.p, 0, res.p, 4 * POLY, 0, 1, c->pp_table(pp, 1).pack, (int)hp.n, 1, (int)hp.t_conv, c->bits_conv, (int)hp.version, c->stream,
+  launch_pack(c->dp, raw.p, 0, res.p, 4 * POLY, 0, 1, c->pp_table(pp, 1).pack, (int)hp.n, 1, (int)hp.t_conv, c->bits_conv, c->live_conv, (int)hp.version, c->stream,
               cts.p);
   launch_to_ntt(c->dp, o.p, raw.p, outp, c->stream);
   launch_widen(wide.p, o.p, o.n, c->stream);
diff --git a/sdk_b200/csrc/gadget.hpp b/sdk_b200/csrc/gadget.hpp
--- /dev/null
+++ b/sdk_b200/csrc/gadget.hpp
@@ -0,0 +1,18 @@
+#pragma once
+
+namespace b200pir {
+
+constexpr int kModulusLog2 = 56;
+
+inline int bits_per(int t) {
+  if (t == 56) return 1;
+  return kModulusLog2 / t + 1;
+}
+
+inline int live_digits(int t) {
+  const int bits = bits_per(t);
+  const int need = (kModulusLog2 + bits - 1) / bits;
+  return need < t ? need : t;
+}
+
+}
diff --git a/sdk_b200/csrc/kernels.h b/sdk_b200/csrc/kernels.h
--- a/sdk_b200/csrc/kernels.h
+++ b/sdk_b200/csrc/kernels.h
@@ -76,7 +76,7 @@
                        const uint32_t* c_pos, const uint32_t* c_neg, size_t c_batch_stride ,
                        int slices_per_query, int t_gsw, int bits, cudaStream_t s);
 void launch_fold_res(const DevParams& P, const uint32_t* in, uint32_t* out, size_t batch, size_t batch_stride ,
-                     int half, const uint32_t* c_pos, size_t c_batch_stride, int slices_per_query, int t_gsw, int bits,
+                     int half, const uint32_t* c_pos, size_t c_batch_stride, int slices_per_query, int t_gsw, int bits, int live,
                      uint32_t* zero_flags , cudaStream_t s);
 void launch_folding_neg(const DevParams& P, uint32_t* out, const uint32_t* v_folding, int count, int t_gsw, int bits,
                         cudaStream_t s);
@@ -90,6 +90,7 @@
   const uint32_t* const* tab_right;
   size_t off_left, off_right;
   int t_left, t_right, bits_left, bits_right;
+  int live_left, live_right;
   int fill_skipped;
 };
 void launch_expand_round(const DevParams& P, uint32_t* v, size_t v_stride, int nq, const ExpandRound& R, cudaStream_t s);
@@ -101,11 +102,11 @@
                      int idx_factor, cudaStream_t s);
 void launch_regev_to_gsw(const DevParams& P, uint32_t* v_gsw, size_t gsw_stride, const uint32_t* v, size_t v_stride,
                          int nq, int count, int idx_factor, int idx_offset, const uint32_t* const* tab_conv, int t_gsw,
-                         int t_conv, int bits_conv, cudaStream_t s);
+                         int t_conv, int bits_conv, int live_conv, cudaStream_t s);
 
 void launch_pack(const DevParams& P, uint64_t* out_raw, size_t out_q_stride, const uint32_t* folded, size_t ct_stride,
                  size_t in_q_stride, int nq, const uint32_t* const* tab_pack, int n, int instances, int t_conv, int bits_conv,
-                 int version, cudaStream_t s, const uint64_t* raw_cts = nullptr);
+                 int live_conv, int version, cudaStream_t s, const uint64_t* raw_cts = nullptr);
 void launch_encode(const DevParams& P, uint8_t* out, size_t out_bytes, const uint64_t* packed_raw, size_t packed_q_stride,
                    int nq, int n, int instances, uint64_t q2, int q2_bits, uint64_t q1, int q1_bits, cudaStream_t s);
 
diff --git a/sdk_b200/csrc/poly_kernels.cu b/sdk_b200/csrc/poly_kernels.cu
--- a/sdk_b200/csrc/poly_kernels.cu
+++ b/sdk_b200/csrc/poly_kernels.cu
@@ -142,6 +142,22 @@
   __device__ __forceinline__ uint64_t operator()(int a) const { return p[a * 256]; }
 };
 
+template <int ROWS>
+__device__ __forceinline__ void mac_digit(uint64_t (&acc)[ROWS][8], const uint32_t (&x)[8], const uint32_t* c, size_t row_step) {
+#pragma unroll
+  for (int r = 0; r < ROWS; r++) {
+    uint32_t cv[8];
+    ld8_ro(cv, c + (size_t)r * row_step);
+#pragma unroll
+    for (int e = 0; e < 8; e++) acc[r][e] += (uint64_t)x[e] * cv[e];
+  }
+}
+template <int ROWS>
+__device__ __forceinline__ void acc_room(uint64_t (&acc)[ROWS][8], int& cnt, int n, const Grp& g) {
+  if (cnt + n > 16) { acc_reduce<ROWS>(acc, g); cnt = 1; }
+  cnt += n;
+}
+
 template <int ROWS, bool SM, bool BYTE, typename Coef>
 __device__ __forceinline__ void digits_mac_impl(uint64_t (&acc)[ROWS][8], int& cnt, Coef v, int ndig,
                                                 int bits, const uint32_t* c0, size_t col_step, size_t row_step,
@@ -159,23 +175,10 @@
         x1[a] = gadget_digit_fast<BYTE>(va, k + 1, bits, mask);
       }
       ntt_forward_group2_lz<NTT_OUT_LAZY16>(g.tid, x0, x1, g.smem, g.smem2, TwConst{g.n, 0}, TwShared{g.fwd_hi_sm}, g.q, CtaSync());
-      if (cnt + 2 > 16) { acc_reduce<ROWS>(acc, g); cnt = 1; }
-      cnt += 2;
+      acc_room<ROWS>(acc, cnt, 2, g);
       const uint32_t* c = c0 + (size_t)k * col_step;
-#pragma unroll
-      for (int r = 0; r < ROWS; r++) {
-        uint32_t cv[8];
-        ld8_ro(cv, c + (size_t)r * row_step);
-#pragma unroll
-        for (int e = 0; e < 8; e++) acc[r][e] += (uint64_t)x0[e] * cv[e];
-      }
-#pragma unroll
-      for (int r = 0; r < ROWS; r++) {
-        uint32_t cv[8];
-        ld8_ro(cv, c + col_step + (size_t)r * row_step);
-#pragma unroll
-        for (int e = 0; e < 8; e++) acc[r][e] += (uint64_t)x1[e] * cv[e];
-      }
+      mac_digit<ROWS>(acc, x0, c, row_step);
+      mac_digit<ROWS>(acc, x1, c + col_step, row_step);
     }
   }
 #pragma unroll 1
@@ -185,16 +188,8 @@
     for (int a = 0; a < 8; a++) x[a] = gadget_digit_fast<BYTE>(v(a), k, bits, mask);
     if (SM) ntt_forward_group_lz<NTT_OUT_LAZY16>(g.tid, x, g.smem, TwConst{g.n, 0}, TwShared{g.fwd_hi_sm}, g.q, CtaSync());
     else ntt_forward_group_lz<NTT_OUT_LAZY16>(g.tid, x, g.smem, TwConst{g.n, 0}, TwGlobal{g.fwd}, g.q, CtaSync());
-    if (cnt + 1 > 16) { acc_reduce<ROWS>(acc, g); cnt = 1; }
-    cnt += 1;
-    const uint32_t* c = c0 + (size_t)k * col_step;
-#pragma unroll
-    for (int r = 0; r < ROWS; r++) {
-      uint32_t cv[8];
-      ld8_ro(cv, c + (size_t)r * row_step);
-#pragma unroll
-      for (int e = 0; e < 8; e++) acc[r][e] += (uint64_t)x[e] * cv[e];
-    }
+    acc_room<ROWS>(acc, cnt, 1, g);
+    mac_digit<ROWS>(acc, x, c0 + (size_t)k * col_step, row_step);
   }
 }
 
@@ -376,24 +371,24 @@
   return __byte_perm((uint32_t)vh, (uint32_t)(vh >> 32), sel) + 0x01000100u -
          __byte_perm((uint32_t)vi, (uint32_t)(vi >> 32), sel);
 }
-constexpr int kFoldPlanes = 4;
+constexpr int kFoldPlanes = 3;
 
 template <bool BYTE>
 __global__ void __launch_bounds__(256, 2)
 k_fold_res_lz(DevParams P, const uint32_t* __restrict__ in, uint32_t* __restrict__ out, size_t batch_stride, int half,
-              const uint32_t* __restrict__ c_pos, size_t c_batch_stride, int slices_per_query, int t_gsw, int bits,
+              const uint32_t* __restrict__ c_pos, size_t c_batch_stride, int slices_per_query, int t_gsw, int bits, int live,
               const uint32_t* __restrict__ zero_flags ) {
+  const int n = blockIdx.x, i = blockIdx.y, b = blockIdx.z;
   if (zero_flags) {
-    const int bz = blockIdx.x / half, iz = blockIdx.x % half;
-    const uint32_t fa = zero_flags[(size_t)bz * 2 * half + iz], fb = zero_flags[(size_t)bz * 2 * half + half + iz];
+    const uint32_t fa = zero_flags[(size_t)b * 2 * half + i], fb = zero_flags[(size_t)b * 2 * half + half + i];
     if (fa | fb) {
-      const uint32_t* src = in + (size_t)bz * batch_stride + (size_t)((fa ? half : 0) + iz) * 4 * POLY;
-      uint32_t* dst = out + (size_t)bz * batch_stride + (size_t)iz * 4 * POLY;
+      const uint32_t* src = in + (size_t)b * batch_stride + (size_t)((fa ? half : 0) + i) * 4 * POLY;
+      uint32_t* dst = out + (size_t)b * batch_stride + (size_t)i * 4 * POLY;
 #pragma unroll
       for (int rho = 0; rho < 2; rho++) {
         uint32_t x[8];
-        ld8_ro(x, src + ((size_t)rho * 2 + blockIdx.y) * POLY + threadIdx.x * 8);
-        st8(dst + ((size_t)rho * 2 + blockIdx.y) * POLY + threadIdx.x * 8, x);
+        ld8_ro(x, src + ((size_t)rho * 2 + n) * POLY + threadIdx.x * 8);
+        st8(dst + ((size_t)rho * 2 + n) * POLY + threadIdx.x * 8, x);
       }
       return;
     }
@@ -402,11 +397,10 @@
   uint32_t* sm0 = reinterpret_cast<uint32_t*>(dyn_smem);
   uint32_t* sm1 = sm0 + NTT_SMEM_WORDS;
   Twiddle* tw = reinterpret_cast<Twiddle*>(sm1 + NTT_SMEM_WORDS);
-  Grp g = make_grp_single(P, sm0, blockIdx.y);
+  Grp g = make_grp_single(P, sm0, n);
   stage_fwd_twiddles(g, tw);
   const TwConst lo{g.n, 0};
   const TwShared hi{tw};
-  const int b = blockIdx.x / half, i = blockIdx.x % half;
   const uint32_t* ci = in + (size_t)b * batch_stride + (size_t)i * 4 * POLY;
   const uint32_t* ch = in + (size_t)b * batch_stride + (size_t)(half + i) * 4 * POLY;
   const uint32_t* C = c_pos + (size_t)(b / slices_per_query) * c_batch_stride;
@@ -415,6 +409,8 @@
   const uint64_t mask = (1ull << bits) - 1;
   const uint32_t q = g.q;
   uint32_t* planes = reinterpret_cast<uint32_t*>(tw + HI_TW) + g.tid;
+  uint32_t* spare = planes + (BYTE ? kFoldPlanes : 0) * POLY;
+  const uint32_t* cb = C + (size_t)g.n * POLY + g.tid * 8;
 
   uint64_t acc[2][8];
 #pragma unroll
@@ -433,13 +429,13 @@
       if (BYTE) {
 #pragma unroll
         for (int p = 0; p < kFoldPlanes; p++)
-          if (2 * p < t_gsw) planes[p * POLY + a * 256] = byte_pair_diff(vh[a], vi[a], 2 * p);
+          if (2 * p + 1 < live) planes[p * POLY + a * 256] = byte_pair_diff(vh[a], vi[a], 2 * p);
       }
-    }
-    const uint32_t* c0 = C + ((size_t)rho * 2 + g.n) * POLY + g.tid * 8;
-    int k = 0;
-#pragma unroll 1
-    for (; k + 1 < t_gsw; k += 2) {
+      if (live & 1) spare[rho * POLY + a * 256] = digit_diff(vh[a], vi[a], live - 1, bits, mask, q);
+    }
+    const uint32_t* c0 = cb + (size_t)rho * 2 * POLY;
+#pragma unroll 1
+    for (int k = 0; k + 1 < live; k += 2) {
       uint32_t x0[8], x1[8];
 #pragma unroll
       for (int a = 0; a < 8; a++) {
@@ -453,39 +449,23 @@
         }
       }
       ntt_forward_group2_lz<NTT_OUT_LAZY16>(g.tid, x0, x1, sm0, sm1, lo, hi, q, CtaSync());
-      if (cnt + 2 > 16) { acc_reduce<2>(acc, g); cnt = 1; }
-      cnt += 2;
-#pragma unroll
-      for (int r = 0; r < 2; r++) {
-        uint32_t cv[8];
-        ld8_ro(cv, c0 + (size_t)r * row_step + (size_t)k * 4 * POLY);
-#pragma unroll
-        for (int e = 0; e < 8; e++) acc[r][e] += (uint64_t)x0[e] * cv[e];
-      }
-#pragma unroll
-      for (int r = 0; r < 2; r++) {
-        uint32_t cv[8];
-        ld8_ro(cv, c0 + (size_t)r * row_step + (size_t)(k + 1) * 4 * POLY);
-#pragma unroll
-        for (int e = 0; e < 8; e++) acc[r][e] += (uint64_t)x1[e] * cv[e];
-      }
-    }
-    if (k < t_gsw) {
-      uint32_t x0[8];
-#pragma unroll
-      for (int a = 0; a < 8; a++)
-        x0[a] = BYTE ? (planes[(k >> 1) * POLY + a * 256] & 0xffffu) + (q - 256u) : digit_diff(vh[a], vi[a], k, bits, mask, q);
-      ntt_forward_group_lz<NTT_OUT_LAZY16>(g.tid, x0, sm0, lo, hi, q, CtaSync());
-      if (cnt + 1 > 16) { acc_reduce<2>(acc, g); cnt = 1; }
-      cnt += 1;
-#pragma unroll
-      for (int r = 0; r < 2; r++) {
-        uint32_t cv[8];
-        ld8_ro(cv, c0 + (size_t)r * row_step + (size_t)k * 4 * POLY);
-#pragma unroll
-        for (int e = 0; e < 8; e++) acc[r][e] += (uint64_t)x0[e] * cv[e];
-      }
-    }
+      acc_room<2>(acc, cnt, 2, g);
+      mac_digit<2>(acc, x0, c0 + (size_t)k * 4 * POLY, row_step);
+      mac_digit<2>(acc, x1, c0 + (size_t)(k + 1) * 4 * POLY, row_step);
+    }
+  }
+  if (live & 1) {
+    const int k = live - 1;
+    uint32_t x0[8], x1[8];
+#pragma unroll
+    for (int a = 0; a < 8; a++) {
+      x0[a] = spare[a * 256];
+      x1[a] = spare[POLY + a * 256];
+    }
+    ntt_forward_group2_lz<NTT_OUT_LAZY16>(g.tid, x0, x1, sm0, sm1, lo, hi, q, CtaSync());
+    acc_room<2>(acc, cnt, 2, g);
+    mac_digit<2>(acc, x0, cb + (size_t)k * 4 * POLY, row_step);
+    mac_digit<2>(acc, x1, cb + (size_t)k * 4 * POLY + 2 * POLY, row_step);
   }
   uint32_t y0[8], y1[8];
 #pragma unroll
@@ -566,6 +546,7 @@
   const uint32_t* W = left ? R.tab_left[blockIdx.y] + R.off_left : R.tab_right[blockIdx.y] + R.off_right;
   const int t_exp = left ? R.t_left : R.t_right;
   const int bits = left ? R.bits_left : R.bits_right;
+  const int live = left ? R.live_left : R.live_right;
 
   stage_fwd_twiddles(g, tw + g.n * HI_TW);
   uint32_t* vi = v + (size_t)i * 4 * POLY;
@@ -588,7 +569,7 @@
 #pragma unroll
     for (int e = 0; e < 8; e++) acc[r][e] = 0;
   int cnt = 0;
-  digits_mac<2, true>(acc, cnt, SmemCoef{autom + g.tid}, t_exp, bits, W + (size_t)g.n * POLY + g.tid * 8, (size_t)2 * POLY,
+  digits_mac<2, true>(acc, cnt, SmemCoef{autom + g.tid}, live, bits, W + (size_t)g.n * POLY + g.tid * 8, (size_t)2 * POLY,
                       (size_t)t_exp * 2 * POLY, g);
   uint32_t y[8];
   {
@@ -651,6 +632,7 @@
   const uint32_t* W = left ? R.tab_left[blockIdx.y] + R.off_left : R.tab_right[blockIdx.y] + R.off_right;
   const int t_exp = left ? R.t_left : R.t_right;
   const int bits = left ? R.bits_left : R.bits_right;
+  const int live = left ? R.live_left : R.live_right;
 
   stage_fwd_twiddles(g, tw + g.n * HI_TW);
   uint32_t* vi = v + (size_t)i * 4 * POLY;
@@ -704,7 +686,7 @@
 #pragma unroll
       for (int e = 0; e < 8; e++) acc[r][e] = 0;
     int cnt = 0;
-    digits_mac<2, true>(acc, cnt, SmemCoef{autom + g.tid}, t_exp, bits, W + (size_t)g.n * POLY + g.tid * 8, (size_t)2 * POLY,
+    digits_mac<2, true>(acc, cnt, SmemCoef{autom + g.tid}, live, bits, W + (size_t)g.n * POLY + g.tid * 8, (size_t)2 * POLY,
                         (size_t)t_exp * 2 * POLY, g);
     uint32_t* dst = half ? vo : vi;
 #pragma unroll
@@ -762,7 +744,7 @@
   uint32_t* sm0 = reinterpret_cast<uint32_t*>(dyn_smem);
   uint32_t* sm1 = sm0 + NTT_SMEM_WORDS;
   uint64_t* autom = reinterpret_cast<uint64_t*>(sm1 + NTT_SMEM_WORDS);
-  Twiddle* tw = reinterpret_cast<Twiddle*>(autom + POLY);
+  Twiddle* tw = reinterpret_cast<Twiddle*>(autom + 2 * POLY);
   Grp g = make_grp_single(P, sm0, blockIdx.y);
   g.smem2 = sm1;
   const int i = blockIdx.x;
@@ -789,6 +771,7 @@
   const uint32_t* W = left ? R.tab_left[blockIdx.z] + R.off_left : R.tab_right[blockIdx.z] + R.off_right;
   const int t_exp = left ? R.t_left : R.t_right;
   const int bits = left ? R.bits_left : R.bits_right;
+  const int live = left ? R.live_left : R.live_right;
   stage_fwd_twiddles(g, tw);
   const uint32_t* x0r = xr + (size_t)i * 2 * POLY;
   const uint32_t* x1r = x0r + POLY;
@@ -810,17 +793,39 @@
       const uint64_t val = crt_compose(a0, a1, P);
       const unsigned prod = (unsigned)k * (unsigned)R.t_auto;
       const unsigned num = prod >> NTT_LOG_N, rem = prod & (POLY - 1);
-      autom[rem] = (num & 1u) ? Q - val : val;
-    }
-    __syncthreads();
+      autom[half * POLY + rem] = (num & 1u) ? Q - val : val;
+    }
+  }
+  __syncthreads();
+  const uint32_t* Wn = W + (size_t)g.n * POLY + g.tid * 8;
+  const size_t row_step = (size_t)t_exp * 2 * POLY;
+  const int kl = live - 1;
+  uint32_t carry[8];
+#pragma unroll 1
+  for (int half = 1; half >= 0; half--) {
     uint64_t acc[2][8];
 #pragma unroll
     for (int r = 0; r < 2; r++)
 #pragma unroll
       for (int e = 0; e < 8; e++) acc[r][e] = 0;
     int cnt = 0;
-    digits_mac<2, true>(acc, cnt, SmemCoef{autom + g.tid}, t_exp, bits, W + (size_t)g.n * POLY + g.tid * 8, (size_t)2 * POLY,
-                        (size_t)t_exp * 2 * POLY, g);
+    if (!half && (live & 1)) {
+      mac_digit<2>(acc, carry, Wn + (size_t)kl * 2 * POLY, row_step);
+      cnt = 1;
+    }
+    digits_mac<2, true>(acc, cnt, SmemCoef{autom + half * POLY + g.tid}, live & ~1, bits, Wn, (size_t)2 * POLY, row_step, g);
+    if (half && (live & 1)) {
+      const uint64_t mask = (1ull << bits) - 1;
+      uint32_t x[8];
+#pragma unroll
+      for (int a = 0; a < 8; a++) {
+        x[a] = gadget_digit(autom[POLY + a * 256 + g.tid], kl, bits, mask);
+        carry[a] = gadget_digit(autom[a * 256 + g.tid], kl, bits, mask);
+      }
+      ntt_forward_group2_lz<NTT_OUT_LAZY16>(g.tid, x, carry, sm0, sm1, TwConst{g.n, 0}, TwShared{tw}, g.q, CtaSync());
+      acc_room<2>(acc, cnt, 1, g);
+      mac_digit<2>(acc, x, Wn + (size_t)kl * 2 * POLY, row_step);
+    }
     uint32_t yy[8];
 #pragma unroll
     for (int e = 0; e < 8; e++) {
@@ -865,7 +870,7 @@
 
 __global__ void __launch_bounds__(CTA, 1)
 k_regev_to_gsw(DevParams P, uint32_t* v_gsw, size_t gsw_stride, const uint32_t* v, size_t v_stride, int idx_factor,
-               int idx_offset, const uint32_t* const* tab_conv, int t_gsw, int t_conv, int bits_conv) {
+               int idx_offset, const uint32_t* const* tab_conv, int t_gsw, int t_conv, int bits_conv, int live_conv) {
   const uint32_t* v_conv = tab_conv[blockIdx.y];
   v_gsw += (size_t)blockIdx.y * gsw_stride;
   v += (size_t)blockIdx.y * v_stride;
@@ -902,7 +907,7 @@
 #pragma unroll 1
   for (int rho = 0; rho < 2; rho++) {
     const uint32_t* c0 = v_conv + ((size_t)rho * 2 + g.n) * POLY + g.tid * 8;
-    digits_mac<2, true>(acc, cnt, SmemCoef{raw + rho * POLY + g.tid}, t_conv, bits_conv, c0, (size_t)2 * 2 * POLY, (size_t)ccols * 2 * POLY, g);
+    digits_mac<2, true>(acc, cnt, SmemCoef{raw + rho * POLY + g.tid}, live_conv, bits_conv, c0, (size_t)2 * 2 * POLY, (size_t)ccols * 2 * POLY, g);
   }
 #pragma unroll
   for (int r = 0; r < 2; r++) {
@@ -916,7 +921,7 @@
 template <int ROWS>
 __global__ void __launch_bounds__(CTA, 1)
 k_pack(DevParams P, uint64_t* out_raw, size_t out_q_stride, const uint32_t* folded, size_t ct_stride, size_t in_q_stride,
-       const uint32_t* const* tab_pack, int t_conv, int bits, int version, const uint64_t* __restrict__ raw_cts) {
+       const uint32_t* const* tab_pack, int t_conv, int bits, int live, int version, const uint64_t* __restrict__ raw_cts) {
   const uint32_t* v_packing = tab_pack[blockIdx.y];
   out_raw += (size_t)blockIdx.y * out_q_stride;
   folded += (size_t)blockIdx.y * in_q_stride;
@@ -959,7 +964,8 @@
 #pragma unroll
         for (int a = 0; a < 8; a++) vv[a] = crt_compose(__ldg(ct + a * 256 + g.tid), __ldg(ct + POLY + a * 256 + g.tid), P);
       }
-      digits_mac<ROWS, true>(acc, cnt, RegCoef{vv}, t_conv, bits, W + (size_t)g.n * POLY + g.tid * 8, col_step, row_step, g);
+      digits_mac<ROWS, true>(acc, cnt, RegCoef{vv}, raw_cts ? t_conv : live, bits, W + (size_t)g.n * POLY + g.tid * 8, col_step,
+                             row_step, g);
     }
     uint32_t y[8];
 #pragma unroll
@@ -995,7 +1001,7 @@
 #pragma unroll
           for (int e = 0; e < 8; e++) acc[m][e] = 0;
         cnt = 0;
-        digits_mac<ROWS, true>(acc, cnt, SmemCoef{rawbuf + g.tid}, t_conv, bits, Wshift + (size_t)g.n * POLY + g.tid * 8, col_step, row_step, g);
+        digits_mac<ROWS, true>(acc, cnt, SmemCoef{rawbuf + g.tid}, live, bits, Wshift + (size_t)g.n * POLY + g.tid * 8, col_step, row_step, g);
         uint32_t np[ROWS][8];
 #pragma unroll
         for (int m = 0; m < ROWS; m++)
@@ -1110,7 +1116,7 @@
   if (polys) ++g_kernel_launches, k_res_to_raw<<<grid1d(polys * POLY, 256), 256, 0, s>>>(P, out, res, polys);
 }
 void launch_fold_res(const DevParams& P, const uint32_t* in, uint32_t* out, size_t batch, size_t batch_stride, int half,
-                     const uint32_t* c_pos, size_t c_batch_stride, int slices_per_query, int t_gsw, int bits,
+                     const uint32_t* c_pos, size_t c_batch_stride, int slices_per_query, int t_gsw, int bits, int live,
                      uint32_t* zero_flags, cudaStream_t s) {
   if (batch == 0 || half == 0) return;
   if (zero_flags) {
@@ -1118,12 +1124,15 @@
     k_ct_zero_flags<<<(unsigned)(batch * 2 * half), 256, 0, s>>>(in, batch_stride, 2 * half, zero_flags);
   }
   ++g_kernel_launches;
-  const dim3 grid((unsigned)(batch * half), 2);
-  const bool byte = bits == 8 && t_gsw <= 2 * kFoldPlanes;
-  const size_t smem = kDynSmemFold + (byte ? (size_t)kFoldPlanes * POLY * 4 : 0);
+  if (batch > 65535) throw Error(-2, "fold: more than 65535 ciphertext batches in one launch");
+  const dim3 grid(2, (unsigned)half, (unsigned)batch);
+  const bool byte = bits == 8 && live / 2 <= kFoldPlanes;
+  const size_t planes = (size_t)(byte ? kFoldPlanes : 0) * POLY * 4, spare = (size_t)2 * POLY * 4;
+  const size_t smem = kDynSmemFold + planes + ((live & 1) ? spare : 0);
   auto kern = byte ? k_fold_res_lz<true> : k_fold_res_lz<false>;
-  opt_in_smem(kern, (int)smem);
-  kern<<<grid, 256, smem, s>>>(P, in, out, batch_stride, half, c_pos, c_batch_stride, slices_per_query, t_gsw, bits, zero_flags);
+  opt_in_smem(kern, (int)(kDynSmemFold + planes + spare));
+  kern<<<grid, 256, smem, s>>>(P, in, out, batch_stride, half, c_pos, c_batch_stride, slices_per_query, t_gsw, bits, live,
+                               zero_flags);
 }
 void launch_from_ntt(const DevParams& P, uint64_t* out_raw, const uint32_t* in, size_t count, cudaStream_t s) {
   if (count) ++g_kernel_launches, k_from_ntt<<<(unsigned)count, CTA, 0, s>>>(P, out_raw, in);
@@ -1166,7 +1175,7 @@
 }
 void launch_expand_round_res(const DevParams& P, uint32_t* v, size_t v_stride, uint32_t* xr, size_t xr_stride, int nq,
                              const ExpandRound& R, const uint32_t* neg1_r, cudaStream_t s) {
-  const size_t smem = (size_t)2 * NTT_SMEM_WORDS * 4 + (size_t)POLY * 8 + (size_t)HI_TW * 8;
+  const size_t smem = (size_t)2 * NTT_SMEM_WORDS * 4 + (size_t)2 * POLY * 8 + (size_t)HI_TW * 8;
   opt_in_smem(k_expand_round_res, (int)smem);
   g_kernel_launches += 2;
   k_expand_intt<<<dim3((unsigned)R.num_in, 2, nq), 256, 0, s>>>(P, v, v_stride, xr, xr_stride, R);
@@ -1180,32 +1189,32 @@
 }
 void launch_regev_to_gsw(const DevParams& P, uint32_t* v_gsw, size_t gsw_stride, const uint32_t* v, size_t v_stride,
                          int nq, int count, int idx_factor, int idx_offset, const uint32_t* const* tab_conv, int t_gsw,
-                         int t_conv, int bits_conv, cudaStream_t s) {
+                         int t_conv, int bits_conv, int live_conv, cudaStream_t s) {
   if (count == 0) return;
   opt_in_smem(k_regev_to_gsw, (int)kDynSmemBig);
   ++g_kernel_launches;
   k_regev_to_gsw<<<dim3((unsigned)(count * t_gsw), nq), CTA, kDynSmemBig, s>>>(P, v_gsw, gsw_stride, v, v_stride,
                                                                                idx_factor, idx_offset, tab_conv, t_gsw,
-                                                                               t_conv, bits_conv);
+                                                                               t_conv, bits_conv, live_conv);
 }
 template <int ROWS>
 static void launch_pack_t(const DevParams& P, uint64_t* out_raw, size_t out_q_stride, const uint32_t* folded,
                           size_t ct_stride, size_t in_q_stride, int nq, const uint32_t* const* tab_pack, int instances,
-                          int t_conv, int bits_conv, int version, const uint64_t* raw_cts, cudaStream_t s) {
+                          int t_conv, int bits_conv, int live_conv, int version, const uint64_t* raw_cts, cudaStream_t s) {
   opt_in_smem(k_pack<ROWS>, (int)kDynSmemBig);
   ++g_kernel_launches;
   k_pack<ROWS><<<dim3((unsigned)(instances * (ROWS - 1)), nq), CTA, kDynSmemBig, s>>>(
-      P, out_raw, out_q_stride, folded, ct_stride, in_q_stride, tab_pack, t_conv, bits_conv, version, raw_cts);
+      P, out_raw, out_q_stride, folded, ct_stride, in_q_stride, tab_pack, t_conv, bits_conv, live_conv, version, raw_cts);
 }
 void launch_pack(const DevParams& P, uint64_t* out_raw, size_t out_q_stride, const uint32_t* folded, size_t ct_stride,
                  size_t in_q_stride, int nq, const uint32_t* const* tab_pack, int n, int instances, int t_conv, int bits_conv,
-                 int version, cudaStream_t s, const uint64_t* raw_cts) {
+                 int live_conv, int version, cudaStream_t s, const uint64_t* raw_cts) {
   if (raw_cts && nq != 1) throw Error(-2, "pack: raw ciphertexts are taken for one query");
   switch (n) {
-    case 1: launch_pack_t<2>(P, out_raw, out_q_stride, folded, ct_stride, in_q_stride, nq, tab_pack, instances, t_conv, bits_conv, version, raw_cts, s); break;
-    case 2: launch_pack_t<3>(P, out_raw, out_q_stride, folded, ct_stride, in_q_stride, nq, tab_pack, instances, t_conv, bits_conv, version, raw_cts, s); break;
-    case 3: launch_pack_t<4>(P, out_raw, out_q_stride, folded, ct_stride, in_q_stride, nq, tab_pack, instances, t_conv, bits_conv, version, raw_cts, s); break;
-    case 4: launch_pack_t<5>(P, out_raw, out_q_stride, folded, ct_stride, in_q_stride, nq, tab_pack, instances, t_conv, bits_conv, version, raw_cts, s); break;
+    case 1: launch_pack_t<2>(P, out_raw, out_q_stride, folded, ct_stride, in_q_stride, nq, tab_pack, instances, t_conv, bits_conv, live_conv, version, raw_cts, s); break;
+    case 2: launch_pack_t<3>(P, out_raw, out_q_stride, folded, ct_stride, in_q_stride, nq, tab_pack, instances, t_conv, bits_conv, live_conv, version, raw_cts, s); break;
+    case 3: launch_pack_t<4>(P, out_raw, out_q_stride, folded, ct_stride, in_q_stride, nq, tab_pack, instances, t_conv, bits_conv, live_conv, version, raw_cts, s); break;
+    case 4: launch_pack_t<5>(P, out_raw, out_q_stride, folded, ct_stride, in_q_stride, nq, tab_pack, instances, t_conv, bits_conv, live_conv, version, raw_cts, s); break;
     default: throw Error(-2, "pack: n must be 1..4");
   }
 }
```

After: 1288, median of 6. 1.06x the previous value.
